# 34j/vr180-convert

Measured on AMD Instinct MI355X. Metric: Mpixels/s dual-fisheye->SBS-equirect remap; achieved HBM GB/s vs peak, higher is better.
Workload: dtype f64; 1 GPU; C2: L+R 4096x4096 fisheye -> 8192x4096 SBS equirect, PolynomialScaler([0,1,-0.1]), bilinear; arithmetic=f64 coordinates (fused chain), u8 pixels with int32 fixed-point blend, split=frames, buffer_sets=4

## Files before the change

include/vr180_remap.h:

```cpp
#ifndef VR180_REMAP_H
#define VR180_REMAP_H

#include <stdint.h>

#ifdef __cplusplus
extern "C" {
#endif

#define V1C_ABI_VERSION 1

#define V1C_OK             0
#define V1C_E_INVALID     -1
#define V1C_E_UNSUPPORTED -2
#define V1C_E_HIP         -3
#define V1C_E_NODEVICE    -4
#define V1C_E_CORRUPT     -5

#define V1C_INTER_NEAREST  0
#define V1C_INTER_LINEAR   1
#define V1C_INTER_CUBIC    2
#define V1C_INTER_AREA     3
#define V1C_INTER_LANCZOS4 4

#define V1C_BORDER_CONSTANT    0
#define V1C_BORDER_REPLICATE   1
#define V1C_BORDER_REFLECT     2
#define V1C_BORDER_WRAP        3
#define V1C_BORDER_REFLECT_101 4
#define V1C_BORDER_TRANSPARENT 5

#define V1C_MAX_OPS    16
#define V1C_MAX_PARAMS 16

enum v1c_opcode {
    V1C_OP_NORMALIZE = 1,
    V1C_OP_DENORMALIZE = 2,
    V1C_OP_DENORMALIZE_INV = 3,
    V1C_OP_ZOOM = 4,
    V1C_OP_ZOOM_INV = 5,
    V1C_OP_EQUIRECT_ENC = 6,
    V1C_OP_EQUIRECT_DEC = 7,
    V1C_OP_RADIAL = 8,
    V1C_OP_ROTATE = 9
};

enum v1c_radial {
    V1C_RAD_ENC_RECTILINEAR   = 1,
    V1C_RAD_ENC_STEREOGRAPHIC = 2,
    V1C_RAD_ENC_EQUIDISTANT   = 3,
    V1C_RAD_ENC_EQUISOLID     = 4,
    V1C_RAD_ENC_ORTHOGRAPHIC  = 5,
    V1C_RAD_DEC_RECTILINEAR   = 6,
    V1C_RAD_DEC_STEREOGRAPHIC = 7,
    V1C_RAD_DEC_EQUIDISTANT   = 8,
    V1C_RAD_DEC_EQUISOLID     = 9,
    V1C_RAD_DEC_ORTHOGRAPHIC  = 10,
    V1C_RAD_POLYNOMIAL        = 11,
    V1C_RAD_RECTDEC_FWD       = 12,
    V1C_RAD_RECTDEC_INV       = 13
};

typedef struct v1c_op {
    int32_t opcode;
    int32_t iparam;
    int32_t nparam;
    int32_t reserved;
    double  p[V1C_MAX_PARAMS];
} v1c_op;

typedef struct v1c_chain {
    int32_t n_ops;
    int32_t reserved;
    v1c_op  ops[V1C_MAX_OPS];
} v1c_chain;

typedef struct v1c_unit {
    const uint8_t* src;
    uint8_t*       dst;
    int64_t        src_pitch;
    int64_t        dst_pitch;
    double         rot[9];
    int32_t        has_rot;
    int32_t        reserved;
} v1c_unit;

typedef struct v1c_plan v1c_plan;


int v1c_abi_version(void);
int v1c_device_count(void);
const char* v1c_last_error(void);


int v1c_plan_create(v1c_plan** out, int device, const v1c_chain* chain,
                    int src_h, int src_w, int dst_h, int dst_w, int cn,
                    int interp, int border_mode, const uint8_t border_val[4]);

#define V1C_DEPTH_8U  0
#define V1C_DEPTH_16U 2
#define V1C_DEPTH_32F 5

int v1c_plan_create_ex(v1c_plan** out, int device, const v1c_chain* chain, int src_h, int src_w,
                       int dst_h, int dst_w, int cn, int depth, int interp, int border_mode,
                       const double border_val[4]);
int v1c_plan_destroy(v1c_plan* plan);

int v1c_plan_path(const v1c_plan* plan);

int v1c_plan_run(v1c_plan* plan, void* stream, const v1c_unit* units, int n_units);

int v1c_plan_run_auto(v1c_plan* plan, void* stream, const v1c_unit* units, int n_units,
                      const double* rad_dev, int n_rad);

int v1c_plan_run_auto_images(v1c_plan* plan, void* stream, const v1c_unit* units, int n_units,
                             int threshold);

int v1c_plan_release_captures(v1c_plan* plan);

enum {
    V1C_LAUNCH_GENERIC = 0,
    V1C_LAUNCH_TILE = 1,
    V1C_LAUNCH_MIRROR = 2,
    V1C_LAUNCH_CN = 3,
    V1C_LAUNCH_CN_ROT = 4,
    V1C_LAUNCH_BATCH = 5,
    V1C_LAUNCH_ROT_PAIR = 6,
    V1C_LAUNCH_WIDE = 7,
    V1C_LAUNCH_CHROMA = 8,
    V1C_LAUNCH_FIXUP = 0x100
};
int v1c_plan_last_launch(const v1c_plan* plan);

int64_t v1c_plan_tap_table_bytes(const v1c_plan* plan);

int v1c_plan_get_map(v1c_plan* plan, void* stream, float* xmap, float* ymap,
                     int64_t map_pitch, const double* rot_or_null);

int v1c_remap_fused(int device, void* stream,
                    const uint8_t* src, int src_h, int src_w, int64_t src_pitch, int cn,
                    uint8_t* dst, int dst_h, int dst_w, int64_t dst_pitch,
                    const v1c_chain* chain, int interp, int border_mode,
                    const uint8_t border_val[4]);

int v1c_fused_cache_size(void);

int v1c_remap_lut(int device, void* stream,
                  const uint8_t* src, int src_h, int src_w, int64_t src_pitch, int cn,
                  uint8_t* dst, int dst_h, int dst_w, int64_t dst_pitch,
                  const float* xmap, const float* ymap, int64_t map_pitch,
                  int interp, int border_mode, const uint8_t border_val[4]);

int v1c_remap_lut_ex(int device, void* stream, const void* src, int src_h, int src_w, int64_t src_pitch,
                     int cn, int depth, void* dst, int dst_h, int dst_w, int64_t dst_pitch,
                     const float* xmap, const float* ymap, int64_t map_pitch,
                     int interp, int border_mode, const double border_val[4]);

int v1c_get_radius(int device, void* stream, const uint8_t* img, int h, int w,
                   int64_t pitch, int cn, int threshold, double* radius);
int v1c_get_radius_async(int device, void* stream, const uint8_t* img, int h, int w,
                         int64_t pitch, int cn, int threshold, double* out_dev);

int v1c_anaglyph(int device, void* stream,
                 const uint8_t* left, int64_t left_pitch, const uint8_t* right, int64_t right_pitch,
                 int h, int w, double* out, int64_t out_pitch);

int v1c_build_itab(int interp, int16_t* out);

int v1c_build_ftab(int interp, float* out);

typedef struct v1c_feat_params {
    double  scale;
    double  radius;
    int32_t fast_threshold;
    int32_t margin;
    int32_t cell;
    int32_t per_cell;
    int32_t max_keypoints;
    int32_t max_distance;
    int32_t ratio_num;
    int32_t ratio_den;
} v1c_feat_params;

typedef struct v1c_feat_kp {
    int32_t x, y;
    int32_t score;
    int32_t bin;
    int32_t src_x2, src_y2;
} v1c_feat_kp;

int v1c_feat_detect(int device, void* stream, const uint8_t* img, int h, int w, int64_t pitch, int cn,
                    const v1c_feat_params* params, v1c_feat_kp* kp_out, uint8_t* desc_out, int32_t* count_out_dev);

int v1c_feat_match(int device, void* stream, const uint8_t* desc_a, int n_a, const uint8_t* desc_b, int n_b,
                   const v1c_feat_params* params, int32_t* pairs_out, int32_t* dist_out, int32_t* count_out_dev);

int v1c_feat_pattern(int8_t* out);

typedef struct v1c_circle_params {
    int32_t threshold;
    int32_t run;
    int32_t rounds;
    int32_t min_points;
    int32_t tol16[8];
} v1c_circle_params;

typedef struct v1c_circle_point {
    int32_t x, y;
    int32_t selected;
} v1c_circle_point;

uint64_t v1c_fit_circle_workspace(int h, int w);

int v1c_fit_circle_async(int device, void* stream, const void* img, int h, int w, int64_t pitch, int cn, int depth,
                         const v1c_circle_params* params, void* workspace, double* out_dev8);

int v1c_fit_circle(int device, void* stream, const void* img, int h, int w, int64_t pitch, int cn, int depth,
                   const v1c_circle_params* params, void* workspace, double* out_host8, v1c_circle_point* points_out,
                   int32_t capacity, int32_t* n_points_out);

#define V1C_CM_MODE_HISTOGRAM   0
#define V1C_CM_MODE_GAIN        1
#define V1C_CM_REFERENCE_LEFT   0
#define V1C_CM_REFERENCE_RIGHT  1

typedef struct v1c_color_match_params {
    int32_t mode;
    int32_t reference;
    int32_t lo, hi;
    int32_t max_shift;
    int32_t min_pixels;
} v1c_color_match_params;

uint64_t v1c_color_match_workspace(void);

int v1c_color_match_luts_async(int device, void* stream, const void* left, int64_t left_pitch, const void* right, int64_t right_pitch,
                               int h, int w, int cn, const v1c_color_match_params* params, void* workspace, uint8_t* luts_dev,
                               int32_t* report_dev);

int v1c_apply_luts_async(int device, void* stream, const void* src, int64_t src_pitch, void* dst, int64_t dst_pitch, int h, int w, int cn,
                         const uint8_t* luts_dev);

#define V1C_PNG_FILTER_UP    2
#define V1C_PNG_FILTER_PAETH 4

typedef struct v1c_png_band {
    uint32_t row0, row1;
    uint64_t offset, size;
    uint32_t adler32;
    uint32_t stored;
} v1c_png_band;

uint64_t v1c_png_bound(int h, int w, int cn, int depth, int band_rows);

int v1c_png_deflate(int device, void* stream, const void* img, int h, int w, int64_t pitch, int cn, int depth, int filter,
                    int band_rows, uint8_t* out_host, uint64_t capacity, v1c_png_band* bands_out, int32_t* n_bands_out,
                    uint64_t* size_out);

#define V1C_JPEG_444 0
#define V1C_JPEG_420 2
#define V1C_JPEG_HEADER_MAX 1024

uint64_t v1c_jpeg_bound(int h, int w, int cn, int subsampling, int restart_mcus);

int64_t v1c_jpeg_header(int h, int w, int cn, int quality, int subsampling, int restart_mcus, uint8_t* out, uint64_t capacity);

int v1c_jpeg_encode(int device, void* stream, const void* img, int h, int w, int64_t pitch, int cn, int quality, int subsampling,
                    int restart_mcus, uint8_t* out_host, uint64_t capacity, uint64_t* size_out);

typedef struct v1c_jpeg_image {
    const void* img;
    int h, w;
    int64_t pitch;
    int cn, quality, subsampling, restart_mcus;
    uint8_t* out_host;
    uint64_t capacity;
    uint64_t size;
} v1c_jpeg_image;
int v1c_jpeg_encode_batch(int device, void* stream, int n, v1c_jpeg_image* images, uint64_t workspace_budget, uint32_t* chunks_out);

#define V1C_JPEG_DHT_MAX (4 * (1 + 16 + 256))
#define V1C_JPEG_HEADER_OPT_MAX 2048

int64_t v1c_jpeg_header_opt(int h, int w, int cn, int quality, int subsampling, int restart_mcus, const uint8_t* dht, uint32_t dht_size,
                            uint8_t* out, uint64_t capacity);

int v1c_jpeg_encode_opt(int device, void* stream, const void* img, int h, int w, int64_t pitch, int cn, int quality, int subsampling,
// ... 144 lines not shown
```

vr180_convert_amd/_native.py:

```python
from __future__ import annotations

import ctypes as C
from pathlib import Path

from . import _abi

import os

LIB_PATH = Path(os.environ.get("V1C_LIB") or (Path(__file__).resolve().parent / "csrc" / "libvr180remap.so"))

SYMBOLS = [
    "v1c_abi_version", "v1c_device_count", "v1c_last_error", "v1c_plan_create", "v1c_plan_destroy",
    "v1c_plan_path", "v1c_plan_run", "v1c_plan_get_map", "v1c_remap_fused", "v1c_remap_lut",
    "v1c_get_radius", "v1c_get_radius_async", "v1c_build_itab", "v1c_anaglyph", "v1c_fused_cache_size", "v1c_plan_last_launch",
    "v1c_plan_release_captures", "v1c_plan_run_auto", "v1c_plan_run_auto_images",
    "v1c_plan_create_ex", "v1c_remap_lut_ex", "v1c_build_ftab",
    "v1c_feat_detect", "v1c_feat_match", "v1c_feat_pattern",
    "v1c_png_bound", "v1c_png_deflate",
    "v1c_jpeg_bound", "v1c_jpeg_header", "v1c_jpeg_encode", "v1c_jpeg_encode_batch",
    "v1c_jpeg_decode_info", "v1c_jpeg_decode", "v1c_jpeg_decode_batch",
    "v1c_jpeg_header_opt", "v1c_jpeg_encode_opt", "v1c_jpeg_encode_batch_opt",
    "v1c_jpeg_prog_info", "v1c_jpeg_prog_decode",
    "v1c_jpeg_transcode_bound", "v1c_jpeg_transcode_check", "v1c_jpeg_header_xc", "v1c_jpeg_transcode",
    "v1c_jpeg_compose_bound", "v1c_jpeg_compose_check", "v1c_jpeg_header_xf", "v1c_jpeg_compose",
    "v1c_fit_circle_workspace", "v1c_fit_circle_async", "v1c_fit_circle",
    "v1c_color_match_workspace", "v1c_color_match_luts_async", "v1c_apply_luts_async",
    "v1c_plan_tap_table_bytes",
    "v1c_ca_plan_create", "v1c_ca_plan_run", "v1c_ca_plan_get_map", "v1c_ca_plan_path", "v1c_ca_plan_last_launch", "v1c_ca_plan_destroy",
]


class EngineUnavailable(RuntimeError):
    """The HIP library is not built / not loadable."""


class EngineError(RuntimeError):
    """A C-ABI call returned an error code."""


_lib = None


def lib() -> C.CDLL:
    global _lib
    if _lib is not None:
        return _lib
    if not LIB_PATH.exists():
        raise EngineUnavailable(
            f"{LIB_PATH} is missing: build the HIP engine first (make -C {LIB_PATH.parent}); "
            "vr180_convert_amd has no CPU fallback"
        )
    try:
        L = C.CDLL(str(LIB_PATH))
    except OSError as e:
        raise EngineUnavailable(f"cannot load {LIB_PATH}: {e}") from e
    vp, i32, i64 = C.c_void_p, C.c_int, C.c_int64
    L.v1c_abi_version.restype = i32
    L.v1c_device_count.restype = i32
    L.v1c_last_error.restype = C.c_char_p
    L.v1c_plan_create.argtypes = [C.POINTER(vp), i32, C.POINTER(_abi.Chain), i32, i32, i32, i32, i32, i32, i32, vp]
    L.v1c_plan_destroy.argtypes = [vp]
    L.v1c_plan_path.argtypes = [vp]
    L.v1c_plan_last_launch.argtypes = [vp]
    L.v1c_plan_last_launch.restype = i32
    try:
        L.v1c_plan_release_captures.argtypes = [vp]
        L.v1c_plan_run_auto.argtypes = [vp, vp, C.POINTER(_abi.Unit), i32, vp, i32]
        L.v1c_plan_run_auto_images.argtypes = [vp, vp, C.POINTER(_abi.Unit), i32, i32]
    except AttributeError:
        pass
    try:
        L.v1c_plan_create_ex.argtypes = [C.POINTER(vp), i32, C.POINTER(_abi.Chain), i32, i32, i32, i32, i32, i32, i32, i32, vp]
        L.v1c_remap_lut_ex.argtypes = [i32, vp, vp, i32, i32, i64, i32, i32, vp, i32, i32, i64, vp, vp, i64, i32, i32, vp]
        L.v1c_build_ftab.argtypes = [i32, vp]
    except AttributeError:
        pass
    try:
        L.v1c_feat_detect.argtypes = [i32, vp, vp, i32, i32, i64, i32, vp, vp, vp, vp]
        L.v1c_feat_match.argtypes = [i32, vp, vp, i32, vp, i32, vp, vp, vp, vp]
        L.v1c_feat_pattern.argtypes = [vp]
    except AttributeError:
        pass
    try:
        L.v1c_png_bound.argtypes = [i32, i32, i32, i32, i32]
        L.v1c_png_bound.restype = C.c_uint64
        L.v1c_png_deflate.argtypes = [i32, vp, vp, i32, i32, i64, i32, i32, i32, i32, vp, C.c_uint64, vp, vp, vp]
    except AttributeError:
        pass
    try:
        L.v1c_jpeg_bound.argtypes = [i32, i32, i32, i32, i32]
        L.v1c_jpeg_bound.restype = C.c_uint64
        L.v1c_jpeg_header.argtypes = [i32, i32, i32, i32, i32, i32, vp, C.c_uint64]
        L.v1c_jpeg_header.restype = i64
        L.v1c_jpeg_encode.argtypes = [i32, vp, vp, i32, i32, i64, i32, i32, i32, i32, vp, C.c_uint64, vp]
    except AttributeError:
        pass
    try:
        L.v1c_jpeg_decode_info.argtypes = [C.c_char_p, C.c_uint64, vp]
        L.v1c_jpeg_decode.argtypes = [i32, vp, C.c_char_p, C.c_uint64, vp, i64, i32, C.c_uint32, vp]
    except AttributeError:
        pass
    try:
        L.v1c_jpeg_decode_batch.argtypes = [i32, vp, i32, vp, vp, vp, vp, vp, C.c_uint32, C.c_uint64, vp, vp, vp]
    except AttributeError:
        pass
    try:
        L.v1c_jpeg_encode_batch.argtypes = [i32, vp, i32, vp, C.c_uint64, vp]
    except AttributeError:
        pass
    try:
        L.v1c_jpeg_header_opt.argtypes = [i32, i32, i32, i32, i32, i32, vp, C.c_uint32, vp, C.c_uint64]
        L.v1c_jpeg_header_opt.restype = i64
        L.v1c_jpeg_encode_opt.argtypes = [i32, vp, vp, i32, i32, i64, i32, i32, i32, i32, vp, C.c_uint64, vp, vp, vp]
        L.v1c_jpeg_encode_batch_opt.argtypes = [i32, vp, i32, vp, C.c_uint64, vp]
    except AttributeError:
        pass
    try:
        L.v1c_jpeg_prog_info.argtypes = [C.c_char_p, C.c_uint64, vp]
        L.v1c_jpeg_prog_decode.argtypes = [i32, vp, C.c_char_p, C.c_uint64, vp, i64, i32, C.c_uint32, vp, vp, C.c_uint32]
    except AttributeError:
        pass
    try:
        L.v1c_jpeg_transcode_bound.argtypes = [C.c_char_p, C.c_uint64, i32, i32, i32]
        L.v1c_jpeg_transcode_bound.restype = C.c_uint64
        L.v1c_jpeg_transcode_check.argtypes = [C.c_char_p, C.c_uint64, i32, vp, vp]
        L.v1c_jpeg_header_xc.argtypes = [C.c_char_p, C.c_uint64, i32, i32, i32, vp, C.c_uint32, vp, C.c_uint64]
        L.v1c_jpeg_header_xc.restype = i64
        L.v1c_jpeg_transcode.argtypes = [i32, vp, C.c_char_p, C.c_uint64, i32, vp, C.c_uint32, vp]
    except AttributeError:
        pass
    try:
        L.v1c_jpeg_compose_bound.argtypes = [C.c_char_p, C.c_uint64, i32, i32, i32]
        L.v1c_jpeg_compose_bound.restype = C.c_uint64
        L.v1c_jpeg_compose_check.argtypes = [i32, vp, i32, vp, vp]
        L.v1c_jpeg_header_xf.argtypes = [C.c_char_p, C.c_uint64, i32, i32, i32, i32, vp, C.c_uint32, vp, C.c_uint64]
        L.v1c_jpeg_header_xf.restype = i64
        L.v1c_jpeg_compose.argtypes = [i32, vp, i32, vp, i32, vp, C.c_uint32, vp]
    except AttributeError:
        pass
    try:
        L.v1c_fit_circle_workspace.argtypes = [i32, i32]
        L.v1c_fit_circle_workspace.restype = C.c_uint64
        L.v1c_fit_circle_async.argtypes = [i32, vp, vp, i32, i32, i64, i32, i32, vp, vp, vp]
        L.v1c_fit_circle.argtypes = [i32, vp, vp, i32, i32, i64, i32, i32, vp, vp, vp, vp, i32, vp]
    except AttributeError:
        pass
    try:
        L.v1c_color_match_workspace.argtypes = []
        L.v1c_color_match_workspace.restype = C.c_uint64
        L.v1c_color_match_luts_async.argtypes = [i32, vp, vp, i64, vp, i64, i32, i32, i32, vp, vp, vp, vp]
        L.v1c_apply_luts_async.argtypes = [i32, vp, vp, i64, vp, i64, i32, i32, i32, vp]
    except AttributeError:
        pass
    try:
        L.v1c_ca_plan_create.argtypes = [C.POINTER(vp), i32, C.POINTER(_abi.Chain), i32, i32, i32, i32, i32, i32, vp]
        L.v1c_ca_plan_run.argtypes = [vp, vp, C.POINTER(_abi.Unit), i32]
        L.v1c_ca_plan_get_map.argtypes = [vp, vp, i32, vp, vp, i64, vp]
        L.v1c_ca_plan_path.argtypes = [vp]
        L.v1c_ca_plan_last_launch.argtypes = [vp]
        L.v1c_ca_plan_destroy.argtypes = [vp]
    except AttributeError:
        pass
    try:
        L.v1c_plan_tap_table_bytes.argtypes = [vp]
        L.v1c_plan_tap_table_bytes.restype = i64
    except AttributeError:
        pass
    L.v1c_plan_run.argtypes = [vp, vp, C.POINTER(_abi.Unit), i32]
    L.v1c_plan_get_map.argtypes = [vp, vp, vp, vp, i64, vp]
    L.v1c_remap_fused.argtypes = [i32, vp, vp, i32, i32, i64, i32, vp, i32, i32, i64, C.POINTER(_abi.Chain), i32, i32, vp]
    L.v1c_remap_lut.argtypes = [i32, vp, vp, i32, i32, i64, i32, vp, i32, i32, i64, vp, vp, i64, i32, i32, vp]
    L.v1c_get_radius.argtypes = [i32, vp, vp, i32, i32, i64, i32, i32, C.POINTER(C.c_double)]
    L.v1c_get_radius_async.argtypes = [i32, vp, vp, i32, i32, i64, i32, i32, vp]
    L.v1c_fused_cache_size.restype = i32
    L.v1c_build_itab.argtypes = [i32, vp]
    L.v1c_anaglyph.argtypes = [i32, vp, vp, i64, vp, i64, i32, i32, vp, i64]
    if L.v1c_abi_version() != _abi.ABI_VERSION:
        raise EngineUnavailable("libvr180remap.so was built for a different ABI version; rebuild it")
    _lib = L
    return L


def check(rc: int, what: str) -> None:
    if rc == _abi.OK:
        return
    msg = lib().v1c_last_error().decode("utf-8", "replace")
    if rc == _abi.E_INVALID:
        raise ValueError(f"{what}: {msg}")
    if rc == _abi.E_UNSUPPORTED:
        raise NotImplementedError(f"{what}: {msg}")
    raise EngineError(f"{what}: {msg} (code {rc})")
```

vr180_convert_amd/csrc/kernels.hpp:

```cpp
#pragma once

#include <cstdlib>
#include <vector>

#include "v1c_core.hpp"

namespace v1c {

#ifdef V1C_TUNING
inline const char* tuning_env(const char* name) { return std::getenv(name); }
#else
inline const char* tuning_env(const char*) { return nullptr; }
#endif

constexpr int kPX = 4;
constexpr int kBlockX = 64;
constexpr int kBlockY = 4;

enum { MODE_LITERAL = 0, MODE_RAY = 1, MODE_LUT = 2, MODE_FIXUP = 3 };

struct KernelCtx {
    Geom g;
    const v1c_chain* chain;
    RayParams ray;
    const short* itab;
    uint32_t* tile_flags;
    const float* xmap;
    const float* ymap;
    int64_t map_pitch;
};

constexpr int kInlineUnits = 16;
struct TileBox;
struct TileArgs {
    const KernelCtx* ctx;
    const DevUnit* units;
    const TileBox* boxes;
    const TileBox* mboxes;
    const uint32_t* rest_list;
    uint32_t* tile_flags;
    int n_units, upb;
    int half_dwords, n_rest;
    unsigned tiles_x_magic, strip_len, strip_magic, rest_rows;
    int mirror_h, kb, tiles_x, same_rot;
    const double *col_s, *col_c, *col_h, *row_s, *row_c, *row_h;
    int dst_w, dst_h, pad2[2];
    DevUnit inl[kInlineUnits];
};

struct LaunchUnits {
    const DevUnit* host;
    const DevUnit* dev;
    int n;
};

int tiles_per_unit(const Geom& g);
hipError_t launch_remap(int mode, const KernelCtx& c, const UnitArgs& ua, int n_units, hipStream_t stream);
hipError_t launch_get_map(int mode, const KernelCtx& c, const UnitArgs& u, float* xmap, float* ymap, int64_t pitch,
                          hipStream_t stream);

struct WideArgs {
    const float* ftab;
    float cval[4];
};
hipError_t launch_remap_wide(int mode, int depth, const KernelCtx& c, const UnitArgs& ua, const WideArgs& wa, int n_units, hipStream_t stream);

hipError_t launch_put_units(DevUnit* dst, const DevUnit* host, int n, hipStream_t stream);
bool tile_kernel_supports(const Geom& g);
bool cn_kernel_supports(const Geom& g);
int tile_cn_box_kb(const void* host_boxes, const Geom& g);
hipError_t launch_ray_lin_cn(const KernelCtx& c, const KernelCtx* cdev, const LaunchUnits& lu, uint32_t* flags, bool use_rot, const void* boxes,
                             int kb, hipStream_t stream);
size_t tile_box_bytes(const Geom& g);
hipError_t launch_tile_boxes(const KernelCtx& c, const KernelCtx* cdev, void* boxes, bool shared_entry, hipStream_t stream, int mirror_h = 0);
bool tile_mirror_rest(const void* host_boxes, const void* host_mboxes, const Geom& g, int half_dwords, int mirror_h,
                      std::vector<uint32_t>& rest, int raw_nwp, bool full_rows = false, int n_eyes = 2);
int tile_mirror_raw_passes(const void* host_boxes, const void* host_mboxes, const Geom& g, int permille = 980, int max_kb = 12);
hipError_t launch_ray_lin3_pair_mirror(const KernelCtx& c, const KernelCtx* cdev, const LaunchUnits& lu, uint32_t* flags, const void* boxes,
                                       const void* mboxes, int half_dwords, int mirror_h, const uint32_t* rest_list, int n_rest, int raw_nwp,
                                       hipStream_t stream, int seq_kb, const void* recs = nullptr, const void* tap_table = nullptr);
size_t tap_table_bytes(const Geom& g);
hipError_t launch_fill_tap_table(const KernelCtx& c, const KernelCtx* cdev, const void* boxes, const void* mboxes, void* table, uint32_t* overflow);
void tile_mirror_records(const void* host_boxes, const void* host_mboxes, size_t n_tiles, const Geom& g, int seq_kb, int one_kb, std::vector<char>& out);
int tile_half_dwords(const void* host_boxes, size_t n_tiles, int max_chunks, bool occupancy_classes);
hipError_t launch_ray_lin3_tile(const KernelCtx& c, const KernelCtx* cdev, const LaunchUnits& lu, uint32_t* flags, bool use_rot, const void* boxes,
                                int half_dwords, bool shared_entry, bool mpoly_all, const uint32_t* rest_list, int n_rest, int lean_half,
                                int strip_len, int lean_raw_nwp, hipStream_t stream, bool coords_bounded = false, int* kind = nullptr,
                                bool same_rot = false);
int tile_xcd_strips(const void* host_boxes, const Geom& g, int half_dwords, int lean_half);
int tile_lean_half_dwords(int half_dwords);
std::vector<uint32_t> tile_rest_list(const void* host_boxes, const Geom& g, int half_dwords, int raw_nwp);
int tile_lean_raw_passes(const void* host_boxes, const Geom& g);

hipError_t launch_anaglyph(const uint8_t* left, int64_t left_pitch, const uint8_t* right, int64_t right_pitch, int h, int w,
                           double* out, int64_t out_pitch, hipStream_t stream);

hipError_t launch_get_radius(const uint8_t* img, int h, int w, int64_t pitch, int cn, int threshold, double* out, hipStream_t stream);

hipError_t launch_patch_radius(KernelCtx* ctx_dev, const double* rad_dev, int n, double r_limit, double cx32, double cy32, hipStream_t stream);
constexpr int kAutoBlocks = 64;
constexpr int kAutoScratchInts = 2 * kInlineUnits + 1;
struct AutoLines {
    const uint8_t* line[kInlineUnits];
    int64_t step[kInlineUnits];
    int n, cn, threshold, count;
};
inline void auto_scratch_init(int* host)
{
    for (int k = 0; k < kInlineUnits; k++)
        host[k] = 0x7fffffff, host[kInlineUnits + k] = -1;
    host[2 * kInlineUnits] = 0;
}
hipError_t launch_auto_radius(KernelCtx* ctx_dev, int* scratch_dev, const AutoLines& im, double r_limit, double cx32, double cy32, hipStream_t stream);

}
```

vr180_convert_amd/csrc/kernels_mirror.hip:

```cpp
#include "tile_device.hpp"

namespace v1c {

__device__ __forceinline__ void sample_pair_cells(units_cptr U, const TileIds& t, int j, const TileBox& b, const uint32_t* boxw,
                                                  const int (&sx)[kPX], const int (&sy)[kPX])
{
    typedef uint32_t __attribute__((ext_vector_type(2))) u32x2;
    typedef const __attribute__((address_space(3))) u32x2* lds_u64_ptr;
    const uint32_t lpw8 = (uint32_t)(b.cpr * 4 + 4) * 8u;
    const uint32_t base0 = (uint32_t)(uintptr_t)(lds_u32_ptr)boxw - ((uint32_t)b.y0 * lpw8 + (uint32_t)b.x0 * 8u);
    Taps2 T0, T1;
#pragma unroll
    for (int k = 0; k < kPX; k++) {
        const uint32_t rel = __umul24((uint32_t)(sy[k] >> 5), lpw8) + (((uint32_t)sx[k] >> 2) & ~7u);
        const lds_u64_ptr ra = (lds_u64_ptr)(uintptr_t)(rel + base0), rb = (lds_u64_ptr)(uintptr_t)(rel + base0 + lpw8);
        const u32x2 a_lo = ra[0], a_hi = ra[1], b_lo = rb[0], b_hi = rb[1];
        T0.alo[k] = a_lo.x, T0.ahi[k] = a_hi.x, T0.blo[k] = b_lo.x, T0.bhi[k] = b_hi.x;
        T1.alo[k] = a_lo.y, T1.ahi[k] = a_hi.y, T1.blo[k] = b_lo.y, T1.bhi[k] = b_hi.y;
    }
    uint32_t pix[kPX];
    const uint32_t row_off = (uint32_t)t.x0 * 3u;
#pragma unroll
    for (int e = 0; e < 2; e++) {
#pragma unroll
        for (int k = 0; k < kPX; k++) {
            const BlendW w = blend_weights(sx[k], sy[k]);
            pix[k] = e == 0 ? blend3<4>(T0.alo[k], T0.ahi[k], T0.blo[k], T0.bhi[k], w) : blend3<4>(T1.alo[k], T1.ahi[k], T1.blo[k], T1.bhi[k], w);
        }
        uint8_t* drow = U[e].dst + (__umul24((uint32_t)j, (uint32_t)U[e].dst_pitch) + row_off);
        store4(drow, pix, 0xFu, dst_rows_dword_aligned(U, e));
    }
}

#ifdef V1C_TUNING
template <int VAR_W>
__global__ __launch_bounds__(256) __attribute__((amdgpu_waves_per_eu(5, 8))) void k_ray_lin3_pair_mirror(TileArgs a_)
{
    constexpr int NT = 256;
    __shared__ __attribute__((aligned(16))) double tabw[kTabSlice * kRadialCoefs];
    extern __shared__ __attribute__((aligned(16))) uint32_t dyn_box[];
    args_cref a = kernel_args();
    const int tid = threadIdx.x;
    if (blockIdx.z == 0) {
        const unsigned lin = blockIdx.y * gridDim.x + blockIdx.x;
        if (lin >= (unsigned)a.n_rest)
            return;
        const uint32_t v = ((const V1C_CONST uint32_t*)a.rest_list)[lin];
        shared_map_tile<VAR_W, 0, 2, 0, 1, NT, 0>(a, 2, 2, 0, (int)(v & 0xffffu), (int)(v >> 16), (int)gridDim.x, dyn_box, a.half_dwords,
                                                  tabw, (glb_u32_ptr) nullptr);
        return;
    }
    ctx_cref c = args_ctx(a);
    const units_cptr U = args_units(a);
    const TileBox* __restrict__ boxes = a.boxes;
    const TileBox* __restrict__ mboxes = a.mboxes;
    const int half_dwords = a.half_dwords, mirror_h = a.mirror_h;
    geom_cref g = c.g;
    ray_cref P = c.ray;
    int tx, ty;
    xcd_tile(a.tiles_x_magic, a.strip_len, a.strip_magic, tx, ty);
    ty += 1;
    const TileIds t = tile_ids(g, 0, tid, tx, ty, (int)gridDim.x, NT / kLanesX);
    const uint8_t* __restrict__ src0 = U[0].src;
    const uint8_t* __restrict__ src1 = U[1].src;
    const uint32_t pitch0 = (uint32_t)U[0].src_pitch, pitch1 = (uint32_t)U[1].src_pitch;
    const TileBox b = load_tile_box(boxes, t.box_tile), q = load_tile_box(mboxes, t.box_tile);
    if (!mirror_static_ok(b, q, half_dwords, g.src_h, g.src_w))
        return;
    ChunkMap M;
    make_chunk_map<NT>(b, tid, M);
    Staged S0, S1;
    stage_load<false, false>(M, src0, pitch0, 0u, S0);
    stage_load<false, false>(M, src1, pitch1, 0u, S1);
    typedef double __attribute__((ext_vector_type(2))) d2;
    d2 tv = {0.0, 0.0};
    const bool mpoly = (b.interior & 2) != 0;
    if (tid < b.nidx * 4)
        tv = ((const d2*)(radial_table(P, mpoly) + (size_t)b.idx0 * kRadialCoefs))[tid];
    RowCol rc;
    load_rowcol<0>(P, t.xc, t.jc, rc);
    stage_store_pair(M, S0, S1, dyn_box);
    if (tid < b.nidx * 4)
        ((d2*)tabw)[tid] = tv;
    __syncthreads();
    make_chunk_map<NT>(q, tid, M);
    stage_load<false, false>(M, src0, pitch0, 0u, S0);
    stage_load<false, false>(M, src1, pitch1, 0u, S1);
    LaneCoords L;
    if (mpoly)
        lane_coords<VAR_W, 0, 2, 0, 1, 1, 1>(c, nullptr, rc, kPX, (const double*)tabw, b.idx0, b.nidx, L);
    else
        lane_coords<VAR_W, 0, 2, 0, 1, 0, 1>(c, nullptr, rc, kPX, (const double*)tabw, b.idx0, b.nidx, L);
    sample_pair_cells(U, t, t.j, b, dyn_box, L.sx, L.sy);
    __syncthreads();
    stage_store_pair(M, S0, S1, dyn_box);
    __syncthreads();
    sample_pair_cells(U, t, mirror_h - t.j, q, dyn_box, L.sx, L.sy2);
}
#endif

template <int VAR_W, int NE, int REC>
__device__ __forceinline__ void mirror_raw_tile(V1C_MIRROR_HEAD, double* tabw, uint32_t* dyn_box)
{
    static_assert(!REC || NE == 1, "the record serves the one-eye form");
    constexpr int NT = 256;
    if (V1C_PRIO & 4)
        __builtin_amdgcn_s_setprio(3);
    args_cref a = kernel_args<kMirrorHeadBytes>();
    const int tid = threadIdx.x;
    const unsigned tiles_x = gx_rest & 0xffffu, rest_rows = gx_rest >> 16;
    if (blockIdx.y < rest_rows) {
        const unsigned lin = blockIdx.y * tiles_x + blockIdx.x;
        if (lin >= (unsigned)a.n_rest)
            return;
        const uint32_t v = ((const V1C_CONST uint32_t*)a.rest_list)[lin];
        shared_map_tile<VAR_W, 0, 2, 0, 1, NT, 0>(a, NE, 2, 0, (int)(v & 0xffffu), (int)(v >> 16), (int)tiles_x, dyn_box, a.half_dwords,
                                                  tabw, (glb_u32_ptr) nullptr);
        return;
    }
    int tx, ty;
    {
        const unsigned slen = ((rows_strip >> 16) * tiles_x) & (REC ? 0x7fffffffu : 0xffffffffu);
        xcd_tile_at(tiles_x_magic, slen, ((tiles_x_magic - 1u) >> 1) + 1u, tx, ty, rows_strip & 0xffffu, rest_rows, tiles_x, 0u);
    }
    const DstSize dsz{(int)(dst_wh & 0xffffu), (int)(dst_wh >> 16)};
    const TileIds t = tile_ids(dsz, 0, tid, tx, ty, (int)tiles_x, NT / kLanesX);
    RowCol rc;
    load_rowcol<0>(rowcol_tables_at(rowcol_tables, dsz.dst_w, dsz.dst_h), t.xc, t.jc, rc);
    TileBoxPair bq{};
    MirrorRec r{};
    if constexpr (REC)
        r = load_mirror_rec(pairs, t.box_tile);
    else
        bq = load_tile_box_pair(pairs, t.box_tile);
    const TileBox &b = bq.b, &q = bq.q;
    ctx_cref c = *(const V1C_CONST KernelCtx*)ctxp;
    const units_cptr U = (units_cptr)a.inl;
    geom_cref g = c.g;
    ray_cref P = c.ray;
    touch_plan_and_units<0, NE>(c, U, 0, NE - 1);
    const int nwp = (int)(kb_mh & 0xffffu);
    if (REC ? !(r.flags & kMirrorRecFitOne) : mirror_raw_fit(b, q, nwp, g.src_h, g.src_w) != 1)
        return;
    const bool mpoly = REC ? (r.flags & kMirrorRecMpoly) != 0 : (b.interior & 2) != 0;
    const int idx0 = REC ? r.idx0 : b.idx0, nidx = REC ? r.nidx : b.nidx;
#pragma unroll
    for (int k = 0; k < kPX; k++)
        asm volatile("" ::"v"(rc.slon[k]), "v"(rc.qlon[k]));
    asm volatile("" ::"v"(rc.sl), "v"(rc.cl), "v"(rc.hl));
    const uint32_t lds_tab = (uint32_t)(uintptr_t)(lds_u32_ptr)(const uint32_t*)tabw;
    const uint32_t box_bytes = (uint32_t)nwp * 1024u;
    const uint32_t raw_b = (uint32_t)(uintptr_t)(lds_u32_ptr)dyn_box, raw_q = raw_b + (uint32_t)NE * box_bytes;
// ... 76 lines not shown
#endif
__device__ __forceinline__ void gather_taps_raw(const uint32_t (&ta)[kPX], const BlendW (&W)[kPX], uint32_t pitch, uint32_t (&pix)[kPX])
{
#pragma unroll
    for (int k = 0; k < kPX; k++) {
        const uint32_t a = ta[k], d = a & ~3u;
        const lds_u32_ptr r0 = (lds_u32_ptr)(uintptr_t)d, r1 = (lds_u32_ptr)(uintptr_t)(d + pitch);
        const uint32_t a0 = r0[0], a1 = r0[1], a2 = r0[2], b0 = r1[0], b1 = r1[1], b2 = r1[2];
        pix[k] = blend3<3>(__builtin_amdgcn_alignbyte(a1, a0, a), __builtin_amdgcn_alignbyte(a2, a1, a), __builtin_amdgcn_alignbyte(b1, b0, a),
                           __builtin_amdgcn_alignbyte(b2, b1, a), W[k]);
    }
}

template <int VAR_W, int REST, int REC>
__device__ __forceinline__ void mirror_seq_tile(V1C_MIRROR_HEAD, double* tabw, uint32_t* dyn_box)
{
    constexpr int NT = 256;
    if (V1C_PRIO & 4)
        __builtin_amdgcn_s_setprio(3);
    args_cref a = kernel_args<kMirrorHeadBytes>();
    const int tid = threadIdx.x;
    const unsigned tiles_x = gx_rest & 0xffffu, rest_rows = REST ? gx_rest >> 16 : 0u;
    if constexpr (REST) {
        if (blockIdx.y < rest_rows) {
            const unsigned lin = blockIdx.y * tiles_x + blockIdx.x;
            if (lin >= (unsigned)a.n_rest)
                return;
            const uint32_t v = ((const V1C_CONST uint32_t*)a.rest_list)[lin];
            shared_map_tile<VAR_W, 0, 2, 0, 1, NT, 0>(a, 2, 2, 0, (int)(v & 0xffffu), (int)(v >> 16), (int)tiles_x, dyn_box,
                                                      a.half_dwords, tabw, (glb_u32_ptr) nullptr);
            return;
        }
    }
    int tx, ty;
    {
        const unsigned slen = ((rows_strip >> 16) * tiles_x) & (REC ? 0x7fffffffu : 0xffffffffu);
        xcd_tile_at(tiles_x_magic, slen, ((tiles_x_magic - 1u) >> 1) + 1u, tx, ty, rows_strip & 0xffffu, rest_rows, tiles_x, 0u);
    }
    const DstSize dsz{(int)(dst_wh & 0xffffu), (int)(dst_wh >> 16)};
    const TileIds t = tile_ids(dsz, 0, tid, tx, ty, (int)tiles_x, NT / kLanesX);
    RowCol rc;
    load_rowcol<0>(rowcol_tables_at(rowcol_tables, dsz.dst_w, dsz.dst_h), t.xc, t.jc, rc);
    TileBoxPair bq{};
    MirrorRec r{};
    if constexpr (REC)
        r = load_mirror_rec(pairs, t.box_tile);
    else
        bq = load_tile_box_pair(pairs, t.box_tile);
    const TileBox &b = bq.b, &q = bq.q;
    ctx_cref c = *(const V1C_CONST KernelCtx*)ctxp;
    const units_cptr U = (units_cptr)a.inl;
    geom_cref g = c.g;
    ray_cref P = c.ray;
    touch_plan_and_units<0, 2>(c, U, 0, 1);
    const int cap_kb = (int)(kb_mh & 0xffffu);
    if (REC ? !(r.flags & kMirrorRecFitSeq) : mirror_raw_fit(b, q, cap_kb, g.src_h, g.src_w) != 1)
        return;
    const bool mpoly = REC ? (r.flags & kMirrorRecMpoly) != 0 : (b.interior & 2) != 0;
    const int idx0 = REC ? r.idx0 : b.idx0, nidx = REC ? r.nidx : b.nidx;
#pragma unroll
    for (int k = 0; k < kPX; k++)
        asm volatile("" ::"v"(rc.slon[k]), "v"(rc.qlon[k]));
    asm volatile("" ::"v"(rc.sl), "v"(rc.cl), "v"(rc.hl));
    const uint32_t lds_tab = (uint32_t)(uintptr_t)(lds_u32_ptr)(const uint32_t*)tabw;
    const uint32_t raw_b = (uint32_t)(uintptr_t)(lds_u32_ptr)dyn_box, raw_q = raw_b + (uint32_t)cap_kb * 1024u;
    const int wave = __builtin_amdgcn_readfirstlane(tid >> 6), lane = tid & 63;
    {
        const uint32_t u = min((uint32_t)tid, (uint32_t)(nidx * 4 - 1));
        const uint8_t* gp = (const uint8_t*)(radial_table(P, mpoly) + (size_t)idx0 * kRadialCoefs) + u * 16u;
        __builtin_amdgcn_global_load_lds((glb_void_ptr)gp, (lds_void_ptr)(uintptr_t)(lds_tab + (uint32_t)__builtin_amdgcn_readfirstlane(tid & ~63) * 16u), 16, 0, 0);
    }
    const RawLanes mb = REC ? rec_lanes(r.b, lane) : raw_lanes(b.cpr, lane), mq = REC ? rec_lanes(r.q, lane) : raw_lanes(q.cpr, lane);
    auto request = [&](int e, int which) {
        const uint8_t* src = U[e].src;
        const uint32_t sp = (uint32_t)U[e].src_pitch;
        if constexpr (REC)
            return which == 0 ? rec_box_dma(r.b, mb, src, sp, lane, wave, raw_b) : rec_box_dma(r.q, mq, src, sp, lane, wave, raw_q);
        else
            return which == 0 ? raw_box_dma(b, mb, src, sp, lane, wave, raw_b) : raw_box_dma(q, mq, src, sp, lane, wave, raw_q);
    };
    const int nb = request(0, 0);
    const int nq = request(0, 1);
    if (V1C_PRIO & 4)
        __builtin_amdgcn_s_setprio(0);
    wait_vm_barrier(nb + nq);
    const uint32_t pitch_b = REC ? r.b.lpitch : (uint32_t)raw_units_per_row(b.cpr) * 16u, pitch_q = REC ? r.q.lpitch : (uint32_t)raw_units_per_row(q.cpr) * 16u;
    uint32_t ta_b[kPX], ta_q[kPX];
    BlendW W_b[kPX], W_q[kPX];
    {
        LaneCoords L;
        if (mpoly)
            lane_coords<VAR_W, 0, 2, 0, 1, 1, 1, 0, REC>(c, nullptr, rc, kPX, (const double*)tabw, idx0, nidx, L);
        else
            lane_coords<VAR_W, 0, 2, 0, 1, 0, 1, 0, REC>(c, nullptr, rc, kPX, (const double*)tabw, idx0, nidx, L);
        const uint32_t kb = r.b.tapk + raw_b, kq = r.q.tapk + raw_q;
#pragma unroll
        for (int k = 0; k < kPX; k++) {
            if constexpr (REC) {
                const uint32_t bx = ((uint32_t)L.sx[k] >> 5), x3 = bx * 2u + bx;
                ta_b[k] = mad24_vsv((uint32_t)L.sy[k] >> 5, pitch_b, x3 + kb);
                ta_q[k] = mad24_vsv((uint32_t)L.sy2[k] >> 5, pitch_q, x3 + kq);
            } else {
                const uint32_t ixb = (uint32_t)((L.sx[k] >> 5) - b.x0), ixq = (uint32_t)((L.sx[k] >> 5) - q.x0);
                ta_b[k] = __umul24((uint32_t)((L.sy[k] >> 5) - b.y0), pitch_b) + (ixb * 2u + ixb) + raw_b;
                ta_q[k] = __umul24((uint32_t)((L.sy2[k] >> 5) - q.y0), pitch_q) + (ixq * 2u + ixq) + raw_q;
            }
            W_b[k] = blend_weights(L.sx[k], L.sy[k]);
            W_q[k] = blend_weights(L.sx[k], L.sy2[k]);
        }
    }
    const uint32_t row_off = (uint32_t)t.x0 * 3u;
    const int jm = (int)(kb_mh >> 16) - t.j;
    const bool band_row = jm < dsz.dst_h;
    auto drow = [&](int e, int j) {
        return (REC ? mul24_vs((uint32_t)j, (uint32_t)U[e].dst_pitch) : __umul24((uint32_t)j, (uint32_t)U[e].dst_pitch)) + row_off;
    };
    uint32_t pix[kPX];
    wait_vm_barrier(nq);
    gather_taps_raw(ta_b, W_b, pitch_b, pix);
    asm volatile("s_waitcnt vmcnt(0) lgkmcnt(0)\n\ts_barrier" ::: "memory");
    request(1, 0);
    store4<1>(U[0].dst + drow(0, t.j), pix, 0xFu, dst_rows_dword_aligned(U, 0));
    gather_taps_raw(ta_q, W_q, pitch_q, pix);
    asm volatile("s_waitcnt lgkmcnt(0)\n\ts_barrier" ::: "memory");
    request(1, 1);
    if (band_row)
        store4<1>(U[0].dst + drow(0, jm), pix, 0xFu, dst_rows_dword_aligned(U, 0));
    wait_vm_barrier(nq + 1);
    gather_taps_raw(ta_b, W_b, pitch_b, pix);
    wait_vm_barrier_imm<0>();
    store4<1>(U[1].dst + drow(1, t.j), pix, 0xFu, dst_rows_dword_aligned(U, 1));
    gather_taps_raw(ta_q, W_q, pitch_q, pix);
    if (band_row)
        store4<1>(U[1].dst + drow(1, jm), pix, 0xFu, dst_rows_dword_aligned(U, 1));
}

template <int VAR_W, int REST = 1>
__global__ __launch_bounds__(256) __attribute__((amdgpu_waves_per_eu(REST ? V1C_SEQ_WAVES : V1C_SEQ_WAVES + 1, 8))) void k_ray_lin3_pair_mirror_seq(V1C_MIRROR_HEAD, TileArgs a_)
{
    __shared__ __attribute__((aligned(16))) double tabw[kTabSlice * kRadialCoefs];
    extern __shared__ __attribute__((aligned(16))) uint32_t dyn_box[];
    mirror_seq_tile<VAR_W, REST, 1>(pairs, tiles_x_magic, gx_rest, rows_strip, dst_wh, rowcol_tables, ctxp, kb_mh, tabw, dyn_box);
}
#ifdef V1C_TUNING
template <int VAR_W, int REST = 1>
__global__ __launch_bounds__(256) __attribute__((amdgpu_waves_per_eu(REST ? V1C_SEQ_WAVES : V1C_SEQ_WAVES + 1, 8))) void k_ray_lin3_pair_mirror_seq_box(V1C_MIRROR_HEAD, TileArgs a_)
{
    __shared__ __attribute__((aligned(16))) double tabw[kTabSlice * kRadialCoefs];
    extern __shared__ __attribute__((aligned(16))) uint32_t dyn_box[];
    mirror_seq_tile<VAR_W, REST, 0>(pairs, tiles_x_magic, gx_rest, rows_strip, dst_wh, rowcol_tables, ctxp, kb_mh, tabw, dyn_box);
}
#endif

constexpr int kTapSliceBytes = 256 * kTapEntryBytes;
__global__ __launch_bounds__(256) __attribute__((amdgpu_waves_per_eu(V1C_SEQ_WAVES + 1, 8))) void k_ray_lin3_pair_mirror_seq_tab(V1C_MIRROR_HEAD, TileArgs a_)
{
    constexpr int NT = 256;
    __shared__ __attribute__((aligned(16))) uint32_t tapw[kTapSliceBytes / 4];
    extern __shared__ __attribute__((aligned(16))) uint32_t dyn_box[];
    if (V1C_PRIO & 4)
        __builtin_amdgcn_s_setprio(3);
    args_cref a = kernel_args<kMirrorHeadBytes>();
    const int tid = threadIdx.x;
    const unsigned tiles_x = gx_rest & 0xffffu;
    int tx, ty;
    {
        const unsigned slen = ((rows_strip >> 16) * tiles_x) & 0x7fffffffu;
        xcd_tile_at(tiles_x_magic, slen, ((tiles_x_magic - 1u) >> 1) + 1u, tx, ty, rows_strip & 0xffffu, 0u, tiles_x, 0u);
    }
    const DstSize dsz{(int)(dst_wh & 0xffffu), (int)(dst_wh >> 16)};
    const TileIds t = tile_ids(dsz, 0, tid, tx, ty, (int)tiles_x, NT / kLanesX);
    const MirrorRec r = load_mirror_rec(pairs, t.box_tile);
    const units_cptr U = (units_cptr)a.inl;
    const uint8_t* usrc[2] = {U[0].src, U[1].src};
    uint8_t* udst[2] = {U[0].dst, U[1].dst};
    uint32_t uspitch[2] = {(uint32_t)U[0].src_pitch, (uint32_t)U[1].src_pitch}, udpitch[2] = {(uint32_t)U[0].dst_pitch, (uint32_t)U[1].dst_pitch};
    asm volatile("" : "+s"(usrc[0]), "+s"(usrc[1]), "+s"(udst[0]), "+s"(udst[1]), "+s"(uspitch[0]), "+s"(uspitch[1]), "+s"(udpitch[0]), "+s"(udpitch[1]));
    const bool ualigned[2] = {((((uintptr_t)udst[0]) | (uintptr_t)udpitch[0]) & 3u) == 0, ((((uintptr_t)udst[1]) | (uintptr_t)udpitch[1]) & 3u) == 0};
    const int cap_kb = (int)(kb_mh & 0xffffu);
    if (!(r.flags & kMirrorRecFitSeq))
        return;
    const uint32_t lds_tap = (uint32_t)(uintptr_t)(lds_u32_ptr)(const uint32_t*)tapw;
    const uint32_t raw_b = (uint32_t)(uintptr_t)(lds_u32_ptr)dyn_box, raw_q = raw_b + (uint32_t)cap_kb * 1024u;
    const int wave = __builtin_amdgcn_readfirstlane(tid >> 6), lane = tid & 63;
    {
        const uint32_t wave_off = (uint32_t)__builtin_amdgcn_readfirstlane(tid & ~63) * (uint32_t)kTapEntryBytes;
        const uint8_t* gp = (const uint8_t*)rowcol_tables + ((size_t)(uint32_t)__builtin_amdgcn_readfirstlane(t.box_tile) * (size_t)kTapSliceBytes + wave_off) +
                            (uint32_t)lane * 16u;
        if (lane < 64 * kTapEntryBytes / 16)
            __builtin_amdgcn_global_load_lds((glb_void_ptr)gp, (lds_void_ptr)(uintptr_t)(lds_tap + wave_off), 16, 0, 0);
    }
    const RawLanes mb = rec_lanes(r.b, lane), mq = rec_lanes(r.q, lane);
    auto request = [&](int e, int which) {
        const uint8_t* src = usrc[e];
        const uint32_t sp = uspitch[e];
        return which == 0 ? rec_box_dma(r.b, mb, src, sp, lane, wave, raw_b) : rec_box_dma(r.q, mq, src, sp, lane, wave, raw_q);
    };
    const int nb = request(0, 0);
    const int nq = request(0, 1);
    if (V1C_PRIO & 4)
        __builtin_amdgcn_s_setprio(0);
    wait_vm_barrier(nb + nq);
    const uint32_t pitch_b = r.b.lpitch, pitch_q = r.q.lpitch;
    uint32_t ta_b[kPX], ta_q[kPX];
    BlendW W_b[kPX], W_q[kPX];
    {
        const lds_u32_ptr ep = (lds_u32_ptr)(uintptr_t)(lds_tap + (uint32_t)tid * (uint32_t)kTapEntryBytes);
        const TapCoords tc = tap_entry_decode(TapEntry{{ep[0], ep[1], ep[2]}});
        const uint32_t kb = raw_b, kq = raw_q + (uint32_t)(r.b.x3 - r.q.x3);
#pragma unroll
        for (int k = 0; k < kPX; k++) {
            const uint32_t ix = (uint32_t)tc.x[k] >> 5, x3 = ix * 2u + ix;
            ta_b[k] = mad24_vsv((uint32_t)tc.y[k] >> 5, pitch_b, x3 + kb);
            ta_q[k] = mad24_vsv((uint32_t)tc.y2[k] >> 5, pitch_q, x3 + kq);
            W_b[k] = blend_weights(tc.x[k], tc.y[k]);
            W_q[k] = blend_weights(tc.x[k], tc.y2[k]);
        }
    }
    const uint32_t row_off = (uint32_t)t.x0 * 3u;
    const int jm = (int)(kb_mh >> 16) - t.j;
    const bool band_row = jm < dsz.dst_h;
    auto drow = [&](int e, int j) { return mul24_vs((uint32_t)j, udpitch[e]) + row_off; };
    uint32_t pix[kPX];
    wait_vm_barrier(nq);
    gather_taps_raw(ta_b, W_b, pitch_b, pix);
    asm volatile("s_waitcnt vmcnt(0) lgkmcnt(0)\n\ts_barrier" ::: "memory");
    request(1, 0);
    store4<1>(udst[0] + drow(0, t.j), pix, 0xFu, ualigned[0]);
    gather_taps_raw(ta_q, W_q, pitch_q, pix);
    asm volatile("s_waitcnt lgkmcnt(0)\n\ts_barrier" ::: "memory");
    request(1, 1);
    if (band_row)
        store4<1>(udst[0] + drow(0, jm), pix, 0xFu, ualigned[0]);
    wait_vm_barrier(nq + 1);
    gather_taps_raw(ta_b, W_b, pitch_b, pix);
    wait_vm_barrier_imm<0>();
    store4<1>(udst[1] + drow(1, t.j), pix, 0xFu, ualigned[1]);
    gather_taps_raw(ta_q, W_q, pitch_q, pix);
    if (band_row)
        store4<1>(udst[1] + drow(1, jm), pix, 0xFu, ualigned[1]);
}

template <int VAR_W>
__global__ __launch_bounds__(256) void k_fill_tap_table(const KernelCtx* ctxp, const TileBox* __restrict__ boxes, const TileBox* __restrict__ mboxes,
                                                        int tiles_x, uint32_t* __restrict__ table, uint32_t* overflow)
{
    ctx_cref c = *(const V1C_CONST KernelCtx*)ctxp;
    ray_cref P = c.ray;
    const int tid = threadIdx.x;
    const TileIds t = tile_ids(c.g, 0, tid, (int)blockIdx.x, (int)blockIdx.y, tiles_x, 256 / kLanesX);
    const TileBox b = boxes[t.box_tile], q = mboxes[t.box_tile];
    RowCol rc;
    load_rowcol<0>(P, t.xc, t.jc, rc);
    const bool mpoly = (b.interior & 2) != 0;
    const int nidx = max(b.nidx, 1), idx0 = max(b.idx0, 0);
    const double* tab = (mpoly ? P.radial_m : P.radial) + (size_t)idx0 * kRadialCoefs;
    LaneCoords L;
    if (mpoly)
        lane_coords<VAR_W, 0, 2, 0, 1, 1, 1, 0, 1>(c, nullptr, rc, kPX, tab, idx0, nidx, L);
    else
        lane_coords<VAR_W, 0, 2, 0, 1, 0, 1, 0, 1>(c, nullptr, rc, kPX, tab, idx0, nidx, L);
    TapCoords tc;
#pragma unroll
    for (int k = 0; k < kPX; k++) {
        tc.x[k] = (int)((uint32_t)L.sx[k] - kRoundBias) - 32 * b.x0;
        tc.y[k] = (int)((uint32_t)L.sy[k] - kRoundBias) - 32 * b.y0;
        tc.y2[k] = (int)((uint32_t)L.sy2[k] - kRoundBias) - 32 * q.y0;
    }
    if (!tap_entry_fits(tc))
        atomicOr(overflow, 1u);
    const TapEntry e = tap_entry_encode(tc);
    uint32_t* out = table + ((size_t)t.box_tile * 256u + (size_t)tid) * 3u;
    out[0] = e.w[0], out[1] = e.w[1], out[2] = e.w[2];
}

size_t tap_table_bytes(const Geom& g)
{
    const dim3 full = tile_grid(g, 256, 1);
    return (size_t)full.x * (size_t)(full.y / 2 + 1) * (size_t)kTapSliceBytes;
}

hipError_t launch_fill_tap_table(const KernelCtx& c, const KernelCtx* cdev, const void* boxes, const void* mboxes, void* table, uint32_t* overflow)
{
    const dim3 full = tile_grid(c.g, 256, 1);
    const dim3 grid(full.x, full.y / 2 + 1, 1), block(256, 1, 1);
    if (c.ray.var_is_w)
        hipLaunchKernelGGL((k_fill_tap_table<1>), grid, block, 0, 0, cdev, (const TileBox*)boxes, (const TileBox*)mboxes, (int)full.x, (uint32_t*)table, overflow);
    else
        hipLaunchKernelGGL((k_fill_tap_table<0>), grid, block, 0, 0, cdev, (const TileBox*)boxes, (const TileBox*)mboxes, (int)full.x, (uint32_t*)table, overflow);
    return hipGetLastError();
}

int tile_mirror_raw_passes(const void* host_boxes, const void* host_mboxes, const Geom& g, int permille, int max_kb)
{
    const TileBox* b = (const TileBox*)host_boxes;
    const TileBox* q = (const TileBox*)host_mboxes;
    const dim3 d = tile_grid(g, tile_threads(g), 1);
    std::vector<int> hist(kRawMaxWavePasses + 2, 0);
    size_t n = 0;
    for (unsigned ty = 0; ty <= d.y / 2; ty++)
        for (unsigned tx = 0; tx < d.x; tx++) {
            const size_t i = (size_t)ty * d.x + tx;
            if (b[i].cpr <= 0 || q[i].cpr <= 0 || b[i].cpr > kMaxCpr || q[i].cpr > kMaxCpr)
                continue;
            const int u = std::max(b[i].nrows * raw_units_per_row(b[i].cpr), q[i].nrows * raw_units_per_row(q[i].cpr));
            hist[std::min((u + 63) / 64, kRawMaxWavePasses + 1)]++, n++;
        }
    size_t acc = 0;
    for (int k = 0; k <= kRawMaxWavePasses; k++) {
        acc += hist[k];
        if (acc * 1000 >= n * (size_t)permille)
            return std::min(std::max(k, 4), max_kb);
    }
    return max_kb;
}

bool tile_mirror_rest(const void* host_boxes, const void* host_mboxes, const Geom& g, int half_dwords, int mirror_h,
                      std::vector<uint32_t>& rest, int raw_nwp, bool full_rows, int n_eyes)
{
    const TileBox* b = (const TileBox*)host_boxes;
    const TileBox* q = (const TileBox*)host_mboxes;
    const dim3 d = tile_grid(g, tile_threads(g), 1);
    rest.clear();
    const int th = tile_threads(g) / kLanesX;
    if (mirror_h != g.dst_h || g.dst_h % (2 * th) != 0 || g.dst_w % 4 != 0 || d.x > 0xffffu || d.y > 0xffffu)
        return false;
    const unsigned TY = d.y, TYh = TY / 2;
    if (TYh < 3)
        return false;
    std::vector<uint8_t> in_rest((size_t)d.x * d.y, 0);
    auto add = [&](unsigned tx, unsigned ty) { in_rest[(size_t)ty * d.x + tx] = 1; };
    if (full_rows && raw_nwp > 0) {
        for (unsigned ty = 0; ty <= TYh; ty++)
            for (unsigned tx = 0; tx < d.x; tx++) {
                const size_t i = (size_t)ty * d.x + tx;
                const int fit = mirror_raw_fit(b[i], q[i], raw_nwp, g.src_h, g.src_w);
                if (fit != 1) {
                    add(tx, ty);
                    if (ty < TYh) {
                        add(tx, TY - 1 - ty);
                        if (ty > 0)
                            add(tx, TY - ty);
                    }
                }
            }
    } else {
        for (unsigned tx = 0; tx < d.x; tx++)
            add(tx, 0), add(tx, TYh), add(tx, TY - 1);
        for (unsigned ty = 1; ty < TYh; ty++)
            for (unsigned tx = 0; tx < d.x; tx++) {
                const size_t i = (size_t)ty * d.x + tx;
                if (raw_nwp > 0 ? !mirror_raw_static_ok(b[i], q[i], raw_nwp, g.src_h, g.src_w) : !mirror_static_ok(b[i], q[i], half_dwords, g.src_h, g.src_w))
                    add(tx, ty), add(tx, TY - 1 - ty), add(tx, TY - ty);
            }
    }
    for (unsigned ty = 0; ty < d.y; ty++)
        for (unsigned tx = 0; tx < d.x; tx++)
            if (in_rest[(size_t)ty * d.x + tx])
                rest.push_back(ty << 16 | tx);
    return rest.size() <= (size_t)d.x * (TYh - 1) && rest.size() * 4 <= (size_t)d.x * d.y;
}

void tile_mirror_records(const void* host_boxes, const void* host_mboxes, size_t n_tiles, const Geom& g, int seq_kb, int one_kb, std::vector<char>& out)
{
    const TileBox* b = (const TileBox*)host_boxes;
    const TileBox* q = (const TileBox*)host_mboxes;
    out.resize(n_tiles * sizeof(MirrorRecWords));
    for (size_t i = 0; i < n_tiles; i++) {
        const MirrorRecWords w = mirror_rec_encode(b[i], q[i], seq_kb, one_kb, g.src_h, g.src_w);
        std::memcpy(&out[i * sizeof(MirrorRecWords)], &w, sizeof(w));
    }
}

hipError_t launch_ray_lin3_pair_mirror(const KernelCtx& c, const KernelCtx* cdev, const LaunchUnits& lu, uint32_t* flags, const void* boxes,
                                       const void* mboxes, int half_dwords, int mirror_h, const uint32_t* rest_list, int n_rest, int raw_nwp,
                                       hipStream_t stream, int seq_kb, const void* recs, const void* tap_table)
{
    const int n_eyes = lu.n;
    const dim3 full = tile_grid(c.g, 256, 1);
    const dim3 block(256, 1, 1);
    TileArgs a = tile_args(c, cdev, lu, flags);
    a.boxes = (const TileBox*)boxes, a.mboxes = (const TileBox*)mboxes;
    a.rest_list = rest_list, a.n_rest = n_rest;
    a.half_dwords = half_dwords, a.mirror_h = mirror_h;
    a.tiles_x_magic = (unsigned)(0x100000000ull / full.x) + 1u;
    static const unsigned strip_rows = [] {
        const char* e = tuning_env("V1C_MIRROR_STRIP_ROWS");
        return e ? (unsigned)std::atoi(e) : 2u;
    }();
    static const unsigned block_rows = [] {
        const char* e = tuning_env("V1C_MIRROR_BLOCK_ROWS");
        return e ? (unsigned)std::atoi(e) : 0u;
    }();
    [[maybe_unused]] auto strips = [&](unsigned rows) {
        const unsigned per = (full.x * rows) >> 3;
        unsigned slen = strip_rows && strip_rows * full.x < per ? strip_rows * full.x : 0u;
        if (block_rows && full.x % 8 == 0 && raw_nwp > 0)
            slen = 0x80000000u | std::min(block_rows, 0xffffu);
        a.strip_len = slen;
        a.strip_magic = (slen && !(slen & 0x80000000u)) ? (unsigned)(0x100000000ull / slen) + 1u : 0u;
    };
    const unsigned raw_rows = full.y / 2 + 1;
    const unsigned rest_rows = ((((unsigned)n_rest + full.x - 1) / full.x) + 7u) & ~7u;
    const unsigned srows = strip_rows == 2u && 2u * full.x < ((full.x * raw_rows) >> 3) ? 2u : 0u;
    const unsigned rows_strip = raw_rows | srows << 16, dst_wh = (unsigned)c.g.dst_w | (unsigned)c.g.dst_h << 16;
    const TileBox* head_pairs = (const TileBox*)recs;
#define V1C_MIRROR_LAUNCH(KERNEL, GRID, LDS, RESTROWS)                                                                                    \
    hipLaunchKernelGGL(KERNEL, GRID, block, LDS, stream, head_pairs, a.tiles_x_magic, full.x | (unsigned)(RESTROWS) << 16, rows_strip, dst_wh, \
                       a.col_s, a.ctx, (unsigned)a.kb | (unsigned)a.mirror_h << 16, a)
    [[maybe_unused]] bool rec_off = false;
#ifdef V1C_TUNING
    static const bool rec_off_env = [] {
        const char* e = tuning_env("V1C_MIRROR_REC");
        return e && e[0] == '0';
    }();
    rec_off = rec_off_env;
#endif
    if (seq_kb > 0 && n_eyes == 2) {
        static const bool norest_off = [] {
            const char* e = tuning_env("V1C_SEQ_NOREST");
            return e && e[0] == '0';
        }();
        a.kb = seq_kb;
        if (!rec_off && recs == nullptr)
            return hipErrorInvalidValue;
        if (n_rest == 0 && !norest_off) {
            const dim3 rgrid(full.x, raw_rows, 1);
            const size_t slds = (size_t)2 * 1024 * (size_t)seq_kb + 16;
            a.rest_rows = 0;
#ifdef V1C_TUNING
            if (rec_off) {
                head_pairs = a.mboxes;
                if (c.ray.var_is_w)
                    V1C_MIRROR_LAUNCH((k_ray_lin3_pair_mirror_seq_box<1, 0>), rgrid, slds, 0u);
                else
                    V1C_MIRROR_LAUNCH((k_ray_lin3_pair_mirror_seq_box<0, 0>), rgrid, slds, 0u);
                return hipGetLastError();
            }
            static const bool tab_off = [] {
                const char* e = tuning_env("V1C_MIRROR_TAB");
                return e && e[0] == '0';
            }();
            if (tab_off)
                tap_table = nullptr;
#endif
            if (tap_table) {
                hipLaunchKernelGGL(k_ray_lin3_pair_mirror_seq_tab, rgrid, block, slds, stream, head_pairs, a.tiles_x_magic, full.x, rows_strip, dst_wh,
                                   (const double*)tap_table, a.ctx, (unsigned)a.kb | (unsigned)a.mirror_h << 16, a);
                return hipGetLastError();
            }
            if (c.ray.var_is_w)
                V1C_MIRROR_LAUNCH((k_ray_lin3_pair_mirror_seq<1, 0>), rgrid, slds, 0u);
            else
                V1C_MIRROR_LAUNCH((k_ray_lin3_pair_mirror_seq<0, 0>), rgrid, slds, 0u);
            return hipGetLastError();
        }
        const dim3 rgrid(full.x, raw_rows + rest_rows, 1);
        const size_t slds = std::max((size_t)half_dwords * 8 + 16, (size_t)2 * 1024 * (size_t)seq_kb);
        a.rest_rows = rest_rows;
#ifdef V1C_TUNING
        if (rec_off) {
            head_pairs = a.mboxes;
            if (c.ray.var_is_w)
                V1C_MIRROR_LAUNCH((k_ray_lin3_pair_mirror_seq_box<1>), rgrid, slds, rest_rows);
            else
                V1C_MIRROR_LAUNCH((k_ray_lin3_pair_mirror_seq_box<0>), rgrid, slds, rest_rows);
            return hipGetLastError();
        }
#endif
        if (c.ray.var_is_w)
            V1C_MIRROR_LAUNCH((k_ray_lin3_pair_mirror_seq<1>), rgrid, slds, rest_rows);
        else
            V1C_MIRROR_LAUNCH((k_ray_lin3_pair_mirror_seq<0>), rgrid, slds, rest_rows);
        return hipGetLastError();
    }
    if (raw_nwp > 0 && n_eyes == 1) {
        const dim3 rgrid(full.x, raw_rows + rest_rows, 1);
        const size_t lds = std::max((size_t)half_dwords * 4 + 16, (size_t)2 * 1024 * (size_t)raw_nwp);
        a.kb = raw_nwp, a.rest_rows = rest_rows;
        if (!rec_off && recs == nullptr)
            return hipErrorInvalidValue;
#ifdef V1C_TUNING
        if (rec_off) {
            head_pairs = a.mboxes;
            if (c.ray.var_is_w)
                V1C_MIRROR_LAUNCH((k_ray_lin3_pair_mirror_box_raw<1>), rgrid, lds, rest_rows);
            else
                V1C_MIRROR_LAUNCH((k_ray_lin3_pair_mirror_box_raw<0>), rgrid, lds, rest_rows);
            return hipGetLastError();
        }
#endif
        if (c.ray.var_is_w)
            V1C_MIRROR_LAUNCH((k_ray_lin3_pair_mirror_raw<1, 1>), rgrid, lds, rest_rows);
        else
            V1C_MIRROR_LAUNCH((k_ray_lin3_pair_mirror_raw<0, 1>), rgrid, lds, rest_rows);
        return hipGetLastError();
    }
#ifdef V1C_TUNING
    if (n_eyes != 2)
        return hipErrorInvalidValue;
    const size_t lds = std::max((size_t)half_dwords * 8 + 16, (size_t)4 * 1024 * (size_t)std::max(raw_nwp, 0));
    if (raw_nwp > 0) {
        dim3 rgrid(full.x, raw_rows + rest_rows, 1);
        strips(raw_rows);
        a.kb = raw_nwp, a.rest_rows = rest_rows;
        static const int skip = [] {
            const char* e = tuning_env("V1C_MIRROR_SKIP");
            return e ? std::atoi(e) : 0;
        }();
        if (skip == 1)
            a.n_rest = 0, a.rest_rows = 0, rgrid.y = raw_rows;
        if (skip == 2)
            rgrid.y = rest_rows;
        const unsigned rr = skip == 1 ? 0u : rest_rows;
        head_pairs = a.mboxes;
        if (c.ray.var_is_w)
            V1C_MIRROR_LAUNCH((k_ray_lin3_pair_mirror_raw<1, 2>), rgrid, lds, rr);
        else
            V1C_MIRROR_LAUNCH((k_ray_lin3_pair_mirror_raw<0, 2>), rgrid, lds, rr);
        return hipGetLastError();
    }
    const dim3 grid(full.x, full.y / 2 - 1, 2);
    strips(grid.y);
    if (c.ray.var_is_w)
        hipLaunchKernelGGL((k_ray_lin3_pair_mirror<1>), grid, block, lds, stream, a);
    else
        hipLaunchKernelGGL((k_ray_lin3_pair_mirror<0>), grid, block, lds, stream, a);
    return hipGetLastError();
#else
    return hipErrorInvalidValue;
#endif
}

}
```

vr180_convert_amd/csrc/plan.hip:

```cpp
#include <hip/hip_runtime.h>

#include <algorithm>
#include <atomic>
#include <chrono>
#include <cmath>
#include <cstdio>
#include <cstdlib>
#include <cstring>
#include <list>
#include <map>
#include <memory>
#include <mutex>
#include <string>
#include <vector>

#include "../../include/vr180_remap.h"
#include "host_util.hpp"
#include "kernels.hpp"
#include "radial_fit.hpp"

using namespace v1c;

static thread_local std::string g_err;

static int fail(int code, const std::string& msg)
{
    g_err = msg;
    return code;
}

namespace v1c {
int set_error(int code, const std::string& msg)
{
    return fail(code, msg);
}
}

#define HIP_TRY(expr)                                                                                   \
    do {                                                                                                \
        hipError_t _e = (expr);                                                                         \
        if (_e != hipSuccess)                                                                           \
            return fail(V1C_E_HIP, std::string(#expr) + ": " + hipGetErrorString(_e));                  \
    } while (0)

static int cv_round_host(float v)
{
    return (std::fabs(v) < 2147483648.0f) ? (int)std::nearbyintf(v) : INT_MIN;
}

static short sat_short_host(int v)
{
    return (short)std::min(32767, std::max(-32768, v));
}

static void coeffs_1d(int interp, float x, float* c)
{
    if (interp == V1C_INTER_CUBIC) {
        const float A = -0.75f;
        c[0] = ((A * (x + 1) - 5 * A) * (x + 1) + 8 * A) * (x + 1) - 4 * A;
        c[1] = ((A + 2) * x - (A + 3)) * x * x + 1;
        c[2] = ((A + 2) * (1 - x) - (A + 3)) * (1 - x) * (1 - x) + 1;
        c[3] = 1.f - c[0] - c[1] - c[2];
        return;
    }
    static const double s45 = 0.70710678118654752440084436210485;
    static const double cs[][2] = {{1, 0},  {-s45, -s45}, {0, 1},  {s45, -s45},
                                   {-1, 0}, {s45, s45},   {0, -1}, {-s45, s45}};
    if (x < 1.1920928955078125e-07f) {
        for (int i = 0; i < 8; i++)
            c[i] = 0;
        c[3] = 1;
        return;
    }
    float sum = 0;
    const double y0 = -(x + 3) * 3.1415926535897932384626433832795 * 0.25, s0 = std::sin(y0), c0 = std::cos(y0);
    for (int i = 0; i < 8; i++) {
        const double y = -(x + 3 - i) * 3.1415926535897932384626433832795 * 0.25;
        c[i] = (float)((cs[i][0] * s0 + cs[i][1] * c0) / (y * y));
        sum += c[i];
    }
    sum = 1.f / sum;
    for (int i = 0; i < 8; i++)
        c[i] *= sum;
}

#pragma clang fp contract(off)
static std::vector<short> build_itab(int interp)
{
    const int K = interp == V1C_INTER_CUBIC ? 4 : 8;
    std::vector<float> t1(32 * K);
    for (int i = 0; i < 32; i++)
        coeffs_1d(interp, i * (1.f / 32), &t1[i * K]);
    std::vector<short> tab((size_t)1024 * K * K);
    for (int fy = 0; fy < 32; fy++)
        for (int fx = 0; fx < 32; fx++) {
            short* e = &tab[(size_t)(fy * 32 + fx) * K * K];
            int isum = 0;
            for (int k1 = 0; k1 < K; k1++)
                for (int k2 = 0; k2 < K; k2++) {
                    const float v = t1[fy * K + k1] * t1[fx * K + k2];
                    e[k1 * K + k2] = sat_short_host(cv_round_host(v * 32768));
                    isum += e[k1 * K + k2];
                }
            if (isum != 32768) {
                const int diff = isum - 32768, h = K / 2;
                int Mk = h * K + h, mk = h * K + h;
                for (int k1 = h; k1 < h + 2; k1++)
                    for (int k2 = h; k2 < h + 2; k2++) {
                        const int q = k1 * K + k2;
                        if (e[q] < e[mk])
                            mk = q;
                        else if (e[q] > e[Mk])
                            Mk = q;
                    }
                if (diff < 0)
                    e[Mk] = (short)(e[Mk] - diff);
                else
                    e[mk] = (short)(e[mk] - diff);
            }
        }
    return tab;
}
#pragma clang fp contract(fast)

extern "C" int v1c_build_itab(int interp, int16_t* out)
{
    if (!out || (interp != V1C_INTER_CUBIC && interp != V1C_INTER_LANCZOS4))
        return fail(V1C_E_INVALID, "v1c_build_itab: interp must be CUBIC or LANCZOS4, out non-NULL");
    const std::vector<short> tab = build_itab(interp);
    std::memcpy(out, tab.data(), tab.size() * sizeof(short));
    return V1C_OK;
}

#pragma clang fp contract(off)
static std::vector<float> build_ftab(int interp)
{
    const int K = interp == V1C_INTER_LINEAR ? 2 : (interp == V1C_INTER_CUBIC ? 4 : 8);
    std::vector<float> t1(32 * K);
    for (int i = 0; i < 32; i++) {
        if (K == 2) {
            t1[i * 2 + 1] = i * (1.f / 32);
            t1[i * 2] = 1.f - t1[i * 2 + 1];
        } else {
            coeffs_1d(interp, i * (1.f / 32), &t1[i * K]);
        }
    }
    std::vector<float> tab((size_t)1024 * K * K);
    for (int fy = 0; fy < 32; fy++)
        for (int fx = 0; fx < 32; fx++)
            for (int k1 = 0; k1 < K; k1++)
                for (int k2 = 0; k2 < K; k2++)
                    tab[((size_t)(fy * 32 + fx) * K + k1) * K + k2] = t1[fy * K + k1] * t1[fx * K + k2];
    return tab;
}
#pragma clang fp contract(fast)

extern "C" int v1c_build_ftab(int interp, float* out)
{
    if (!out || (interp != V1C_INTER_LINEAR && interp != V1C_INTER_CUBIC && interp != V1C_INTER_LANCZOS4))
        return fail(V1C_E_INVALID, "v1c_build_ftab: interp must be LINEAR, CUBIC or LANCZOS4, out non-NULL");
    const std::vector<float> tab = build_ftab(interp);
    std::memcpy(out, tab.data(), tab.size() * sizeof(float));
    return V1C_OK;
}

static int depth_bytes(int depth)
{
    return depth == V1C_DEPTH_8U ? 1 : depth == V1C_DEPTH_16U ? 2 : depth == V1C_DEPTH_32F ? 4 : 0;
}

static void border_for_depth(int depth, const double* bv, uint8_t cval8[4], float cvalf[4])
{
    for (int k = 0; k < 4; k++) {
        const double v = bv ? bv[k] : 0.0;
        cval8[k] = (uint8_t)border_component(V1C_DEPTH_8U, v);
        cvalf[k] = border_component(depth, v);
    }
}

static constexpr size_t kTapTableMaxBytes = (size_t)64 << 20;

struct v1c_plan {
    int device = 0;
    int mode = MODE_LITERAL;
    v1c_chain chain{};
    RayAnalysis ana;
    RadialTable table;
    bool chain_has_rot = false;
    int n_rot_stages = 0;
    bool ray_no_rot_safe = false;
    bool ray_plan_rot_safe = false;
    bool front_hemisphere = false;
    KernelCtx ctx{};
    KernelCtx* ctx_dev = nullptr;
    static constexpr int kRingSlots = 4, kCaptureSlots = 4, kRingUnits = 256;
    DevUnit* ring = nullptr;
    hipEvent_t ring_ev[kRingSlots] = {nullptr, nullptr, nullptr, nullptr};
    hipStream_t ring_last[kRingSlots] = {nullptr, nullptr, nullptr, nullptr};
    bool ring_used[kRingSlots] = {false, false, false, false};
    int ring_next = 0, capture_next = 0;
    std::mutex ring_mu;
    int tiles = 0;
    void* tile_boxes = nullptr;
    int half_dwords = 256;
    const uint32_t* rest_list = nullptr;
    int n_rest = 0;
    int lean_half = 256;
    int lean_raw_nwp = 0;
    int strip_len = 0;
    void* mirror_boxes = nullptr;
    const void* mirror_recs = nullptr;
    const void* tap_table = nullptr;
    size_t tap_table_bytes = 0;
    const void* mirror_pairs = nullptr;
    const uint32_t* mirror_rest = nullptr;
    int n_mirror_rest = 0;
    int cn_kb = 0;
    int mirror_seq_kb = 0;
    const uint32_t* mirror_rest1 = nullptr;
    int n_mirror_rest1 = -1;
    int mirror_raw_nwp = 0;
    int mirror_h = 0;
    bool disable_fast = false;
    bool disable_coords_bounded = false;
    bool disable_shared_entry = false;
    bool disable_mpoly = false;
    bool plan_shared_entry = false;
    double ray_step = 0;
    int mp_valid_upto = -1;
    int gen_mode = 0;
    TableStep step;
    double m_reach_norot = 0;
    std::vector<double> g_bounds;
    std::mutex flags_mu;
    hipEvent_t flags_ev = nullptr;
    hipStream_t flags_stream = nullptr;
    bool flags_pending = false;
    int depth = V1C_DEPTH_8U;
    WideArgs wide{};
    std::atomic<int> last_launch{-1};
    KernelCtx* ctx_dyn = nullptr;
    int* auto_scratch = nullptr;
    std::mutex dyn_mu;
    hipEvent_t dyn_ev = nullptr;
    hipStream_t dyn_stream = nullptr;
    bool dyn_pending = false;
    std::vector<void*> allocs;
};

template <typename T>
static int upload(v1c_plan* p, const std::vector<T>& h, const T** out)
{
    void* d = nullptr;
    HIP_TRY(hipMalloc(&d, std::max<size_t>(h.size() * sizeof(T), 16)));
    p->allocs.push_back(d);
    if (!h.empty())
        HIP_TRY(hipMemcpy(d, h.data(), h.size() * sizeof(T), hipMemcpyHostToDevice));
    *out = (const T*)d;
    return V1C_OK;
}

static int validate_chain(const v1c_chain* ch)
{
    if (!ch)
        return fail(V1C_E_INVALID, "chain is NULL");
    if (ch->n_ops < 1 || ch->n_ops > V1C_MAX_OPS)
        return fail(V1C_E_INVALID, "chain.n_ops out of range");
    for (int i = 0; i < ch->n_ops; i++) {
        const v1c_op& op = ch->ops[i];
        if (op.opcode < V1C_OP_NORMALIZE || op.opcode > V1C_OP_ROTATE)
            return fail(V1C_E_INVALID, "unknown opcode in chain");
        if (op.nparam < 0 || op.nparam > V1C_MAX_PARAMS)
            return fail(V1C_E_INVALID, "op.nparam out of range");
        if (op.opcode == V1C_OP_RADIAL && (op.iparam < V1C_RAD_ENC_RECTILINEAR || op.iparam > V1C_RAD_RECTDEC_INV))
            return fail(V1C_E_INVALID, "unknown radial kind in chain");
    }
    return V1C_OK;
}

static int validate_geom(int src_h, int src_w, int dst_h, int dst_w, int cn, int interp, int border)
{
    if (src_h <= 0 || src_w <= 0 || dst_h <= 0 || dst_w <= 0)
        return fail(V1C_E_INVALID, "image sizes must be positive");
    if (src_h >= 32768 || src_w >= 32768 || dst_h >= 32768 || dst_w >= 32768)
        return fail(V1C_E_INVALID, "image sizes must be < 32768 (cv2.remap limit)");
    if (cn != 1 && cn != 3 && cn != 4)
        return fail(V1C_E_INVALID, "cn must be 1, 3 or 4");
    if (interp < V1C_INTER_NEAREST || interp > V1C_INTER_LANCZOS4)
        return fail(V1C_E_INVALID, "unknown interpolation");
    if (border < V1C_BORDER_CONSTANT || border > V1C_BORDER_TRANSPARENT)
        return fail(V1C_E_INVALID, "unknown border mode");
    return V1C_OK;
}

extern "C" int v1c_abi_version(void)
{
    return V1C_ABI_VERSION;
}

extern "C" int v1c_device_count(void)
{
    int n = 0;
    if (hipGetDeviceCount(&n) != hipSuccess)
        return fail(V1C_E_NODEVICE, "hipGetDeviceCount failed");
    return n;
}

extern "C" const char* v1c_last_error(void)
{
    return g_err.c_str();
}

extern "C" int v1c_plan_destroy(v1c_plan* p)
{
    if (!p)
        return V1C_OK;
    DeviceGuard dg(p->device);
    for (void* d : p->allocs)
        (void)hipFree(d);
    if (p->flags_ev)
        (void)hipEventDestroy(p->flags_ev);
    if (p->dyn_ev)
        (void)hipEventDestroy(p->dyn_ev);
    for (hipEvent_t e : p->ring_ev)
        if (e)
            (void)hipEventDestroy(e);
    delete p;
    return V1C_OK;
}

static int plan_common(v1c_plan* p, int device, int src_h, int src_w, int dst_h, int dst_w, int cn, int interp,
                       int border_mode, const uint8_t border_val[4])
{
    p->device = device;
    Geom& g = p->ctx.g;
    g.src_h = src_h, g.src_w = src_w, g.dst_h = dst_h, g.dst_w = dst_w;
    g.cn = cn;
    g.interp = interp == V1C_INTER_AREA ? V1C_INTER_LINEAR : interp;
    g.border = border_mode;
    for (int k = 0; k < 4; k++)
        g.cval[k] = border_val ? border_val[k] : 0;
    p->tiles = tiles_per_unit(g);
    if (g.interp == V1C_INTER_CUBIC || g.interp == V1C_INTER_LANCZOS4) {
        const std::vector<short> tab = build_itab(g.interp);
        int rc = upload(p, tab, &p->ctx.itab);
        if (rc)
            return rc;
    }
    return V1C_OK;
}

namespace {
struct FitKey {
    std::string ops;
    int n_int, fn, force_var;
    double m_max, m_front;
    bool operator==(const FitKey& o) const
    {
        return n_int == o.n_int && fn == o.fn && force_var == o.force_var && m_max == o.m_max && m_front == o.m_front && ops == o.ops;
    }
};
struct FitEntry {
    FitKey key;
    std::shared_ptr<const RadialTable> table;
    std::shared_ptr<const MPolyTable> mpoly;
};
// ... 243 lines not shown
                }
                void* ring = nullptr;
                if (e == hipSuccess)
                    e = hipMalloc(&ring, sizeof(DevUnit) * (size_t)(v1c_plan::kRingSlots + v1c_plan::kCaptureSlots) * v1c_plan::kRingUnits);
                if (e == hipSuccess)
                    p->allocs.push_back(ring);
                for (int k = 0; k < v1c_plan::kRingSlots && e == hipSuccess; k++)
                    e = hipEventCreateWithFlags(&p->ring_ev[k], hipEventDisableTiming);
                if (e != hipSuccess) {
                    v1c_plan_destroy(p);
                    return fail(V1C_E_HIP, std::string("plan context upload: ") + hipGetErrorString(e));
                }
                p->ctx_dev = (KernelCtx*)dctx;
                p->ring = (DevUnit*)ring;
                void* ddyn = nullptr;
                const size_t ctx_bytes = (sizeof(KernelCtx) + 15) & ~(size_t)15;
                e = hipMalloc(&ddyn, ctx_bytes + kAutoScratchInts * sizeof(int));
                if (e == hipSuccess) {
                    p->allocs.push_back(ddyn);
                    e = hipMemcpy(ddyn, &p->ctx, sizeof(KernelCtx), hipMemcpyHostToDevice);
                }
                if (e == hipSuccess) {
                    int init[kAutoScratchInts];
                    auto_scratch_init(init);
                    e = hipMemcpy((char*)ddyn + ctx_bytes, init, sizeof(init), hipMemcpyHostToDevice);
                }
                if (e == hipSuccess)
                    e = hipEventCreateWithFlags(&p->dyn_ev, hipEventDisableTiming);
                if (e != hipSuccess) {
                    v1c_plan_destroy(p);
                    return fail(V1C_E_HIP, std::string("plan context (dynamic radius): ") + hipGetErrorString(e));
                }
                p->ctx_dyn = (KernelCtx*)ddyn;
                p->auto_scratch = (int*)((char*)ddyn + ctx_bytes);
            }
            t_up = now_ms();
            const Geom& g = p->ctx.g;
            if (p->depth == V1C_DEPTH_8U && cn_kernel_supports(g) && p->plan_shared_entry && !p->disable_shared_entry && p->gen_mode == 0) {
                void* bx = nullptr;
                e = hipMalloc(&bx, tile_box_bytes(g));
                if (e == hipSuccess) {
                    p->allocs.push_back(bx);
                    e = launch_tile_boxes(p->ctx, p->ctx_dev, bx, true, nullptr);
                }
                std::vector<char> hb(tile_box_bytes(g));
                if (e == hipSuccess)
                    e = hipMemcpy(hb.data(), bx, hb.size(), hipMemcpyDeviceToHost);
                if (e != hipSuccess) {
                    v1c_plan_destroy(p);
                    return fail(V1C_E_HIP, std::string("tile boxes (cn): ") + hipGetErrorString(e));
                }
                p->tile_boxes = bx;
                p->cn_kb = tile_cn_box_kb(hb.data(), g);
                if (const char* kbsw = tuning_env("V1C_CN_KB"))
                    p->cn_kb = std::min(std::max(std::atoi(kbsw), 0), 16);
                if (const char* dbg = tuning_env("V1C_DEBUG"); dbg && dbg[0] == '1')
                    std::fprintf(stderr, "[v1c] cn = %d tile kernel: box buffers of %d KB\n", g.cn, p->cn_kb);
            }
            if (p->depth == V1C_DEPTH_8U && tile_kernel_supports(g)) {
                void* bx = nullptr;
                e = hipMalloc(&bx, tile_box_bytes(g));
                if (e == hipSuccess) {
                    p->allocs.push_back(bx);
                    e = launch_tile_boxes(p->ctx, p->ctx_dev, bx, p->plan_shared_entry && !p->disable_shared_entry, nullptr);
                }
                if (e != hipSuccess) {
                    v1c_plan_destroy(p);
                    return fail(V1C_E_HIP, std::string("tile boxes: ") + hipGetErrorString(e));
                }
                p->tile_boxes = bx;
                std::vector<char> hb(tile_box_bytes(g));
                e = hipMemcpy(hb.data(), bx, hb.size(), hipMemcpyDeviceToHost);
                if (e != hipSuccess) {
                    v1c_plan_destroy(p);
                    return fail(V1C_E_HIP, std::string("tile boxes readback: ") + hipGetErrorString(e));
                }
                p->half_dwords = tile_half_dwords(hb.data(), hb.size() / 32, (p->gen_mode != 0 && (g.interp == V1C_INTER_LANCZOS4 || g.interp == V1C_INTER_CUBIC)) ? 2048 : 1024,
                                                  g.interp == V1C_INTER_LINEAR || g.interp == V1C_INTER_NEAREST);
                if (const char* e = tuning_env("V1C_HALF_CAP"); e && std::atoi(e) >= 256)
                    p->half_dwords = std::min(p->half_dwords, std::atoi(e));
                {
                    p->lean_half = tile_lean_half_dwords(p->half_dwords);
                    p->strip_len = tile_xcd_strips(hb.data(), g, p->half_dwords, p->lean_half);
                    if (const char* dbg = tuning_env("V1C_DEBUG"); dbg && dbg[0] == '1')
                        std::fprintf(stderr, "[v1c] XCD interleave: strips of %d tiles\n", p->strip_len);
                    {
                        const char* sw = tuning_env("V1C_LEAN_RAW");
                        const int v = sw ? std::atoi(sw) : 1;
                        p->lean_raw_nwp = v == 1 ? tile_lean_raw_passes(hb.data(), g) : v > 1 ? std::min(v, 16) : 0;
                    }
                    const std::vector<uint32_t> rest = tile_rest_list(hb.data(), g, p->lean_half, p->lean_raw_nwp);
                    const dim3 full((unsigned)((g.dst_w + 63) / 64), (unsigned)((g.dst_h + 15) / 16));
                    if (full.x <= 0xffffu && full.y <= 0xffffu) {
                        if ((rc = upload(p, rest, &p->rest_list))) {
                            v1c_plan_destroy(p);
                            return rc;
                        }
                        p->n_rest = (int)rest.size();
                    }
                    if (const char* dbg = tuning_env("V1C_DEBUG"); dbg && dbg[0] == '1')
                        std::fprintf(stderr, "[v1c] lean batch kernel: %d of %zu tiles left to the general kernel (raw box KB %d)\n", p->n_rest, hb.size() / 32, p->lean_raw_nwp);
                }
                t_boxes = now_ms();
                {
                    const char* off = tuning_env("V1C_DISABLE_MIRROR");
                    const double two_cy = 2.0 * p->ana.norm_cy;
                    if (!(off && off[0] == '1') && g.interp == V1C_INTER_LINEAR && !p->ana.has_rot && p->plan_shared_entry &&
                        !p->disable_shared_entry && two_cy == (double)g.dst_h) {
                        void* mbx = nullptr;
                        e = hipMalloc(&mbx, tile_box_bytes(g));
                        if (e == hipSuccess) {
                            p->allocs.push_back(mbx);
                            e = launch_tile_boxes(p->ctx, p->ctx_dev, mbx, true, nullptr, g.dst_h);
                        }
                        std::vector<char> hm(tile_box_bytes(g));
                        if (e == hipSuccess)
                            e = hipMemcpy(hm.data(), mbx, hm.size(), hipMemcpyDeviceToHost);
                        if (e != hipSuccess) {
                            v1c_plan_destroy(p);
                            return fail(V1C_E_HIP, std::string("mirror boxes: ") + hipGetErrorString(e));
                        }
                        std::vector<uint32_t> mrest;
                        const char* rawsw = tuning_env("V1C_MIRROR_RAW");
                        const int rawv = rawsw ? std::atoi(rawsw) : 1;
                        p->mirror_raw_nwp = rawv == 1 ? tile_mirror_raw_passes(hb.data(), hm.data(), g) : rawv > 1 ? std::min(rawv, 16) : 0;
                        const char* seqsw = tuning_env("V1C_MIRROR_SEQ");
                        const char* seqkb = tuning_env("V1C_MIRROR_SEQ_KB");
                        if (p->mirror_raw_nwp > 0 && !(seqsw && seqsw[0] == '0'))
                            p->mirror_seq_kb = seqkb ? std::min(std::max(std::atoi(seqkb), 2), 16) : tile_mirror_raw_passes(hb.data(), hm.data(), g, 998, 11);
                        if (tile_mirror_rest(hb.data(), hm.data(), g, p->half_dwords, g.dst_h, mrest,
                                             p->mirror_seq_kb > 0 ? p->mirror_seq_kb : p->mirror_raw_nwp, true, 2)) {
                            if ((rc = upload(p, mrest, &p->mirror_rest))) {
                                v1c_plan_destroy(p);
                                return rc;
                            }
                            p->mirror_boxes = mbx, p->n_mirror_rest = (int)mrest.size(), p->mirror_h = g.dst_h;
#ifdef V1C_TUNING
                            {
                                std::vector<char> pairs(2 * hb.size());
                                for (size_t i = 0; i < hb.size() / 32; i++) {
                                    std::memcpy(&pairs[64 * i], &hb[32 * i], 32);
                                    std::memcpy(&pairs[64 * i + 32], &hm[32 * i], 32);
                                }
                                const char* dp = nullptr;
                                if ((rc = upload(p, pairs, &dp))) {
                                    v1c_plan_destroy(p);
                                    return rc;
                                }
                                p->mirror_pairs = dp;
                            }
#endif
                            if (p->mirror_raw_nwp > 0) {
                                std::vector<char> recs;
                                tile_mirror_records(hb.data(), hm.data(), hb.size() / 32, g, p->mirror_seq_kb, p->mirror_raw_nwp, recs);
                                const char* dr = nullptr;
                                if ((rc = upload(p, recs, &dr))) {
                                    v1c_plan_destroy(p);
                                    return rc;
                                }
                                p->mirror_recs = dr;
                            }
                            if (p->mirror_recs && p->mirror_seq_kb > 0 && mrest.empty() && tap_table_bytes(g) <= kTapTableMaxBytes) {
                                const size_t tb = tap_table_bytes(g);
                                void* tt = nullptr;
                                uint32_t over = 1;
                                if (hipMalloc(&tt, tb + 16) == hipSuccess) {
                                    uint32_t* flag = (uint32_t*)((char*)tt + tb);
                                    hipError_t te = hipMemset(flag, 0, 16);
                                    if (te == hipSuccess)
                                        te = launch_fill_tap_table(p->ctx, p->ctx_dev, p->tile_boxes, mbx, tt, flag);
                                    if (te == hipSuccess)
                                        te = hipMemcpy(&over, flag, sizeof(over), hipMemcpyDeviceToHost);
                                    if (te != hipSuccess) {
                                        (void)hipFree(tt);
                                        v1c_plan_destroy(p);
                                        return fail(V1C_E_HIP, std::string("tap table: ") + hipGetErrorString(te));
                                    }
                                    if (over == 0)
                                        p->allocs.push_back(tt), p->tap_table = tt, p->tap_table_bytes = tb;
                                    else
                                        (void)hipFree(tt);
                                } else {
                                    (void)hipGetLastError();
                                }
                                if (const char* dbg = tuning_env("V1C_DEBUG"); dbg && dbg[0] == '1')
                                    std::fprintf(stderr, "[v1c] tap table: %zu bytes, %s\n", tb, p->tap_table ? "in use" : "not kept");
                            }
                            std::vector<uint32_t> mrest1;
                            if (p->mirror_raw_nwp > 0 && tile_mirror_rest(hb.data(), hm.data(), g, p->half_dwords, g.dst_h, mrest1, p->mirror_raw_nwp, true, 1)) {
                                if ((rc = upload(p, mrest1, &p->mirror_rest1))) {
                                    v1c_plan_destroy(p);
                                    return rc;
                                }
                                p->n_mirror_rest1 = (int)mrest1.size();
                            }
                            if (const char* dbg = tuning_env("V1C_DEBUG"); dbg && dbg[0] == '1')
                                std::fprintf(stderr, "[v1c] mirror launch: seq buffers %d KB\n", p->mirror_seq_kb);
                        }
                        if (const char* dbg = tuning_env("V1C_DEBUG"); dbg && dbg[0] == '1')
                            std::fprintf(stderr, "[v1c] mirror pair launch: %s, %zu of %zu tiles left to the pair kernel (raw wave-passes %d)\n",
                                         p->mirror_boxes ? "yes" : "no", mrest.size(), hb.size() / 32, p->mirror_raw_nwp);
                    }
                }
                if (const char* dbg = tuning_env("V1C_DEBUG"); dbg && dbg[0] == '1') {
                    const int* bi = (const int*)hb.data();
                    const size_t nt = hb.size() / 32;
                    int hist[12] = {0};
                    for (size_t i = 0; i < nt; i++) {
                        const int cpr = bi[i * 8 + 2], nrows = bi[i * 8 + 3];
                        const int need = cpr > 0 ? nrows * (cpr * 4 + 4) : 0;
                        int k = 0;
                        while (k < 11 && need > (512 << k) / 2)
                            k++;
                        hist[k]++;
                    }
                    std::fprintf(stderr, "[v1c] tile boxes: %zu tiles, half_dwords=%d; need<=256:%d <=512:%d <=1k:%d <=2k:%d <=4k:%d <=8k:%d <=16k:%d more:%d\n",
                                 nt, p->half_dwords, hist[0], hist[1], hist[2], hist[3], hist[4], hist[5], hist[6], hist[7] + hist[8] + hist[9] + hist[10] + hist[11]);
                }
            }
        }
    }
    hipError_t e = hipDeviceSynchronize();
    if (e != hipSuccess) {
        v1c_plan_destroy(p);
        return fail(V1C_E_HIP, std::string("plan upload: ") + hipGetErrorString(e));
    }
    if (dbg_t)
        std::fprintf(stderr, "[v1c] plan_create: analysis + fits %.3f ms, tables / context / ring %.3f, tile boxes + sizing + rest list %.3f, mirror boxes + lists + sync %.3f\n",
                     t_fit - t_start, t_up - t_fit, t_boxes - t_up, now_ms() - t_boxes);
    *out = p;
    return V1C_OK;
}

#ifdef V1C_STAMPS
extern "C" int v1c_debug_read_stamps(v1c_plan* p, unsigned long long* out8)
{
    if (!p || !p->ctx.xmap)
        return V1C_E_INVALID;
    DeviceGuard dg(p->device);
    HIP_TRY(hipDeviceSynchronize());
    HIP_TRY(hipMemcpy(out8, p->ctx.xmap, 64, hipMemcpyDeviceToHost));
    HIP_TRY(hipMemset((void*)p->ctx.xmap, 0, 64));
    return V1C_OK;
}
#endif

extern "C" int64_t v1c_plan_tap_table_bytes(const v1c_plan* p)
{
    return p ? (int64_t)p->tap_table_bytes : 0;
}

extern "C" int v1c_plan_path(const v1c_plan* p)
{
    if (!p)
        return fail(V1C_E_INVALID, "plan is NULL");
    return p->mode == MODE_RAY ? (p->ana.base == 1 ? 2 : 1) : 0;
}

static int fill_unit(const v1c_plan* p, const v1c_unit& in, DevUnit& out)
{
    if (!in.src || !in.dst)
        return fail(V1C_E_INVALID, "unit src/dst is NULL");
    const Geom& g = p->ctx.g;
    const int eb = depth_bytes(p->depth);
    if (in.src_pitch < (int64_t)g.src_w * g.cn * eb || in.dst_pitch < (int64_t)g.dst_w * g.cn * eb)
        return fail(V1C_E_INVALID, "unit pitch smaller than a row");
    if (((uintptr_t)in.src | (uintptr_t)in.dst | (uint64_t)in.src_pitch | (uint64_t)in.dst_pitch) & (uint64_t)(eb - 1))
        return fail(V1C_E_INVALID, "unit pointers and pitches must be multiples of the pixel size");
    if (in.has_rot && !p->chain_has_rot)
        return fail(V1C_E_INVALID, "unit carries a rotation but the plan's chain has no rotate stage");
    out.src = in.src, out.dst = in.dst;
    out.src_pitch = in.src_pitch, out.dst_pitch = in.dst_pitch;
    out.has_rot = in.has_rot ? 1 : 0;
    out.pad = 0;
    const bool plan_rot = p->mode == MODE_RAY && p->ana.has_rot;
    for (int q = 0; q < 9; q++)
        out.rot[q] = in.has_rot ? in.rot[q] : (plan_rot ? p->ana.rot[q] : 0.0);
    return V1C_OK;
}

static UnitArgs unit_args(const DevUnit* du, int n)
{
    UnitArgs ua;
    std::memset(&ua, 0, sizeof(ua));
    std::memcpy(ua.u, du, sizeof(DevUnit) * (size_t)n);
    return ua;
}

struct LaunchPlan {
    bool any_rot = false;
    bool fast = false;
    bool need_fixup = false;
    bool shared_entry = false;
    bool mpoly_all = false;
    bool coords_bounded = false;
};

static LaunchPlan decide_launch(const v1c_plan* p, const DevUnit* du, int n, double r32_limit = 0)
{
    LaunchPlan d;
    for (int k = 0; k < n; k++)
        d.any_rot |= du[k].has_rot != 0;
    const Geom& g = p->ctx.g;
    d.fast = p->tile_boxes != nullptr && !p->disable_fast;
    for (int k = 0; k < n && d.fast; k++)
        d.fast = (uint64_t)g.src_h * (uint64_t)du[k].src_pitch < 0xFFFFFF00ull && du[k].src_pitch < (1 << 24) &&
                 (uint64_t)g.dst_h * (uint64_t)du[k].dst_pitch < 0xFFFFFF00ull && du[k].dst_pitch < (1 << 24);
    d.need_fixup = !(p->ray_no_rot_safe || p->ray_plan_rot_safe);
    d.shared_entry = p->plan_shared_entry;
    d.mpoly_all = d.any_rot && p->ctx.ray.radial_m != nullptr;
    d.coords_bounded = d.any_rot && p->front_hemisphere;
    if (d.any_rot) {
        d.need_fixup = !p->front_hemisphere;
        d.shared_entry = p->front_hemisphere;
        for (int k = 0; k < n && !d.need_fixup; k++) {
            const double* r = du[k].has_rot ? du[k].rot : p->ana.rot;
            const bool rotated = du[k].has_rot || p->ana.has_rot;
            const bool covered = rotated ? ray_reach_is_safe(p->table, rotated_reach(r)) : p->ray_no_rot_safe;
            d.need_fixup = !covered;
            if (d.coords_bounded) {
                const RayParams& rp = p->ctx.ray;
                const double gb = covered ? radial_table_g_bound(p->table, p->g_bounds, rotated ? rotated_reach(r) : p->m_reach_norot) : INFINITY;
                const double ax = r32_limit > 0 ? r32_limit : std::fabs(rp.rx32), ay = r32_limit > 0 ? r32_limit : std::fabs(rp.ry32);
                d.coords_bounded = gb * ax + std::fabs(rp.cx32) < 2097152.0 && gb * ay + std::fabs(rp.cy32) < 2097152.0;
            }
            d.shared_entry = d.shared_entry && covered &&
                             (rotated ? ray_entry_is_shared(p->table, rotated_reach(r), p->step) : p->plan_shared_entry);
            if (d.mpoly_all) {
                const double mr = rotated ? rotated_reach(r) : p->m_reach_norot;
                const double u_reach = (p->table.var_is_w ? std::sqrt(mr / 2) : mr) * (1 + 1e-9);
                d.mpoly_all = covered && std::min(p->table.n_int - 1, (int)(u_reach * p->table.inv_step) + 2) <= p->mp_valid_upto;
            }
        }
        d.shared_entry = d.shared_entry && !d.need_fixup;
        d.mpoly_all = d.mpoly_all && d.shared_entry;
        d.coords_bounded = d.coords_bounded && d.shared_entry;
    }
    return d;
}

static int ring_put(v1c_plan* p, hipStream_t st, const DevUnit* du, int n, const DevUnit** out, int* slot_out)
{
    hipStreamCaptureStatus cap = hipStreamCaptureStatusNone;
    if (hipStreamIsCapturing(st, &cap) != hipSuccess)
        cap = hipStreamCaptureStatusNone;
    int slot;
    if (cap != hipStreamCaptureStatusNone) {
        if (p->capture_next >= v1c_plan::kCaptureSlots)
            return fail(V1C_E_UNSUPPORTED, "too many graph-captured launches of more than 16 units for one plan (v1c_plan_release_captures "
                                           "hands the slots out again once their graphs are destroyed)");
        slot = v1c_plan::kRingSlots + p->capture_next++;
        *slot_out = -1;
    } else {
        slot = p->ring_next;
        p->ring_next = (p->ring_next + 1) % v1c_plan::kRingSlots;
        if (p->ring_used[slot] && p->ring_last[slot] != st)
            HIP_TRY(hipStreamWaitEvent(st, p->ring_ev[slot], 0));
        *slot_out = slot;
    }
    DevUnit* dst = p->ring + (size_t)slot * v1c_plan::kRingUnits;
    HIP_TRY(launch_put_units(dst, du, n, st));
    *out = dst;
    return V1C_OK;
}

static int ring_done(v1c_plan* p, hipStream_t st, int slot)
{
    if (slot < 0)
        return V1C_OK;
    HIP_TRY(hipEventRecord(p->ring_ev[slot], st));
    p->ring_last[slot] = st, p->ring_used[slot] = true;
    return V1C_OK;
}

extern "C" int v1c_plan_release_captures(v1c_plan* p)
{
    if (!p)
        return fail(V1C_E_INVALID, "plan is NULL");
    std::lock_guard<std::mutex> lk(p->ring_mu);
    p->capture_next = 0;
    return V1C_OK;
}

static int run_wide(v1c_plan* p, hipStream_t st, const DevUnit* du, int n_units)
{
    for (int base = 0; base < n_units;) {
        const int n = std::min(kMaxUnitsPerLaunch, n_units - base);
        const DevUnit* u = du + base;
        base += n;
        const UnitArgs ua = unit_args(u, n);
        int mode = MODE_LITERAL;
        bool need_fixup = false;
        if (p->mode == MODE_RAY) {
            const LaunchPlan d = decide_launch(p, u, n);
            if (!(d.any_rot && (p->n_rot_stages > 1 || p->gen_mode != 0)))
                mode = MODE_RAY, need_fixup = d.need_fixup;
        }
        if (!need_fixup) {
            HIP_TRY(launch_remap_wide(mode, p->depth, p->ctx, ua, p->wide, n, st));
            p->last_launch.store(V1C_LAUNCH_WIDE, std::memory_order_relaxed);
            continue;
        }
        std::lock_guard<std::mutex> flags_lk(p->flags_mu);
        hipStreamCaptureStatus cap = hipStreamCaptureStatusNone;
        if (hipStreamIsCapturing(st, &cap) != hipSuccess)
            cap = hipStreamCaptureStatusNone;
        const bool capturing = cap != hipStreamCaptureStatusNone;
        if (!capturing && p->flags_pending && p->flags_stream != st)
            HIP_TRY(hipStreamWaitEvent(st, p->flags_ev, 0));
        HIP_TRY(launch_remap_wide(MODE_RAY, p->depth, p->ctx, ua, p->wide, n, st));
        HIP_TRY(launch_remap_wide(MODE_FIXUP, p->depth, p->ctx, ua, p->wide, n, st));
        if (!capturing) {
            HIP_TRY(hipEventRecord(p->flags_ev, st));
            p->flags_stream = st, p->flags_pending = true;
        }
        p->last_launch.store(V1C_LAUNCH_WIDE | V1C_LAUNCH_FIXUP, std::memory_order_relaxed);
    }
    return V1C_OK;
}

extern "C" int v1c_plan_run(v1c_plan* p, void* stream, const v1c_unit* units, int n_units)
{
    if (!p || !units || n_units <= 0)
        return fail(V1C_E_INVALID, "v1c_plan_run: bad arguments");
    DeviceGuard dg(p->device);
    if (!dg.ok)
        return fail(V1C_E_NODEVICE, "hipSetDevice failed");
    hipStream_t st = (hipStream_t)stream;
    DevUnit du_small[kMaxUnitsPerLaunch];
    std::vector<DevUnit> du_big;
    DevUnit* du = du_small;
    if (n_units > kMaxUnitsPerLaunch) {
        du_big.resize((size_t)n_units);
        du = du_big.data();
    }
    for (int k = 0; k < n_units; k++) {
        int rc = fill_unit(p, units[k], du[k]);
        if (rc)
            return rc;
    }
    if (p->depth != V1C_DEPTH_8U)
        return run_wide(p, st, du, n_units);
    for (int base = 0; base < n_units;) {
        if (p->mode != MODE_RAY) {
            const int n = std::min(kMaxUnitsPerLaunch, n_units - base);
            HIP_TRY(launch_remap(MODE_LITERAL, p->ctx, unit_args(du + base, n), n, st));
            p->last_launch.store(V1C_LAUNCH_GENERIC, std::memory_order_relaxed);
            base += n;
            continue;
        }
        int n = std::min(v1c_plan::kRingUnits, n_units - base);
        LaunchPlan d = decide_launch(p, du + base, n);
        const bool literal = d.any_rot && (p->n_rot_stages > 1 || p->gen_mode != 0);
        if (n > kMaxUnitsPerLaunch && (literal || !d.fast || d.need_fixup || p->ctx.g.cn != 3)) {
            n = kMaxUnitsPerLaunch;
            d = decide_launch(p, du + base, n);
        }
        const DevUnit* u = du + base;
        base += n;
        if (literal) {
            HIP_TRY(launch_remap(MODE_LITERAL, p->ctx, unit_args(u, n), n, st));
            p->last_launch.store(V1C_LAUNCH_GENERIC, std::memory_order_relaxed);
            continue;
        }
        std::unique_lock<std::mutex> flags_lk(p->flags_mu, std::defer_lock);
        bool capturing = false;
        if (d.need_fixup) {
            flags_lk.lock();
            hipStreamCaptureStatus cap = hipStreamCaptureStatusNone;
            if (hipStreamIsCapturing(st, &cap) != hipSuccess)
                cap = hipStreamCaptureStatusNone;
            capturing = cap != hipStreamCaptureStatusNone;
            if (!capturing && p->flags_pending && p->flags_stream != st)
                HIP_TRY(hipStreamWaitEvent(st, p->flags_ev, 0));
        }
        uint32_t* flags = d.need_fixup ? p->ctx.tile_flags : nullptr;
        LaunchUnits lu{u, nullptr, n};
        int slot = -1;
        std::unique_lock<std::mutex> ring_lk(p->ring_mu, std::defer_lock);
        if (d.fast && n > kInlineUnits) {
            ring_lk.lock();
            int rc = ring_put(p, st, u, n, &lu.dev, &slot);
            if (rc)
                return rc;
        }
        const bool shared = d.shared_entry && !p->disable_shared_entry;
        bool aligned = true;
        for (int k = 0; k < n && aligned; k++)
            aligned = ((((uintptr_t)u[k].src) | (uintptr_t)u[k].src_pitch) & 3u) == 0;
        const bool mirror = d.fast && (n == 2 || (n == 1 && p->mirror_raw_nwp > 0 && p->n_mirror_rest1 >= 0)) && !d.any_rot &&
                            p->mirror_boxes != nullptr && shared && aligned;
        int kind = V1C_LAUNCH_GENERIC;
        if (mirror) {
            kind = V1C_LAUNCH_MIRROR;
            HIP_TRY(launch_ray_lin3_pair_mirror(p->ctx, p->ctx_dev, lu, flags, p->tile_boxes, p->mirror_raw_nwp > 0 ? p->mirror_pairs : p->mirror_boxes,
                                                p->half_dwords, p->mirror_h,
                                                n == 1 ? p->mirror_rest1 : p->mirror_rest, n == 1 ? p->n_mirror_rest1 : p->n_mirror_rest,
                                                p->mirror_raw_nwp, st, p->mirror_seq_kb, p->mirror_recs, n == 2 ? p->tap_table : nullptr));
        } else if (d.fast && p->ctx.g.cn != 3) {
            if (p->cn_kb > 0 && !d.any_rot && shared && aligned) {
                kind = V1C_LAUNCH_CN;
                HIP_TRY(launch_ray_lin_cn(p->ctx, p->ctx_dev, lu, flags, p->ana.has_rot, p->tile_boxes, p->cn_kb, st));
            } else if (d.any_rot && shared && aligned && cn_kernel_supports(p->ctx.g)) {
                kind = V1C_LAUNCH_CN_ROT;
                HIP_TRY(launch_ray_lin_cn(p->ctx, p->ctx_dev, lu, flags, true, nullptr, 12, st));
            } else {
                HIP_TRY(launch_remap(MODE_RAY, p->ctx, unit_args(u, n), n, st));
            }
        } else if (d.fast) {
            kind = V1C_LAUNCH_TILE;
            HIP_TRY(launch_ray_lin3_tile(p->ctx, p->ctx_dev, lu, flags, d.any_rot || p->ana.has_rot, d.any_rot ? nullptr : p->tile_boxes,
                                         p->half_dwords, shared, d.mpoly_all && !p->disable_mpoly, d.any_rot ? nullptr : p->rest_list, p->n_rest,
                                         p->lean_half, p->strip_len, p->lean_raw_nwp, st, d.coords_bounded && !p->disable_coords_bounded, &kind));
        } else {
            HIP_TRY(launch_remap(MODE_RAY, p->ctx, unit_args(u, n), n, st));
        }
        if (slot >= 0) {
            int rc = ring_done(p, st, slot);
            if (rc)
                return rc;
        }
        if (ring_lk.owns_lock())
            ring_lk.unlock();
        p->last_launch.store(kind | (d.need_fixup ? V1C_LAUNCH_FIXUP : 0), std::memory_order_relaxed);
        if (d.need_fixup) {
            HIP_TRY(launch_remap(MODE_FIXUP, p->ctx, unit_args(u, n), n, st));
            if (!capturing) {
                HIP_TRY(hipEventRecord(p->flags_ev, st));
                p->flags_stream = st, p->flags_pending = true;
            }
        }
    }
    return V1C_OK;
}

static int run_auto(v1c_plan* p, void* stream, const v1c_unit* units, int n_units, const double* rad_dev, int n_rad, int threshold)
{
    if (!p || !units || n_units <= 0 || (rad_dev && n_rad <= 0))
        return fail(V1C_E_INVALID, "v1c_plan_run_auto: bad arguments");
    if (n_units > kInlineUnits)
        return fail(V1C_E_UNSUPPORTED, "v1c_plan_run_auto: at most 16 units per call");
    if (p->depth != V1C_DEPTH_8U)
        return fail(V1C_E_UNSUPPORTED, "v1c_plan_run_auto: 8-bit images only (16-bit / float32: take the radius to the host)");
    if (p->mode != MODE_RAY || p->gen_mode != 0 || p->ana.base != 0 || p->n_rot_stages > 1 || p->disable_fast)
        return fail(V1C_E_UNSUPPORTED, "v1c_plan_run_auto: chains of the form EquirectangularEncoder() * [one rotation] * radial stages only");
    if (p->ctx.ray.rx != p->ctx.ray.ry)
        return fail(V1C_E_UNSUPPORTED, "v1c_plan_run_auto: the plan's Denormalize scale must be isotropic (rx == ry)");
    DeviceGuard dg(p->device);
    if (!dg.ok)
        return fail(V1C_E_NODEVICE, "hipSetDevice failed");
    hipStream_t st = (hipStream_t)stream;
    const Geom& g = p->ctx.g;
    DevUnit du[kInlineUnits];
    bool aligned = true;
    for (int k = 0; k < n_units; k++) {
        int rc = fill_unit(p, units[k], du[k]);
        if (rc)
            return rc;
        if (!du[k].has_rot && !p->ana.has_rot)
            for (int q = 0; q < 9; q++)
                du[k].rot[q] = (q % 4 == 0) ? 1.0 : 0.0;
        du[k].has_rot = 1;
        aligned = aligned && ((((uintptr_t)du[k].src) | (uintptr_t)du[k].src_pitch) & 3u) == 0;
    }
    bool same_rot = true;
    for (int k = 1; k < n_units && same_rot; k++)
        same_rot = std::memcmp(du[k].rot, du[0].rot, sizeof(du[0].rot)) == 0;
    const double r_limit = 4.0 * (double)std::max(g.src_h, g.src_w);
    const LaunchPlan d = decide_launch(p, du, n_units, 32.0 * r_limit);
    if (!d.fast || d.need_fixup)
        return fail(V1C_E_UNSUPPORTED, "v1c_plan_run_auto: this chain needs a fix-up pass (or 64-bit offsets): use the radius on the host");
    const bool shared = d.shared_entry && !p->disable_shared_entry;
    if (g.cn != 3 && !(shared && aligned && cn_kernel_supports(g)))
        return fail(V1C_E_UNSUPPORTED, "v1c_plan_run_auto: grayscale / BGRA need dword-aligned sources and one table entry per lane");
    std::lock_guard<std::mutex> lk(p->dyn_mu);
    if (!p->ctx_dyn)
        return fail(V1C_E_UNSUPPORTED, "v1c_plan_run_auto: the plan has no tile kernels");
    hipStreamCaptureStatus cap = hipStreamCaptureStatusNone;
    if (hipStreamIsCapturing(st, &cap) != hipSuccess)
        cap = hipStreamCaptureStatusNone;
    const bool capturing = cap != hipStreamCaptureStatusNone;
    if (!capturing && p->dyn_pending && p->dyn_stream != st)
        HIP_TRY(hipStreamWaitEvent(st, p->dyn_ev, 0));
    if (rad_dev) {
        HIP_TRY(launch_patch_radius(p->ctx_dyn, rad_dev, n_rad, r_limit, p->ctx.ray.cx32, p->ctx.ray.cy32, st));
    } else {
        AutoLines im;
        std::memset(&im, 0, sizeof(im));
        const bool use_row = g.src_w > g.src_h;
        for (int k = 0; k < n_units; k++)
            im.line[k] = use_row ? du[k].src + (int64_t)(g.src_h / 2) * du[k].src_pitch : du[k].src + (int64_t)(g.src_w / 2) * g.cn;
        im.n = use_row ? g.src_w : g.src_h, im.cn = g.cn, im.threshold = threshold, im.count = n_units;
        for (int k = 0; k < n_units; k++)
            im.step[k] = use_row ? (int64_t)g.cn : du[k].src_pitch;
        HIP_TRY(launch_auto_radius(p->ctx_dyn, p->auto_scratch, im, r_limit, p->ctx.ray.cx32, p->ctx.ray.cy32, st));
    }
    LaunchUnits lu{du, nullptr, n_units};
    int kind = V1C_LAUNCH_GENERIC;
    if (g.cn != 3) {
        kind = V1C_LAUNCH_CN_ROT;
        HIP_TRY(launch_ray_lin_cn(p->ctx, p->ctx_dyn, lu, nullptr, true, nullptr, 12, st));
    } else {
        kind = V1C_LAUNCH_TILE;
        HIP_TRY(launch_ray_lin3_tile(p->ctx, p->ctx_dyn, lu, nullptr, true, nullptr, p->half_dwords, shared, d.mpoly_all && !p->disable_mpoly, nullptr, 0,
                                     p->lean_half, p->strip_len, p->lean_raw_nwp, st, d.coords_bounded && !p->disable_coords_bounded, &kind, same_rot));
    }
    if (!capturing) {
        HIP_TRY(hipEventRecord(p->dyn_ev, st));
        p->dyn_stream = st, p->dyn_pending = true;
    }
    p->last_launch.store(kind, std::memory_order_relaxed);
    return V1C_OK;
}

extern "C" int v1c_plan_run_auto(v1c_plan* p, void* stream, const v1c_unit* units, int n_units, const double* rad_dev, int n_rad)
{
    if (!rad_dev)
        return fail(V1C_E_INVALID, "v1c_plan_run_auto: bad arguments");
    return run_auto(p, stream, units, n_units, rad_dev, n_rad, 0);
}

extern "C" int v1c_plan_run_auto_images(v1c_plan* p, void* stream, const v1c_unit* units, int n_units, int threshold)
{
    return run_auto(p, stream, units, n_units, nullptr, 0, threshold);
}

extern "C" int v1c_plan_get_map(v1c_plan* p, void* stream, float* xmap, float* ymap, int64_t map_pitch,
                                const double* rot_or_null)
{
    if (!p || !xmap || !ymap)
        return fail(V1C_E_INVALID, "v1c_plan_get_map: bad arguments");
    if (map_pitch < (int64_t)p->ctx.g.dst_w * 4 || (map_pitch & 3))
        return fail(V1C_E_INVALID, "map_pitch too small or not a multiple of 4");
    if (rot_or_null && !p->chain_has_rot)
        return fail(V1C_E_INVALID, "rotation given but the plan's chain has no rotate stage");
    DeviceGuard dg(p->device);
    if (!dg.ok)
        return fail(V1C_E_NODEVICE, "hipSetDevice failed");
    UnitArgs ua;
    std::memset(&ua, 0, sizeof(ua));
    int mode = p->mode;
    if (rot_or_null) {
        ua.u[0].has_rot = 1;
        for (int q = 0; q < 9; q++)
            ua.u[0].rot[q] = rot_or_null[q];
        if (p->n_rot_stages > 1 || p->gen_mode != 0)
            mode = MODE_LITERAL;
    }
    HIP_TRY(launch_get_map(mode, p->ctx, ua, xmap, ymap, map_pitch, (hipStream_t)stream));
    return V1C_OK;
}
// ... 232 lines not shown
```

vr180_convert_amd/csrc/tap_table.hpp:

```cpp
#pragma once
#include <cstdint>

#if !defined(__HIPCC__) && !defined(__host__)
#define __host__
#define __device__
#define V1C_TAP_TABLE_OWN_QUALIFIERS
#endif

namespace v1c {

constexpr int kTapPX = 4;
constexpr int kTapEntryBytes = 12;
constexpr int kTapBaseMax = 4095;
constexpr int kTapDxMax = 127;
constexpr int kTapDyMin = -32, kTapDyMax = 31;

struct TapEntry {
    uint32_t w[3];
};
static_assert(sizeof(TapEntry) == kTapEntryBytes, "three dwords per lane");

struct TapCoords {
    int x[kTapPX], y[kTapPX], y2[kTapPX];
};

__host__ __device__ inline bool tap_entry_fits(const TapCoords& c)
{
    bool ok = c.x[0] >= 0 && c.x[0] <= kTapBaseMax && c.y[0] >= 0 && c.y[0] <= kTapBaseMax && c.y2[0] >= 0 && c.y2[0] <= kTapBaseMax;
    for (int k = 1; k < kTapPX; k++) {
        const int dx = c.x[k] - c.x[k - 1], dy = c.y[k] - c.y[k - 1], dy2 = c.y2[k] - c.y2[k - 1];
        ok = ok && dx >= 0 && dx <= kTapDxMax && dy >= kTapDyMin && dy <= kTapDyMax && dy2 >= kTapDyMin && dy2 <= kTapDyMax;
    }
    return ok;
}

__host__ __device__ inline TapEntry tap_entry_encode(const TapCoords& c)
{
    const uint32_t dx1 = (uint32_t)(c.x[1] - c.x[0]) & 127u, dx2 = (uint32_t)(c.x[2] - c.x[1]) & 127u, dx3 = (uint32_t)(c.x[3] - c.x[2]) & 127u;
    TapEntry e;
    e.w[0] = ((uint32_t)c.x[0] & 4095u) | dx1 << 12 | dx2 << 19 | (dx3 & 63u) << 26;
    e.w[1] = ((uint32_t)c.y[0] & 4095u) | ((uint32_t)(c.y[1] - c.y[0]) & 63u) << 12 | ((uint32_t)(c.y[2] - c.y[1]) & 63u) << 18 |
             ((uint32_t)(c.y[3] - c.y[2]) & 63u) << 24 | (dx3 >> 6) << 30;
    e.w[2] = ((uint32_t)c.y2[0] & 4095u) | ((uint32_t)(c.y2[1] - c.y2[0]) & 63u) << 12 | ((uint32_t)(c.y2[2] - c.y2[1]) & 63u) << 18 |
             ((uint32_t)(c.y2[3] - c.y2[2]) & 63u) << 24;
    return e;
}

__host__ __device__ inline int tap_sext6(uint32_t w, int pos)
{
    return (int)(w << (26 - pos)) >> 26;
}

__host__ __device__ inline TapCoords tap_entry_decode(const TapEntry& e)
{
    TapCoords c;
    c.x[0] = (int)(e.w[0] & 4095u);
    c.x[1] = c.x[0] + (int)((e.w[0] >> 12) & 127u);
    c.x[2] = c.x[1] + (int)((e.w[0] >> 19) & 127u);
    c.x[3] = c.x[2] + (int)((e.w[0] >> 26) | ((e.w[1] >> 30) & 1u) << 6);
    c.y[0] = (int)(e.w[1] & 4095u), c.y2[0] = (int)(e.w[2] & 4095u);
    for (int k = 1; k < kTapPX; k++) {
        c.y[k] = c.y[k - 1] + tap_sext6(e.w[1], 6 + 6 * k);
        c.y2[k] = c.y2[k - 1] + tap_sext6(e.w[2], 6 + 6 * k);
    }
    return c;
}

}

#ifdef V1C_TAP_TABLE_OWN_QUALIFIERS
#undef __host__
#undef __device__
#undef V1C_TAP_TABLE_OWN_QUALIFIERS
#endif
```

vr180_convert_amd/csrc/tile_device.hpp:

```cpp
#pragma once

#include <algorithm>
#include <cstddef>
#include <cstdlib>
#include <cstring>

#include "kernels.hpp"
#include "tap_table.hpp"

#ifndef V1C_PRIO
#define V1C_PRIO 15
#endif

namespace v1c {


#ifndef V1C_TILE_W
#define V1C_TILE_W 64
#endif
#define V1C_CONST __attribute__((address_space(4)))
typedef const V1C_CONST KernelCtx& ctx_cref;
typedef const V1C_CONST Geom& geom_cref;
typedef const V1C_CONST RayParams& ray_cref;
typedef const V1C_CONST DevUnit* units_cptr;
// ... 1431 lines not shown
__device__ __forceinline__ void rot_shared_pair_tile(args_cref a, int zA, int zB, int btx, int bty, int* red, uint32_t* boxw, WPtr wtab)
{
    constexpr int NT = 256;
    ctx_cref c = args_ctx(a);
    const units_cptr U = args_units(a);
    geom_cref g = c.g;
    ray_cref P = c.ray;
    const int tid = threadIdx.x;
    const TileIds t = tile_ids(g, zA, tid, btx, bty, gridDim.x, NT / kLanesX);
    RowCol rc;
    load_rowcol<1>(P, t.xc, t.jc, rc);
    const int ext = kxk_ext(g);
    LaneCoords L;
    lane_coords<VAR_W, 1, K, OWN, 0, 0, 0, NN>(c, U[zA].rot, rc, t.npx, P.radial, 0, P.n_int, L, ext);
    const TileBox b = reduce_box<K, NT / 64>(L, red, tid);
    const uint8_t* __restrict__ srcA = U[zA].src;
    const uint8_t* __restrict__ srcB = U[zB].src;
    const uint32_t pitchA = (uint32_t)U[zA].src_pitch, pitchB = (uint32_t)U[zB].src_pitch;
    const bool fits = box_fits(b, srcA, pitchA, 4 * NT, kBoxBytes / 4) & box_fits(b, srcB, pitchB, 4 * NT, kBoxBytes / 4);
    if (!fits) {
        uint32_t px[kPX] = {0, 0, 0, 0};
        patch_and_store<K, NN>(c, U, zA, t, L, px, 0u, srcA);
        patch_and_store<K, NN>(c, U, zB, t, L, px, 0u, srcB);
        return;
    }
    ChunkMap M;
    make_chunk_map<NT>(b, tid, M);
    Staged SA, SB;
    if (ext && box_leaves_source(b, g)) {
        stage_load_ext<true>(M, srcA, pitchA, g, SA);
        stage_load_ext<true>(M, srcB, pitchB, g, SB);
    } else {
        stage_load<true, true>(M, srcA, pitchA, (uint32_t)(g.src_h - 1) * pitchA + (uint32_t)g.src_w * 3u, SA);
        stage_load<true, true>(M, srcB, pitchB, (uint32_t)(g.src_h - 1) * pitchB + (uint32_t)g.src_w * 3u, SB);
    }
    stage_store_pair(M, SA, SB, boxw);
    __syncthreads();
    if (L.ok != (1u << t.npx) - 1)
        if (uint32_t* flags = a.tile_flags) {
            flags[t.flag_tile] = 1;
            flags[t.flag_tile + (zB - zA) * t.flag_stride] = 1;
        }
    uint32_t pa[kPX], pb[kPX];
    kxk_pair_gather<K>(tid, L, b, boxw, boxw + 2 * (kBoxBytes / 4) + 4, wtab, pa, pb);
    patch_and_store<K, NN>(c, U, zA, t, L, pa, L.inside, srcA);
    patch_and_store<K, NN>(c, U, zB, t, L, pb, L.inside, srcB);
}

__host__ __device__ inline bool mirror_box_ok(int x0, int y0, int cpr, int nrows, int half_dwords, int src_h, int src_w)
{
    return cpr > 0 && cpr <= kMaxCpr && nrows * cpr <= 1024 && nrows * (cpr * 4 + 4) <= half_dwords &&
           !((y0 + nrows >= src_h) && (x0 + 4 * cpr > src_w));
}

__host__ __device__ inline bool mirror_static_ok(const TileBox& b, const TileBox& q, int half_dwords, int src_h, int src_w)
{
    return b.interior != 0 && q.interior == b.interior && b.nidx > 0 && b.nidx <= kTabSlice && q.idx0 == b.idx0 && q.nidx == b.nidx &&
           mirror_box_ok(b.x0, b.y0, b.cpr, b.nrows, half_dwords, src_h, src_w) &&
           mirror_box_ok(q.x0, q.y0, q.cpr, q.nrows, half_dwords, src_h, src_w);
}

constexpr int kRawMaxWavePasses = 16;
__host__ __device__ inline int raw_units_per_row(int cpr)
{
    return (3 * cpr + 3) >> 2;
}
__host__ __device__ inline bool raw_box_ok(int x0, int y0, int cpr, int nrows, int nwp, int src_h, int src_w)
{
    const int upr = raw_units_per_row(cpr);
    return cpr > 0 && cpr <= kMaxCpr && nrows * upr <= nwp * 64 && !((y0 + nrows >= src_h) && (x0 * 3 + upr * 16 > src_w * 3));
}
__host__ __device__ inline int mirror_raw_fit(const TileBox& b, const TileBox& q, int nwp, int src_h, int src_w)
{
    if (!(b.interior != 0 && q.interior == b.interior && b.nidx > 0 && b.nidx <= kTabSlice && q.nidx > 0 && q.idx0 >= b.idx0 &&
          q.idx0 + q.nidx <= b.idx0 + b.nidx))
        return 0;
    if (raw_box_ok(b.x0, b.y0, b.cpr, b.nrows, nwp, src_h, src_w) && raw_box_ok(q.x0, q.y0, q.cpr, q.nrows, nwp, src_h, src_w))
        return 1;
    if (raw_box_ok(b.x0, b.y0, b.cpr, b.nrows, 2 * nwp, src_h, src_w) && raw_box_ok(q.x0, q.y0, q.cpr, q.nrows, 2 * nwp, src_h, src_w))
        return 2;
    return 0;
}
__host__ __device__ inline bool mirror_raw_static_ok(const TileBox& b, const TileBox& q, int nwp, int src_h, int src_w)
{
    return b.interior != 0 && q.interior == b.interior && b.nidx > 0 && b.nidx <= kTabSlice && q.idx0 == b.idx0 && q.nidx == b.nidx &&
           raw_box_ok(b.x0, b.y0, b.cpr, b.nrows, nwp, src_h, src_w) && raw_box_ok(q.x0, q.y0, q.cpr, q.nrows, nwp, src_h, src_w);
}

typedef __attribute__((address_space(3))) void* lds_void_ptr;
typedef const __attribute__((address_space(1))) void* glb_void_ptr;

struct RawLanes {
    uint32_t row_l, col16;
    int R, upr;
};

__device__ __forceinline__ RawLanes raw_lanes_upr(int upr, int lane)
{
    RawLanes m;
    m.upr = upr;
    const float rupr = __builtin_amdgcn_rcpf((float)m.upr);
    m.R = __builtin_amdgcn_readfirstlane((int)(64.5f * rupr));
    m.row_l = (uint32_t)(((float)lane + 0.5f) * rupr);
    m.col16 = ((uint32_t)lane - __umul24(m.row_l, (uint32_t)m.upr)) * 16u;
    return m;
}

__device__ __forceinline__ RawLanes raw_lanes(int cpr, int lane)
{
    return raw_lanes_upr(raw_units_per_row(cpr), lane);
}

template <int BPP = 3>
__device__ __forceinline__ int raw_box_dma(const TileBox& b, const RawLanes& m, const uint8_t* __restrict__ src, uint32_t spitch, int lane,
                                            int wave, uint32_t lds_box)
{
    const uint32_t sp = (uint32_t)__builtin_amdgcn_readfirstlane((int)spitch);
    uint32_t voff;
    asm("v_mul_u32_u24 %0, %1, %2" : "=v"(voff) : "v"(m.row_l), "s"(sp));
    voff += m.col16;
    const int rows = min(m.R, b.nrows);
    const int last0 = b.nrows - rows;
    const bool active = lane < rows * m.upr;
    const uint64_t org = (uint64_t)(uintptr_t)src + (uint64_t)((uint32_t)b.y0 * sp + (uint32_t)b.x0 * (uint32_t)BPP);
    const uint32_t lpitch = (uint32_t)m.upr * 16u;
    int n = 0;
    for (int r0 = wave * m.R; r0 < b.nrows; r0 += 4 * m.R) {
        const int rs = min(r0, last0);
        const uint64_t base = org + (uint64_t)((uint32_t)rs * sp);
        const uint32_t m0v = lds_box + (uint32_t)rs * lpitch;
        uint32_t m0_saved;
        if (active)
            asm volatile("s_mov_b32 %0, m0\n\ts_mov_b32 m0, %3\n\ts_nop 2\n\tglobal_load_lds_dwordx4 %1, %2\n\ts_mov_b32 m0, %0"
                         : "=&s"(m0_saved)
                         : "v"(voff), "s"(base), "s"(m0v)
                         : "memory");
        n++;
    }
    return n;
}

constexpr uint32_t kRoundBias = 0x4B400000u;
constexpr uint32_t kMirrorRecMpoly = 1u, kMirrorRecFitSeq = 2u, kMirrorRecFitOne = 4u;
struct MirrorRecBox {
    int y0, x3;
    int nrows, last0;
    int upr, R, nact;
    uint32_t magic, lpitch, tapk;
};
struct MirrorRec {
    MirrorRecBox b, q;
    int idx0, nidx;
    uint32_t flags;
};
struct MirrorRecWords {
    uint32_t w[16];
};
static_assert(sizeof(MirrorRecWords) == 2 * sizeof(TileBox), "one record per (tile box, band box) slot");

__host__ __device__ inline uint32_t mul24_lo(uint32_t a, uint32_t b)
{
    return (uint32_t)((uint64_t)(a & 0xFFFFFFu) * (uint64_t)(b & 0xFFFFFFu));
}
__host__ __device__ inline uint32_t mirror_rec_lane_row(uint32_t lane, uint32_t magic)
{
    return mul24_lo(lane, magic) >> 16;
}
__host__ __device__ inline uint32_t mirror_rec_tap(uint32_t bx, uint32_t by, uint32_t lpitch, uint32_t tapk)
{
    return mul24_lo(by >> 5, lpitch) + (bx >> 5) * 3u + tapk;
}
__host__ __device__ inline bool mirror_rec_box(const TileBox& t, MirrorRecBox& r, uint32_t (&w)[5])
{
    const bool ok = t.cpr > 0 && t.cpr <= kMaxCpr && t.nrows >= 0 && t.nrows < 2048 && t.x0 >= 0 && t.y0 >= 0 && t.x0 < 32768 && t.y0 < 32768;
    r = MirrorRecBox{0, 0, 0, 0, 1, 1, 0, 65536u, 16u, 0u};
    if (ok) {
        r.upr = raw_units_per_row(t.cpr);
        r.R = 64 / r.upr;
        r.y0 = t.y0, r.x3 = 3 * t.x0, r.nrows = t.nrows;
        const int rows = r.R < t.nrows ? r.R : t.nrows;
        r.last0 = t.nrows - rows, r.nact = rows * r.upr;
        r.magic = (65536u + (uint32_t)r.upr - 1u) / (uint32_t)r.upr;
        r.lpitch = (uint32_t)r.upr * 16u;
        r.tapk = 0u - (((uint32_t)t.y0 + (0xFFFFFFu & (kRoundBias >> 5))) * r.lpitch + 3u * ((uint32_t)t.x0 + (kRoundBias >> 5)));
    }
    w[0] = (uint32_t)r.y0 | (uint32_t)r.nrows << 16;
    w[1] = (uint32_t)r.x3 | (uint32_t)r.last0 << 20;
    w[2] = (uint32_t)r.upr | (uint32_t)r.R << 8 | (uint32_t)r.nact << 16;
    w[3] = r.magic;
    w[4] = r.tapk;
    return ok;
}
__host__ __device__ inline MirrorRecBox mirror_rec_unbox(uint32_t w0, uint32_t w1, uint32_t w2, uint32_t w3, uint32_t w4)
{
    MirrorRecBox r;
    r.y0 = (int)(w0 & 0xffffu), r.nrows = (int)(w0 >> 16);
    r.x3 = (int)(w1 & 0xfffffu), r.last0 = (int)(w1 >> 20);
    r.upr = (int)(w2 & 0xffu), r.R = (int)((w2 >> 8) & 0xffu), r.nact = (int)(w2 >> 16);
    r.magic = w3, r.lpitch = (w2 & 0xffu) * 16u, r.tapk = w4;
    return r;
}
__host__ __device__ inline MirrorRecWords mirror_rec_encode(const TileBox& b, const TileBox& q, int seq_kb, int one_kb, int src_h, int src_w)
{
    MirrorRecWords o;
    MirrorRecBox rb, rq;
    uint32_t wb[5], wq[5];
    const bool okb = mirror_rec_box(b, rb, wb), okq = mirror_rec_box(q, rq, wq);
    for (int k = 0; k < 5; k++)
        o.w[k] = wb[k], o.w[5 + k] = wq[k];
    const bool ok = okb && okq && b.idx0 >= 0;
    const bool fit_seq = ok && seq_kb > 0 && mirror_raw_fit(b, q, seq_kb, src_h, src_w) == 1;
    const bool fit_one = ok && one_kb > 0 && mirror_raw_fit(b, q, one_kb, src_h, src_w) == 1;
    const bool fit = fit_seq || fit_one;
    o.w[10] = fit ? (uint32_t)b.idx0 : 0u;
    o.w[11] = (fit ? (uint32_t)b.nidx : 1u) |
              (((b.interior & 2) ? kMirrorRecMpoly : 0u) | (fit_seq ? kMirrorRecFitSeq : 0u) | (fit_one ? kMirrorRecFitOne : 0u)) << 16;
    o.w[12] = o.w[13] = o.w[14] = o.w[15] = 0u;
    return o;
}
__host__ __device__ inline MirrorRec mirror_rec_decode(const MirrorRecWords& v)
{
    MirrorRec r;
    r.b = mirror_rec_unbox(v.w[0], v.w[1], v.w[2], v.w[3], v.w[4]);
    r.q = mirror_rec_unbox(v.w[5], v.w[6], v.w[7], v.w[8], v.w[9]);
    r.idx0 = (int)v.w[10], r.nidx = (int)(v.w[11] & 0xffffu), r.flags = v.w[11] >> 16;
    return r;
}
__device__ __forceinline__ MirrorRec load_mirror_rec(const TileBox* pairs, int tile)
{
    typedef uint32_t __attribute__((ext_vector_type(16))) u32x16;
    const u32x16 v = *(const V1C_CONST u32x16*)(pairs + 2 * __builtin_amdgcn_readfirstlane(tile));
    MirrorRecWords o;
#pragma unroll
    for (int k = 0; k < 16; k++)
        o.w[k] = v[k];
    return mirror_rec_decode(o);
}

__device__ __forceinline__ uint32_t mul24_vs(uint32_t v, uint32_t s)
{
    uint32_t r;
    asm("v_mul_u32_u24 %0, %1, %2" : "=v"(r) : "v"(v), "s"(s));
    return r;
}
__device__ __forceinline__ uint32_t mad24_vsv(uint32_t v, uint32_t s, uint32_t add)
{
    uint32_t r;
    asm("v_mad_u32_u24 %0, %1, %2, %3" : "=v"(r) : "v"(v), "s"(s), "v"(add));
    return r;
}

__device__ __forceinline__ RawLanes rec_lanes(const MirrorRecBox& r, int lane)
{
    RawLanes m;
    m.upr = r.upr, m.R = r.R;
    m.row_l = mul24_vs((uint32_t)lane, r.magic) >> 16;
    m.col16 = ((uint32_t)lane - mul24_vs(m.row_l, (uint32_t)r.upr)) * 16u;
    return m;
}
__device__ __forceinline__ int rec_box_dma(const MirrorRecBox& r, const RawLanes& m, const uint8_t* __restrict__ src, uint32_t spitch, int lane,
                                            int wave, uint32_t lds_box)
{
    const uint32_t sp = (uint32_t)__builtin_amdgcn_readfirstlane((int)spitch);
    const uint32_t voff = mul24_vs(m.row_l, sp) + m.col16;
    const bool active = lane < r.nact;
    const uint64_t org = (uint64_t)(uintptr_t)src + (uint64_t)((uint32_t)r.y0 * sp + (uint32_t)r.x3);
    int n = 0;
    for (int r0 = wave * r.R; r0 < r.nrows; r0 += 4 * r.R) {
        const int rs = min(r0, r.last0);
        const uint64_t base = org + (uint64_t)((uint32_t)rs * sp);
        const uint32_t m0v = lds_box + (uint32_t)rs * r.lpitch;
        uint32_t m0_saved;
        if (active)
            asm volatile("s_mov_b32 %0, m0\n\ts_mov_b32 m0, %3\n\ts_nop 2\n\tglobal_load_lds_dwordx4 %1, %2\n\ts_mov_b32 m0, %0"
                         : "=&s"(m0_saved)
                         : "v"(voff), "s"(base), "s"(m0v)
                         : "memory");
        n++;
    }
    return n;
}

#define V1C_WAIT_BLOCK(i, extra) "s_waitcnt vmcnt(" #i ")" extra "\n\ts_barrier\n\ts_branch 1f\n\ts_nop 0\n\t"
#define V1C_WAIT_TABLE(extra)                                                                                                      \
    V1C_WAIT_BLOCK(0, extra) V1C_WAIT_BLOCK(1, extra) V1C_WAIT_BLOCK(2, extra) V1C_WAIT_BLOCK(3, extra) V1C_WAIT_BLOCK(4, extra)    \
    V1C_WAIT_BLOCK(5, extra) V1C_WAIT_BLOCK(6, extra) V1C_WAIT_BLOCK(7, extra) V1C_WAIT_BLOCK(8, extra) V1C_WAIT_BLOCK(9, extra)    \
    V1C_WAIT_BLOCK(10, extra) V1C_WAIT_BLOCK(11, extra) V1C_WAIT_BLOCK(12, extra) V1C_WAIT_BLOCK(13, extra)                         \
    V1C_WAIT_BLOCK(14, extra) V1C_WAIT_BLOCK(15, extra) V1C_WAIT_BLOCK(16, extra) V1C_WAIT_BLOCK(17, extra)                         \
    V1C_WAIT_BLOCK(18, extra) V1C_WAIT_BLOCK(19, extra) V1C_WAIT_BLOCK(20, extra)
#define V1C_WAIT_JUMP(extra)                                                                                                       \
    uint32_t off_;                                                                                                                 \
    asm volatile("s_getpc_b64 vcc\n\t"                                               \
                 "s_lshl_b32 %0, %1, 4\n\t"                                                         \
                 "s_add_u32 %0, %0, 20\n\t"                                       \
                 "s_add_u32 vcc_lo, vcc_lo, %0\n\t"                                                                              \
                 "s_addc_u32 vcc_hi, vcc_hi, 0\n\t"                                                                              \
                 "s_setpc_b64 vcc\n\t" V1C_WAIT_TABLE(extra) "1:"                                                                \
                 : "=&s"(off_)                                                                                                     \
                 : "s"(__builtin_amdgcn_readfirstlane((int)min((uint32_t)max(n, 0), 20u)))                                                                            \
                 : "vcc", "scc", "memory")

__device__ __forceinline__ void wait_vm_barrier(int n)
{
    V1C_WAIT_JUMP("");
}

template <int N>
__device__ __forceinline__ void wait_vm_barrier_imm()
{
    static_assert(N >= 0 && N <= 2, "add the case");
    if (N == 0)
        asm volatile("s_waitcnt vmcnt(0)\n\ts_barrier" ::: "memory");
    else if (N == 1)
        asm volatile("s_waitcnt vmcnt(1)\n\ts_barrier" ::: "memory");
    else
        asm volatile("s_waitcnt vmcnt(2)\n\ts_barrier" ::: "memory");
}

__device__ __forceinline__ void gather_pair_raw(const TileBox& b, uint32_t raw, uint32_t eye_off, const int (&sx)[kPX], const int (&sy)[kPX],
                                                uint32_t (&pix0)[kPX], uint32_t (&pix1)[kPX])
{
    const uint32_t pitch = (uint32_t)raw_units_per_row(b.cpr) * 16u;
    const uint32_t base0 = raw - ((uint32_t)b.y0 * pitch + (uint32_t)b.x0 * 3u);
#pragma unroll
    for (int k = 0; k < kPX; k++) {
        const uint32_t ix = (uint32_t)sx[k] >> 5;
        const uint32_t a = __umul24((uint32_t)(sy[k] >> 5), pitch) + (ix * 2u + ix) + base0;
        const uint32_t d = a & ~3u;
        const lds_u32_ptr r0 = (lds_u32_ptr)(uintptr_t)d, r1 = (lds_u32_ptr)(uintptr_t)(d + pitch);
        const lds_u32_ptr s0 = (lds_u32_ptr)(uintptr_t)(d + eye_off), s1 = (lds_u32_ptr)(uintptr_t)(d + pitch + eye_off);
        const uint32_t a0 = r0[0], a1 = r0[1], a2 = r0[2], b0 = r1[0], b1 = r1[1], b2 = r1[2];
        const uint32_t c0 = s0[0], c1 = s0[1], c2 = s0[2], e0 = s1[0], e1 = s1[1], e2 = s1[2];
        const BlendW w = blend_weights(sx[k], sy[k]);
        pix0[k] = blend3<3>(__builtin_amdgcn_alignbyte(a1, a0, a), __builtin_amdgcn_alignbyte(a2, a1, a), __builtin_amdgcn_alignbyte(b1, b0, a),
                            __builtin_amdgcn_alignbyte(b2, b1, a), w);
        pix1[k] = blend3<3>(__builtin_amdgcn_alignbyte(c1, c0, a), __builtin_amdgcn_alignbyte(c2, c1, a), __builtin_amdgcn_alignbyte(e1, e0, a),
                            __builtin_amdgcn_alignbyte(e2, e1, a), w);
    }
}

__device__ __forceinline__ void store_pair_row(units_cptr U, const TileIds& t, int j, const uint32_t (&pix0)[kPX], const uint32_t (&pix1)[kPX])
{
    const uint32_t row_off = (uint32_t)t.x0 * 3u;
    store4<1>(U[0].dst + (__umul24((uint32_t)j, (uint32_t)U[0].dst_pitch) + row_off), pix0, 0xFu, dst_rows_dword_aligned(U, 0));
    store4<1>(U[1].dst + (__umul24((uint32_t)j, (uint32_t)U[1].dst_pitch) + row_off), pix1, 0xFu, dst_rows_dword_aligned(U, 1));
}

__device__ __forceinline__ void gather_one_raw(const TileBox& b, uint32_t raw, const int (&sx)[kPX], const int (&sy)[kPX], uint32_t (&pix)[kPX])
{
    const uint32_t pitch = (uint32_t)raw_units_per_row(b.cpr) * 16u;
    const uint32_t base0 = raw - ((uint32_t)b.y0 * pitch + (uint32_t)b.x0 * 3u);
#pragma unroll
    for (int k = 0; k < kPX; k++) {
        const uint32_t ix = (uint32_t)sx[k] >> 5;
        const uint32_t a = __umul24((uint32_t)(sy[k] >> 5), pitch) + (ix * 2u + ix) + base0;
        const uint32_t d = a & ~3u;
        const lds_u32_ptr r0 = (lds_u32_ptr)(uintptr_t)d, r1 = (lds_u32_ptr)(uintptr_t)(d + pitch);
        const uint32_t a0 = r0[0], a1 = r0[1], a2 = r0[2], b0 = r1[0], b1 = r1[1], b2 = r1[2];
        pix[k] = blend3<3>(__builtin_amdgcn_alignbyte(a1, a0, a), __builtin_amdgcn_alignbyte(a2, a1, a), __builtin_amdgcn_alignbyte(b1, b0, a),
                           __builtin_amdgcn_alignbyte(b2, b1, a), blend_weights(sx[k], sy[k]));
    }
}

__device__ __forceinline__ void gather_one_rec(const MirrorRecBox& r, uint32_t raw, const int (&bx)[kPX], const int (&by)[kPX], uint32_t (&pix)[kPX])
{
    const uint32_t kb = r.tapk + raw;
#pragma unroll
    for (int k = 0; k < kPX; k++) {
        const uint32_t ix = (uint32_t)bx[k] >> 5;
        const uint32_t a = mad24_vsv((uint32_t)by[k] >> 5, r.lpitch, ix * 2u + ix + kb);
        const uint32_t d = a & ~3u;
        const lds_u32_ptr r0 = (lds_u32_ptr)(uintptr_t)d, r1 = (lds_u32_ptr)(uintptr_t)(d + r.lpitch);
        const uint32_t a0 = r0[0], a1 = r0[1], a2 = r0[2], b0 = r1[0], b1 = r1[1], b2 = r1[2];
        pix[k] = blend3<3>(__builtin_amdgcn_alignbyte(a1, a0, a), __builtin_amdgcn_alignbyte(a2, a1, a), __builtin_amdgcn_alignbyte(b1, b0, a),
                           __builtin_amdgcn_alignbyte(b2, b1, a), blend_weights(bx[k], by[k]));
    }
}

// ... 42 lines not shown
```

vr180_convert_amd/remapper.py:

```python
from __future__ import annotations

import ctypes as C
import threading
import time
from collections import OrderedDict
import logging
from logging import getLogger
from pathlib import Path
from typing import Any, Literal, Sequence

import numpy as np
import torch
from numpy.typing import NDArray

from . import _abi, _hostpipe, _io, _native
from .chain import NotLowerable, TransformerBase, denormalize_center, get_radius, lower_for_get_map
from .chain import DenormalizeTransformer, NormalizeTransformer

LOG = getLogger(__name__)

INTER_LANCZOS4 = _abi.INTER_LANCZOS4
BORDER_CONSTANT = _abi.BORDER_CONSTANT


def _device(device: Any = None) -> torch.device:
    if not torch.cuda.is_available():
        raise _native.EngineUnavailable(
            "no HIP device visible: vr180_convert_amd runs the remap on an MI355X and has no CPU fallback"
        )
    if device is None:
        return torch.device("cuda", torch.cuda.current_device())
    d = torch.device(device)
    if d.type != "cuda":
        raise ValueError("device must be a cuda (HIP) device")
    return torch.device("cuda", d.index if d.index is not None else torch.cuda.current_device())


try:
    _raw_stream = torch._C._cuda_getCurrentRawStream
except AttributeError:
    _raw_stream = None


def _stream_ptr(dev: torch.device) -> int:
    if _raw_stream is not None and dev.index is not None:
        return int(_raw_stream(dev.index))
    return int(torch.cuda.current_stream(dev).cuda_stream)


def border_scalar(value: Any) -> np.ndarray:
    vals = [value] if np.isscalar(value) else list(value)
    out = np.zeros(4, np.uint8)
    for i, v in enumerate(vals[:4]):
        out[i] = int(min(255, max(0, np.rint(float(v)))))
    return out


def border_scalar_f64(value: Any) -> np.ndarray:
    vals = [value] if np.isscalar(value) else list(value)
    out = np.zeros(4, np.float64)
    for i, v in enumerate(vals[:4]):
        out[i] = float(v)
    return out


DEPTHS = {torch.uint8: _abi.DEPTH_8U, torch.uint16: _abi.DEPTH_16U, torch.float32: _abi.DEPTH_32F}
NP_DTYPES = (np.uint8, np.uint16, np.float32)


def _border_key(value: Any, dtype: torch.dtype) -> bytes:
    return border_scalar(value).tobytes() if dtype == torch.uint8 else border_scalar_f64(value).tobytes()


def _check_image_tensor(t: torch.Tensor, what: str) -> None:
    if t.dtype not in DEPTHS or t.dim() != 3:
        raise TypeError(f"{what} must be a uint8, uint16 or float32 (H, W, C) tensor")
    cn = t.shape[2]
    if (cn > 1 and t.stride(2) != 1) or (t.shape[1] > 1 and t.stride(1) != cn) or (
        t.shape[0] > 1 and t.stride(0) < t.shape[1] * cn
    ):
        raise ValueError(f"{what}: pixels must be contiguous within a row (column-sliced views are fine)")


def marshal_units(srcs: Sequence[torch.Tensor], dsts: Sequence[torch.Tensor], rots: Sequence[Any] | None, *,
                  src_hw: tuple[int, int], dst_wh: tuple[int, int], cn: int, device: torch.device | None,
                  dtype: torch.dtype | None = None):
    n = len(srcs)
    units = (_abi.Unit * n)()
    for k, (s, d) in enumerate(zip(srcs, dsts)):
        _check_image_tensor(s, "src")
        _check_image_tensor(d, "dst")
        if s.dtype != d.dtype or (dtype is not None and s.dtype != dtype):
            raise TypeError(f"unit {k}: src {s.dtype} / dst {d.dtype}: source and destination must both have the plan's pixel type"
                            + ("" if dtype is None else f" ({dtype})"))
        if tuple(s.shape) != (*src_hw, cn) or tuple(d.shape) != (dst_wh[1], dst_wh[0], cn):
            raise ValueError(f"unit {k}: tensor shapes {tuple(s.shape)} -> {tuple(d.shape)} do not match the plan")
        if device is not None and (s.device != device or d.device != device):
            raise ValueError(f"unit {k}: tensors must live on {device}")
        units[k].src, units[k].dst = s.data_ptr(), d.data_ptr()
        units[k].src_pitch, units[k].dst_pitch = s.stride(0) * s.element_size(), d.stride(0) * d.element_size()
        if rots is not None and rots[k] is not None:
            m = np.asarray(rots[k], dtype=np.float64).reshape(9)
            units[k].has_rot = 1
            for q in range(9):
                units[k].rot[q] = m[q]
    return units


class Plan:

    def __init__(self, chain: _abi.Chain, *, src_hw, dst_wh, cn, interpolation, border_mode, border_value, device,
                 dtype: torch.dtype = torch.uint8):
        self.device = _device(device)
        self.src_hw, self.dst_wh, self.cn = tuple(src_hw), tuple(dst_wh), int(cn)
        if dtype not in DEPTHS:
            raise TypeError(f"pixel type {dtype}: uint8, uint16 or float32 only (cv2.remap's CV_8U / CV_16U / CV_32F)")
        self.dtype = dtype
        self._h = C.c_void_p()
        self._memo: "OrderedDict[tuple, Any]" = OrderedDict()
        t0 = time.perf_counter()
        if dtype == torch.uint8:
            bv = border_scalar(border_value)
            rc = _native.lib().v1c_plan_create(
                C.byref(self._h), self.device.index, C.byref(chain), src_hw[0], src_hw[1], dst_wh[1], dst_wh[0],
                cn, int(interpolation), int(border_mode), bv.ctypes.data,
            )
            _native.check(rc, "v1c_plan_create")
        else:
            bv = border_scalar_f64(border_value)
            rc = _native.lib().v1c_plan_create_ex(
                C.byref(self._h), self.device.index, C.byref(chain), src_hw[0], src_hw[1], dst_wh[1], dst_wh[0],
                cn, DEPTHS[dtype], int(interpolation), int(border_mode), bv.ctypes.data,
            )
            _native.check(rc, "v1c_plan_create_ex")
        self.create_ms = (time.perf_counter() - t0) * 1e3

    @property
    def path(self) -> str:
        return {1: "ray", 2: "planar"}.get(_native.lib().v1c_plan_path(self._h), "literal")

    def last_launch(self) -> str:
        k = _native.lib().v1c_plan_last_launch(self._h)
        if k < 0:
            return ""
        return _abi.LAUNCH_NAMES.get(k & 0xFF, "?") + ("+fixup" if k & _abi.LAUNCH_FIXUP else "")

    def tap_table_bytes(self) -> int:
        f = getattr(_native.lib(), "v1c_plan_tap_table_bytes", None)
        return int(f(self._h)) if f is not None else 0

    def run(self, srcs: Sequence[torch.Tensor], dsts: Sequence[torch.Tensor], rots: Sequence[Any] | None = None) -> None:
        n = len(srcs)
        if n == 0 or len(dsts) != n or (rots is not None and len(rots) != n):
            raise ValueError("srcs / dsts / rots lengths differ or are empty")
        sig = None
        if rots is None:
            try:
                sig = tuple((s.data_ptr(), s.stride(), s.shape, s.dtype, d.data_ptr(), d.stride(), d.shape, d.dtype) for s, d in zip(srcs, dsts))
            except AttributeError:
                sig = None
            units = self._memo.get(sig) if sig is not None else None
            if units is not None:
                rc = _native.lib().v1c_plan_run(self._h, _stream_ptr(self.device), units, n)
                _native.check(rc, "v1c_plan_run")
                return
        units = marshal_units(srcs, dsts, rots, src_hw=self.src_hw, dst_wh=self.dst_wh, cn=self.cn, device=self.device, dtype=self.dtype)
        rc = _native.lib().v1c_plan_run(self._h, _stream_ptr(self.device), units, n)
        _native.check(rc, "v1c_plan_run")
        if sig is not None:
            self._memo[sig] = units
            while len(self._memo) > 64:
                try:
                    self._memo.popitem(last=False)
                except KeyError:
                    break

    def run_auto(self, srcs: Sequence[torch.Tensor], dsts: Sequence[torch.Tensor], rad: torch.Tensor | None = None,
                 rots: Sequence[Any] | None = None, threshold: int = 10) -> None:
        units = marshal_units(srcs, dsts, rots, src_hw=self.src_hw, dst_wh=self.dst_wh, cn=self.cn, device=self.device, dtype=self.dtype)
        if rad is None:
            rc = _native.lib().v1c_plan_run_auto_images(self._h, _stream_ptr(self.device), units, len(srcs), int(threshold))
            _native.check(rc, "v1c_plan_run_auto_images")
            return
        if rad.dtype != torch.float64 or rad.dim() != 2 or rad.shape[1] != 2 or not rad.is_contiguous() or rad.device != self.device:
            raise ValueError("rad must be a contiguous float64 (n, 2) tensor on the plan's device")
        rc = _native.lib().v1c_plan_run_auto(self._h, _stream_ptr(self.device), units, len(srcs), rad.data_ptr(), int(rad.shape[0]))
        _native.check(rc, "v1c_plan_run_auto")

    def run_units(self, units: Any, n: int) -> None:
        rc = _native.lib().v1c_plan_run(self._h, _stream_ptr(self.device), units, int(n))
        _native.check(rc, "v1c_plan_run")

    def release_captures(self) -> None:
        _native.check(_native.lib().v1c_plan_release_captures(self._h), "v1c_plan_release_captures")

    def get_map(self, rot: Any = None) -> tuple[torch.Tensor, torch.Tensor]:
        w, h = self.dst_wh
        xm = torch.empty((h, w), dtype=torch.float32, device=self.device)
        ym = torch.empty((h, w), dtype=torch.float32, device=self.device)
        r = None if rot is None else np.ascontiguousarray(np.asarray(rot, np.float64).reshape(9))
        rc = _native.lib().v1c_plan_get_map(
            self._h, _stream_ptr(self.device), xm.data_ptr(), ym.data_ptr(), xm.stride(0) * 4,
            None if r is None else r.ctypes.data,
        )
        _native.check(rc, "v1c_plan_get_map")
        return xm, ym

    def __del__(self):
        try:
            if self._h:
                _native.lib().v1c_plan_destroy(self._h)
                self._h = C.c_void_p()
        except Exception:
            pass


_PLANS: "OrderedDict[tuple, Plan]" = OrderedDict()
_PLAN_CACHE_SIZE = 32
_PLANS_LOCK = threading.Lock()


_AUTO_LAST: dict = {}
_TLS = threading.local()


class _LutLaunch:

    @staticmethod
    def last_launch() -> str:
        return "lut"


def last_launch_kinds() -> list[str]:
    return [p.last_launch() for p in getattr(_TLS, "plans", [])]


def last_tap_table_bytes() -> list[int]:
    return [p.tap_table_bytes() if isinstance(p, Plan) else 0 for p in getattr(_TLS, "plans", [])]


def last_auto_radius_form() -> str:
    return getattr(_TLS, "auto_form", "")


def clear_caches() -> None:
    with _PLANS_LOCK:
        _PLANS.clear()
        _LOWERED.clear()
        _LAST_SHARED[0] = None
        _AUTO_LAST.clear()
    import sys

    ca = sys.modules.get(__package__ + ".chromatic")
    if ca is not None:
        ca.clear_caches()


def _plan_for(chain: _abi.Chain, *, src_hw, dst_wh, cn, interpolation, border_mode, border_value, device,
              dtype: torch.dtype = torch.uint8) -> Plan:
    dev = _device(device)
    key = (chain.key(), tuple(src_hw), tuple(dst_wh), cn, int(interpolation), int(border_mode),
           _border_key(border_value, dtype), dev.index, dtype)
    with _PLANS_LOCK:
        plan = _PLANS.get(key)
        if plan is not None:
            _PLANS.move_to_end(key)
            return plan
    plan = Plan(chain, src_hw=src_hw, dst_wh=dst_wh, cn=cn, interpolation=interpolation,
                border_mode=border_mode, border_value=border_value, device=dev, dtype=dtype)
    with _PLANS_LOCK:
        plan = _PLANS.setdefault(key, plan)
        _PLANS.move_to_end(key)
        while len(_PLANS) > _PLAN_CACHE_SIZE:
            _PLANS.popitem(last=False)
    return plan


def _split_single_rotation(chain: _abi.Chain) -> tuple[_abi.Chain, np.ndarray | None]:
    idx = [i for i in range(chain.n_ops) if chain.ops[i].opcode == _abi.OP_ROTATE]
    if len(idx) != 1:
        return chain, None
    i = idx[0]
    rot = np.array(chain.ops[i].p[:9], dtype=np.float64)
    blank = _abi.Chain.from_buffer_copy(bytes(chain))
    for q in range(9):
        blank.ops[i].p[q] = 1.0 if q in (0, 4, 8) else 0.0
    return blank, rot


def _host_map(transformer: TransformerBase, *, radius, size_input, size_output, center=None):
    xmap, ymap = np.meshgrid(np.arange(size_output[0]), np.arange(size_output[1]))
    full = (
        NormalizeTransformer()
        * transformer
        * DenormalizeTransformer(scale=(radius, radius), center=denormalize_center(size_input, center))
    )
    xmap, ymap = full.transform(xmap, ymap)
    return xmap.astype(np.float32), ymap.astype(np.float32)


_LOWERED: "OrderedDict[tuple, _abi.Chain]" = OrderedDict()
_LAST_SHARED: list = [None]


class _NoKey(Exception):
    """The transformer holds state the memo key cannot capture exactly: lower it on every call."""


_FIELD_NAMES: dict = {}


def _param_key(obj: Any):
    t = type(obj)
    if t is float:
        return ("f", obj.hex())
    if t is int:
        return ("i", obj)
    if obj is None or t is bool or t is str or t is bytes:
        return obj
    names = _FIELD_NAMES.get(t, 0)
    if names == 0:
        import dataclasses

        if dataclasses.is_dataclass(t):
            names = tuple(f.name for f in dataclasses.fields(t)) if t.__module__ == TransformerBase.__module__ else None
        else:
            names = False
        _FIELD_NAMES[t] = names
    if names is None:
        raise _NoKey
    if names is not False:
        return (t.__name__, tuple([_param_key(getattr(obj, n)) for n in names]))
    if isinstance(obj, (bool, str, bytes)):
        return obj
    if isinstance(obj, (int, np.integer)):
        return ("i", int(obj))
    if isinstance(obj, (float, np.floating)):
        return ("f", float(obj).hex())
    if isinstance(obj, np.ndarray):
        if obj.dtype == object:
            raise _NoKey
        a = np.ascontiguousarray(obj)
        return ("nd", a.dtype.str, a.shape, a.tobytes())
    if isinstance(obj, (list, tuple)):
        return (t.__name__, tuple([_param_key(v) for v in obj]))
    if all(hasattr(obj, c) for c in "wxyz"):
        return ("q", tuple(float(getattr(obj, c)).hex() for c in "wxyz"))
    raise _NoKey


def _transformer_key(t: Any):
    try:
        return _param_key(t)
    except (_NoKey, TypeError, ValueError):
        return None


def _lower_cached(t: TransformerBase, *, radius, size_input, size_output, center=None) -> _abi.Chain:
    k = _transformer_key(t)
    if k is None:
        return lower_for_get_map(t, radius=radius, size_input=size_input, size_output=size_output, center=center)
    key = (k, float(radius).hex(), tuple(size_input), tuple(size_output))
    if center is not None:
        key += (("center", float(center[0]).hex(), float(center[1]).hex()),)
    with _PLANS_LOCK:
        ch = _LOWERED.get(key)
    if ch is None:
        ch = lower_for_get_map(t, radius=radius, size_input=size_input, size_output=size_output, center=center)
        with _PLANS_LOCK:
            _LOWERED[key] = ch
            while len(_LOWERED) > 64:
                _LOWERED.popitem(last=False)
    return ch


def remap_tensors(
    transformer: TransformerBase | Sequence[TransformerBase],
    srcs: Sequence[torch.Tensor],
    dsts: Sequence[torch.Tensor],
    *,
    radius: float,
    interpolation: int = INTER_LANCZOS4,
    boarder_mode: int = BORDER_CONSTANT,
    boarder_value: Any = 0,
    size_input: tuple[int, int] | None = None,
    rotations: Sequence[Any] | None = None,
    center: Any = None,
    chromatic: Any = None,
) -> list[str]:
    n = len(srcs)
    if n == 0:
# ... 736 lines not shown
```

Before: 761,500 Mpixels/s.

## Add compact 8-byte tap table entries with delta encoding for mirror seq kernel

Adds a compact 8-byte-per-lane tap table format that stores each source coordinate as a base, a first delta and second-order deltas, and reconstructs the mirrored y2 coordinates from a per-tile constant K kept in the mirror record. Large tables (over 8 MiB at 12 bytes per entry) default to the compact form, and a templated kernel variant decodes it from LDS. The aim is to cut the HBM traffic and LDS footprint of the precomputed tap table in exchange for extra decode ALU work. If any entry does not fit the narrow fields, the table is discarded and the slower path is used.

New measurement: 774,000 Mpixels/s (median of 6 runs). About the same (+1.6%).

```diff
diff --git a/include/vr180_remap.h b/include/vr180_remap.h
--- a/include/vr180_remap.h
+++ b/include/vr180_remap.h
@@ -132,6 +132,7 @@
 int v1c_plan_last_launch(const v1c_plan* plan);
 
 int64_t v1c_plan_tap_table_bytes(const v1c_plan* plan);
+int v1c_plan_tap_entry_bytes(const v1c_plan* plan);
 
 int v1c_plan_get_map(v1c_plan* plan, void* stream, float* xmap, float* ymap,
                      int64_t map_pitch, const double* rot_or_null);
diff --git a/vr180_convert_amd/_native.py b/vr180_convert_amd/_native.py
--- a/vr180_convert_amd/_native.py
+++ b/vr180_convert_amd/_native.py
@@ -25,7 +25,7 @@
     "v1c_jpeg_compose_bound", "v1c_jpeg_compose_check", "v1c_jpeg_header_xf", "v1c_jpeg_compose",
     "v1c_fit_circle_workspace", "v1c_fit_circle_async", "v1c_fit_circle",
     "v1c_color_match_workspace", "v1c_color_match_luts_async", "v1c_apply_luts_async",
-    "v1c_plan_tap_table_bytes",
+    "v1c_plan_tap_table_bytes", "v1c_plan_tap_entry_bytes",
     "v1c_ca_plan_create", "v1c_ca_plan_run", "v1c_ca_plan_get_map", "v1c_ca_plan_path", "v1c_ca_plan_last_launch", "v1c_ca_plan_destroy",
 ]
 
@@ -166,6 +166,11 @@
         L.v1c_plan_tap_table_bytes.restype = i64
     except AttributeError:
         pass
+    try:
+        L.v1c_plan_tap_entry_bytes.argtypes = [vp]
+        L.v1c_plan_tap_entry_bytes.restype = i32
+    except AttributeError:
+        pass
     L.v1c_plan_run.argtypes = [vp, vp, C.POINTER(_abi.Unit), i32]
     L.v1c_plan_get_map.argtypes = [vp, vp, vp, vp, i64, vp]
     L.v1c_remap_fused.argtypes = [i32, vp, vp, i32, i32, i64, i32, vp, i32, i32, i64, C.POINTER(_abi.Chain), i32, i32, vp]
diff --git a/vr180_convert_amd/csrc/kernels.hpp b/vr180_convert_amd/csrc/kernels.hpp
--- a/vr180_convert_amd/csrc/kernels.hpp
+++ b/vr180_convert_amd/csrc/kernels.hpp
@@ -78,10 +78,14 @@
 int tile_mirror_raw_passes(const void* host_boxes, const void* host_mboxes, const Geom& g, int permille = 980, int max_kb = 12);
 hipError_t launch_ray_lin3_pair_mirror(const KernelCtx& c, const KernelCtx* cdev, const LaunchUnits& lu, uint32_t* flags, const void* boxes,
                                        const void* mboxes, int half_dwords, int mirror_h, const uint32_t* rest_list, int n_rest, int raw_nwp,
-                                       hipStream_t stream, int seq_kb, const void* recs = nullptr, const void* tap_table = nullptr);
-size_t tap_table_bytes(const Geom& g);
-hipError_t launch_fill_tap_table(const KernelCtx& c, const KernelCtx* cdev, const void* boxes, const void* mboxes, void* table, uint32_t* overflow);
-void tile_mirror_records(const void* host_boxes, const void* host_mboxes, size_t n_tiles, const Geom& g, int seq_kb, int one_kb, std::vector<char>& out);
+                                       hipStream_t stream, int seq_kb, const void* recs = nullptr, const void* tap_table = nullptr,
+                                       int tap_entry_bytes = 12);
+size_t tap_table_bytes(const Geom& g, int entry_bytes = 12);
+int tap_table_s(const KernelCtx& c);
+hipError_t launch_fill_tap_table(const KernelCtx& c, const KernelCtx* cdev, const void* boxes, const void* mboxes, void* table, uint32_t* overflow,
+                                 int entry_bytes = 12);
+void tile_mirror_records(const void* host_boxes, const void* host_mboxes, size_t n_tiles, const Geom& g, int seq_kb, int one_kb, std::vector<char>& out,
+                         int tap_s = 0);
 int tile_half_dwords(const void* host_boxes, size_t n_tiles, int max_chunks, bool occupancy_classes);
 hipError_t launch_ray_lin3_tile(const KernelCtx& c, const KernelCtx* cdev, const LaunchUnits& lu, uint32_t* flags, bool use_rot, const void* boxes,
                                 int half_dwords, bool shared_entry, bool mpoly_all, const uint32_t* rest_list, int n_rest, int lean_half,
diff --git a/vr180_convert_amd/csrc/kernels_mirror.hip b/vr180_convert_amd/csrc/kernels_mirror.hip
--- a/vr180_convert_amd/csrc/kernels_mirror.hip
+++ b/vr180_convert_amd/csrc/kernels_mirror.hip
@@ -1,3 +1,5 @@
+#include <cmath>
+
 #include "tile_device.hpp"
 
 namespace v1c {
@@ -380,12 +382,12 @@
 }
 #endif
 
-constexpr int kTapSliceBytes = 256 * kTapEntryBytes;
-__global__ __launch_bounds__(256) __attribute__((amdgpu_waves_per_eu(V1C_SEQ_WAVES + 1, 8))) void k_ray_lin3_pair_mirror_seq_tab(V1C_MIRROR_HEAD, TileArgs a_)
-{
+constexpr int kTapSliceBytes = 256 * kTapEntryBytes, kTap8SliceBytes = 256 * kTap8EntryBytes;
+template <int EB>
+__device__ __forceinline__ void mirror_seq_tab_tile(V1C_MIRROR_HEAD, uint32_t* tapw, uint32_t* dyn_box)
+{
+    static_assert(EB == kTapEntryBytes || EB == kTap8EntryBytes, "the 12-byte entry or the compact one");
     constexpr int NT = 256;
-    __shared__ __attribute__((aligned(16))) uint32_t tapw[kTapSliceBytes / 4];
-    extern __shared__ __attribute__((aligned(16))) uint32_t dyn_box[];
     if (V1C_PRIO & 4)
         __builtin_amdgcn_s_setprio(3);
     args_cref a = kernel_args<kMirrorHeadBytes>();
@@ -412,10 +414,10 @@
     const uint32_t raw_b = (uint32_t)(uintptr_t)(lds_u32_ptr)dyn_box, raw_q = raw_b + (uint32_t)cap_kb * 1024u;
     const int wave = __builtin_amdgcn_readfirstlane(tid >> 6), lane = tid & 63;
     {
-        const uint32_t wave_off = (uint32_t)__builtin_amdgcn_readfirstlane(tid & ~63) * (uint32_t)kTapEntryBytes;
-        const uint8_t* gp = (const uint8_t*)rowcol_tables + ((size_t)(uint32_t)__builtin_amdgcn_readfirstlane(t.box_tile) * (size_t)kTapSliceBytes + wave_off) +
+        const uint32_t wave_off = (uint32_t)__builtin_amdgcn_readfirstlane(tid & ~63) * (uint32_t)EB;
+        const uint8_t* gp = (const uint8_t*)rowcol_tables + ((size_t)(uint32_t)__builtin_amdgcn_readfirstlane(t.box_tile) * (size_t)(256 * EB) + wave_off) +
                             (uint32_t)lane * 16u;
-        if (lane < 64 * kTapEntryBytes / 16)
+        if (lane < 64 * EB / 16)
             __builtin_amdgcn_global_load_lds((glb_void_ptr)gp, (lds_void_ptr)(uintptr_t)(lds_tap + wave_off), 16, 0, 0);
     }
     const RawLanes mb = rec_lanes(r.b, lane), mq = rec_lanes(r.q, lane);
@@ -433,8 +435,16 @@
     uint32_t ta_b[kPX], ta_q[kPX];
     BlendW W_b[kPX], W_q[kPX];
     {
-        const lds_u32_ptr ep = (lds_u32_ptr)(uintptr_t)(lds_tap + (uint32_t)tid * (uint32_t)kTapEntryBytes);
-        const TapCoords tc = tap_entry_decode(TapEntry{{ep[0], ep[1], ep[2]}});
+        TapCoords tc;
+        if constexpr (EB == kTap8EntryBytes) {
+            typedef uint32_t __attribute__((ext_vector_type(2))) u32x2;
+            typedef const __attribute__((address_space(3))) u32x2* lds_u64_ptr;
+            const u32x2 ev = *(lds_u64_ptr)(uintptr_t)(lds_tap + (uint32_t)tid * (uint32_t)EB);
+            tc = tap8_decode(TapEntry8{{ev.x, ev.y}}, r.tap_k);
+        } else {
+            const lds_u32_ptr ep = (lds_u32_ptr)(uintptr_t)(lds_tap + (uint32_t)tid * (uint32_t)EB);
+            tc = tap_entry_decode(TapEntry{{ep[0], ep[1], ep[2]}});
+        }
         const uint32_t kb = raw_b, kq = raw_q + (uint32_t)(r.b.x3 - r.q.x3);
 #pragma unroll
         for (int k = 0; k < kPX; k++) {
@@ -469,9 +479,22 @@
         store4<1>(udst[1] + drow(1, jm), pix, 0xFu, ualigned[1]);
 }
 
+__global__ __launch_bounds__(256) __attribute__((amdgpu_waves_per_eu(V1C_SEQ_WAVES + 1, 8))) void k_ray_lin3_pair_mirror_seq_tab(V1C_MIRROR_HEAD, TileArgs a_)
+{
+    __shared__ __attribute__((aligned(16))) uint32_t tapw[kTapSliceBytes / 4];
+    extern __shared__ __attribute__((aligned(16))) uint32_t dyn_box[];
+    mirror_seq_tab_tile<kTapEntryBytes>(pairs, tiles_x_magic, gx_rest, rows_strip, dst_wh, rowcol_tables, ctxp, kb_mh, tapw, dyn_box);
+}
+__global__ __launch_bounds__(256) __attribute__((amdgpu_waves_per_eu(V1C_SEQ_WAVES + 1, 8))) void k_ray_lin3_pair_mirror_seq_tab8(V1C_MIRROR_HEAD, TileArgs a_)
+{
+    __shared__ __attribute__((aligned(16))) uint32_t tapw[kTap8SliceBytes / 4];
+    extern __shared__ __attribute__((aligned(16))) uint32_t dyn_box[];
+    mirror_seq_tab_tile<kTap8EntryBytes>(pairs, tiles_x_magic, gx_rest, rows_strip, dst_wh, rowcol_tables, ctxp, kb_mh, tapw, dyn_box);
+}
+
 template <int VAR_W>
 __global__ __launch_bounds__(256) void k_fill_tap_table(const KernelCtx* ctxp, const TileBox* __restrict__ boxes, const TileBox* __restrict__ mboxes,
-                                                        int tiles_x, uint32_t* __restrict__ table, uint32_t* overflow)
+                                                        int tiles_x, uint32_t* __restrict__ table, uint32_t* overflow, int entry_bytes, int tap_s)
 {
     ctx_cref c = *(const V1C_CONST KernelCtx*)ctxp;
     ray_cref P = c.ray;
@@ -495,27 +518,49 @@
         tc.y[k] = (int)((uint32_t)L.sy[k] - kRoundBias) - 32 * b.y0;
         tc.y2[k] = (int)((uint32_t)L.sy2[k] - kRoundBias) - 32 * q.y0;
     }
+    const size_t at = (size_t)t.box_tile * 256u + (size_t)tid;
+    if (entry_bytes == kTap8EntryBytes) {
+        const int K = tap_s - 32 * (b.y0 + q.y0);
+        if (!tap8_fits(tc, K))
+            atomicOr(overflow, 1u);
+        const TapEntry8 e = tap8_encode(tc, K);
+        uint32_t* out = table + at * 2u;
+        out[0] = e.w[0], out[1] = e.w[1];
+        return;
+    }
     if (!tap_entry_fits(tc))
         atomicOr(overflow, 1u);
     const TapEntry e = tap_entry_encode(tc);
-    uint32_t* out = table + ((size_t)t.box_tile * 256u + (size_t)tid) * 3u;
+    uint32_t* out = table + at * 3u;
     out[0] = e.w[0], out[1] = e.w[1], out[2] = e.w[2];
 }
 
-size_t tap_table_bytes(const Geom& g)
+size_t tap_table_bytes(const Geom& g, int entry_bytes)
 {
     const dim3 full = tile_grid(g, 256, 1);
-    return (size_t)full.x * (size_t)(full.y / 2 + 1) * (size_t)kTapSliceBytes;
-}
-
-hipError_t launch_fill_tap_table(const KernelCtx& c, const KernelCtx* cdev, const void* boxes, const void* mboxes, void* table, uint32_t* overflow)
-{
+    return (size_t)full.x * (size_t)(full.y / 2 + 1) * 256u * (size_t)entry_bytes;
+}
+
+int tap_table_s(const KernelCtx& c)
+{
+    const double s = 2.0 * c.ray.cy32;
+    return std::fabs(s) < 1.0e9 ? (int)std::llrint(s) : 0;
+}
+
+hipError_t launch_fill_tap_table(const KernelCtx& c, const KernelCtx* cdev, const void* boxes, const void* mboxes, void* table, uint32_t* overflow,
+                                 int entry_bytes)
+{
+    if (entry_bytes != kTapEntryBytes && entry_bytes != kTap8EntryBytes)
+        return hipErrorInvalidValue;
     const dim3 full = tile_grid(c.g, 256, 1);
     const dim3 grid(full.x, full.y / 2 + 1, 1), block(256, 1, 1);
+    const int tap_s = tap_table_s(c);
     if (c.ray.var_is_w)
-        hipLaunchKernelGGL((k_fill_tap_table<1>), grid, block, 0, 0, cdev, (const TileBox*)boxes, (const TileBox*)mboxes, (int)full.x, (uint32_t*)table, overflow);
+        hipLaunchKernelGGL((k_fill_tap_table<1>), grid, block, 0, 0, cdev, (const TileBox*)boxes, (const TileBox*)mboxes, (int)full.x, (uint32_t*)table, overflow,
+                           entry_bytes, tap_s);
     else
-        hipLaunchKernelGGL((k_fill_tap_table<0>), grid, block, 0, 0, cdev, (const TileBox*)boxes, (const TileBox*)mboxes, (int)full.x, (uint32_t*)table, overflow);
+        hipLaunchKernelGGL((k_fill_tap_table<0>), grid, block, 0, 0, cdev, (const TileBox*)boxes, (const TileBox*)mboxes, (int)full.x, (uint32_t*)table, overflow,
+                           entry_bytes, tap_s);
     return hipGetLastError();
 }
 
@@ -589,20 +634,21 @@
     return rest.size() <= (size_t)d.x * (TYh - 1) && rest.size() * 4 <= (size_t)d.x * d.y;
 }
 
-void tile_mirror_records(const void* host_boxes, const void* host_mboxes, size_t n_tiles, const Geom& g, int seq_kb, int one_kb, std::vector<char>& out)
+void tile_mirror_records(const void* host_boxes, const void* host_mboxes, size_t n_tiles, const Geom& g, int seq_kb, int one_kb, std::vector<char>& out,
+                         int tap_s)
 {
     const TileBox* b = (const TileBox*)host_boxes;
     const TileBox* q = (const TileBox*)host_mboxes;
     out.resize(n_tiles * sizeof(MirrorRecWords));
     for (size_t i = 0; i < n_tiles; i++) {
-        const MirrorRecWords w = mirror_rec_encode(b[i], q[i], seq_kb, one_kb, g.src_h, g.src_w);
+        const MirrorRecWords w = mirror_rec_encode(b[i], q[i], seq_kb, one_kb, g.src_h, g.src_w, tap_s);
         std::memcpy(&out[i * sizeof(MirrorRecWords)], &w, sizeof(w));
     }
 }
 
 hipError_t launch_ray_lin3_pair_mirror(const KernelCtx& c, const KernelCtx* cdev, const LaunchUnits& lu, uint32_t* flags, const void* boxes,
                                        const void* mboxes, int half_dwords, int mirror_h, const uint32_t* rest_list, int n_rest, int raw_nwp,
-                                       hipStream_t stream, int seq_kb, const void* recs, const void* tap_table)
+                                       hipStream_t stream, int seq_kb, const void* recs, const void* tap_table, int tap_entry_bytes)
 {
     const int n_eyes = lu.n;
     const dim3 full = tile_grid(c.g, 256, 1);
@@ -673,8 +719,12 @@
                 tap_table = nullptr;
 #endif
             if (tap_table) {
-                hipLaunchKernelGGL(k_ray_lin3_pair_mirror_seq_tab, rgrid, block, slds, stream, head_pairs, a.tiles_x_magic, full.x, rows_strip, dst_wh,
-                                   (const double*)tap_table, a.ctx, (unsigned)a.kb | (unsigned)a.mirror_h << 16, a);
+                if (tap_entry_bytes == kTap8EntryBytes)
+                    hipLaunchKernelGGL(k_ray_lin3_pair_mirror_seq_tab8, rgrid, block, slds, stream, head_pairs, a.tiles_x_magic, full.x, rows_strip, dst_wh,
+                                       (const double*)tap_table, a.ctx, (unsigned)a.kb | (unsigned)a.mirror_h << 16, a);
+                else
+                    hipLaunchKernelGGL(k_ray_lin3_pair_mirror_seq_tab, rgrid, block, slds, stream, head_pairs, a.tiles_x_magic, full.x, rows_strip, dst_wh,
+                                       (const double*)tap_table, a.ctx, (unsigned)a.kb | (unsigned)a.mirror_h << 16, a);
                 return hipGetLastError();
             }
             if (c.ray.var_is_w)
diff --git a/vr180_convert_amd/csrc/plan.hip b/vr180_convert_amd/csrc/plan.hip
--- a/vr180_convert_amd/csrc/plan.hip
+++ b/vr180_convert_amd/csrc/plan.hip
@@ -18,6 +18,7 @@
 #include "host_util.hpp"
 #include "kernels.hpp"
 #include "radial_fit.hpp"
+#include "tap_table.hpp"
 
 using namespace v1c;
 
@@ -179,6 +180,7 @@
 }
 
 static constexpr size_t kTapTableMaxBytes = (size_t)64 << 20;
+static constexpr size_t kTapCompactMinBytes = (size_t)8 << 20;
 
 struct v1c_plan {
     int device = 0;
@@ -212,6 +214,7 @@
     const void* mirror_recs = nullptr;
     const void* tap_table = nullptr;
     size_t tap_table_bytes = 0;
+    int tap_entry_bytes = 0;
     const void* mirror_pairs = nullptr;
     const uint32_t* mirror_rest = nullptr;
     int n_mirror_rest = 0;
@@ -761,7 +764,7 @@
 #endif
                             if (p->mirror_raw_nwp > 0) {
                                 std::vector<char> recs;
-                                tile_mirror_records(hb.data(), hm.data(), hb.size() / 32, g, p->mirror_seq_kb, p->mirror_raw_nwp, recs);
+                                tile_mirror_records(hb.data(), hm.data(), hb.size() / 32, g, p->mirror_seq_kb, p->mirror_raw_nwp, recs, tap_table_s(p->ctx));
                                 const char* dr = nullptr;
                                 if ((rc = upload(p, recs, &dr))) {
                                     v1c_plan_destroy(p);
@@ -769,15 +772,18 @@
                                 }
                                 p->mirror_recs = dr;
                             }
-                            if (p->mirror_recs && p->mirror_seq_kb > 0 && mrest.empty() && tap_table_bytes(g) <= kTapTableMaxBytes) {
-                                const size_t tb = tap_table_bytes(g);
+                            int tap_form = tap_table_bytes(g, kTapEntryBytes) > kTapCompactMinBytes ? kTap8EntryBytes : kTapEntryBytes;
+                            if (const char* f = tuning_env("V1C_TAP_FORM"); f && (std::atoi(f) == kTapEntryBytes || std::atoi(f) == kTap8EntryBytes))
+                                tap_form = std::atoi(f);
+                            if (p->mirror_recs && p->mirror_seq_kb > 0 && mrest.empty() && tap_table_bytes(g, tap_form) <= kTapTableMaxBytes) {
+                                const size_t tb = tap_table_bytes(g, tap_form);
                                 void* tt = nullptr;
                                 uint32_t over = 1;
                                 if (hipMalloc(&tt, tb + 16) == hipSuccess) {
                                     uint32_t* flag = (uint32_t*)((char*)tt + tb);
                                     hipError_t te = hipMemset(flag, 0, 16);
                                     if (te == hipSuccess)
-                                        te = launch_fill_tap_table(p->ctx, p->ctx_dev, p->tile_boxes, mbx, tt, flag);
+                                        te = launch_fill_tap_table(p->ctx, p->ctx_dev, p->tile_boxes, mbx, tt, flag, tap_form);
                                     if (te == hipSuccess)
                                         te = hipMemcpy(&over, flag, sizeof(over), hipMemcpyDeviceToHost);
                                     if (te != hipSuccess) {
@@ -786,14 +792,14 @@
                                         return fail(V1C_E_HIP, std::string("tap table: ") + hipGetErrorString(te));
                                     }
                                     if (over == 0)
-                                        p->allocs.push_back(tt), p->tap_table = tt, p->tap_table_bytes = tb;
+                                        p->allocs.push_back(tt), p->tap_table = tt, p->tap_table_bytes = tb, p->tap_entry_bytes = tap_form;
                                     else
                                         (void)hipFree(tt);
                                 } else {
                                     (void)hipGetLastError();
                                 }
                                 if (const char* dbg = tuning_env("V1C_DEBUG"); dbg && dbg[0] == '1')
-                                    std::fprintf(stderr, "[v1c] tap table: %zu bytes, %s\n", tb, p->tap_table ? "in use" : "not kept");
+                                    std::fprintf(stderr, "[v1c] tap table: %zu bytes, %d per lane, %s\n", tb, tap_form, p->tap_table ? "in use" : "not kept");
                             }
                             std::vector<uint32_t> mrest1;
                             if (p->mirror_raw_nwp > 0 && tile_mirror_rest(hb.data(), hm.data(), g, p->half_dwords, g.dst_h, mrest1, p->mirror_raw_nwp, true, 1)) {
@@ -857,6 +863,11 @@
 extern "C" int64_t v1c_plan_tap_table_bytes(const v1c_plan* p)
 {
     return p ? (int64_t)p->tap_table_bytes : 0;
+}
+
+extern "C" int v1c_plan_tap_entry_bytes(const v1c_plan* p)
+{
+    return p ? p->tap_entry_bytes : 0;
 }
 
 extern "C" int v1c_plan_path(const v1c_plan* p)
@@ -1105,7 +1116,7 @@
             HIP_TRY(launch_ray_lin3_pair_mirror(p->ctx, p->ctx_dev, lu, flags, p->tile_boxes, p->mirror_raw_nwp > 0 ? p->mirror_pairs : p->mirror_boxes,
                                                 p->half_dwords, p->mirror_h,
                                                 n == 1 ? p->mirror_rest1 : p->mirror_rest, n == 1 ? p->n_mirror_rest1 : p->n_mirror_rest,
-                                                p->mirror_raw_nwp, st, p->mirror_seq_kb, p->mirror_recs, n == 2 ? p->tap_table : nullptr));
+                                                p->mirror_raw_nwp, st, p->mirror_seq_kb, p->mirror_recs, n == 2 ? p->tap_table : nullptr, p->tap_entry_bytes));
         } else if (d.fast && p->ctx.g.cn != 3) {
             if (p->cn_kb > 0 && !d.any_rot && shared && aligned) {
                 kind = V1C_LAUNCH_CN;
diff --git a/vr180_convert_amd/csrc/tap_table.hpp b/vr180_convert_amd/csrc/tap_table.hpp
--- a/vr180_convert_amd/csrc/tap_table.hpp
+++ b/vr180_convert_amd/csrc/tap_table.hpp
@@ -66,6 +66,66 @@
     return c;
 }
 
+constexpr int kTap8EntryBytes = 8;
+constexpr int kTap8DxMax = 1023;
+constexpr int kTap8DyMin = -512, kTap8DyMax = 511;
+constexpr int kTap8DdMin = -4, kTap8DdMax = 3;
+constexpr int kTap8EMin = -2, kTap8EMax = 1;
+
+struct TapEntry8 {
+    uint32_t w[2];
+};
+static_assert(sizeof(TapEntry8) == kTap8EntryBytes, "two dwords per lane");
+
+__host__ __device__ inline int tap_sext(uint32_t w, int pos, int bits)
+{
+    return (int)(w << (32 - bits - pos)) >> (32 - bits);
+}
+
+__host__ __device__ inline bool tap8_fits(const TapCoords& c, int K)
+{
+    const int dx1 = c.x[1] - c.x[0], dy1 = c.y[1] - c.y[0];
+    bool ok = c.x[0] >= 0 && c.x[0] <= kTapBaseMax && c.y[0] >= 0 && c.y[0] <= kTapBaseMax && dx1 >= 0 && dx1 <= kTap8DxMax &&
+              dy1 >= kTap8DyMin && dy1 <= kTap8DyMax;
+    for (int k = 2; k < kTapPX; k++) {
+        const int ddx = (c.x[k] - c.x[k - 1]) - (c.x[k - 1] - c.x[k - 2]), ddy = (c.y[k] - c.y[k - 1]) - (c.y[k - 1] - c.y[k - 2]);
+        ok = ok && ddx >= kTap8DdMin && ddx <= kTap8DdMax && ddy >= kTap8DdMin && ddy <= kTap8DdMax;
+    }
+    for (int k = 0; k < kTapPX; k++) {
+        const int e = c.y2[k] - (K - c.y[k]);
+        ok = ok && e >= kTap8EMin && e <= kTap8EMax;
+    }
+    return ok;
+}
+
+__host__ __device__ inline TapEntry8 tap8_encode(const TapCoords& c, int K)
+{
+    uint32_t dd[2][2], e[kTapPX];
+    for (int k = 2; k < kTapPX; k++) {
+        dd[0][k - 2] = (uint32_t)((c.x[k] - c.x[k - 1]) - (c.x[k - 1] - c.x[k - 2])) & 7u;
+        dd[1][k - 2] = (uint32_t)((c.y[k] - c.y[k - 1]) - (c.y[k - 1] - c.y[k - 2])) & 7u;
+    }
+    for (int k = 0; k < kTapPX; k++)
+        e[k] = (uint32_t)(c.y2[k] - (K - c.y[k])) & 3u;
+    TapEntry8 o;
+    o.w[0] = ((uint32_t)c.x[0] & 4095u) | ((uint32_t)(c.x[1] - c.x[0]) & 1023u) << 12 | dd[0][0] << 22 | dd[0][1] << 25 | e[0] << 28 | e[1] << 30;
+    o.w[1] = ((uint32_t)c.y[0] & 4095u) | ((uint32_t)(c.y[1] - c.y[0]) & 1023u) << 12 | dd[1][0] << 22 | dd[1][1] << 25 | e[2] << 28 | e[3] << 30;
+    return o;
+}
+
+__host__ __device__ inline TapCoords tap8_decode(const TapEntry8& t, int K)
+{
+    TapCoords c;
+    const int dx1 = (int)((t.w[0] >> 12) & 1023u), dx2 = dx1 + tap_sext(t.w[0], 22, 3), dx3 = dx2 + tap_sext(t.w[0], 25, 3);
+    const int dy1 = tap_sext(t.w[1], 12, 10), dy2 = dy1 + tap_sext(t.w[1], 22, 3), dy3 = dy2 + tap_sext(t.w[1], 25, 3);
+    c.x[0] = (int)(t.w[0] & 4095u), c.x[1] = c.x[0] + dx1, c.x[2] = c.x[1] + dx2, c.x[3] = c.x[2] + dx3;
+    c.y[0] = (int)(t.w[1] & 4095u), c.y[1] = c.y[0] + dy1, c.y[2] = c.y[1] + dy2, c.y[3] = c.y[2] + dy3;
+    const int e[kTapPX] = {tap_sext(t.w[0], 28, 2), (int)t.w[0] >> 30, tap_sext(t.w[1], 28, 2), (int)t.w[1] >> 30};
+    for (int k = 0; k < kTapPX; k++)
+        c.y2[k] = K - c.y[k] + e[k];
+    return c;
+}
+
 }
 
 #ifdef V1C_TAP_TABLE_OWN_QUALIFIERS
diff --git a/vr180_convert_amd/csrc/tile_device.hpp b/vr180_convert_amd/csrc/tile_device.hpp
--- a/vr180_convert_amd/csrc/tile_device.hpp
+++ b/vr180_convert_amd/csrc/tile_device.hpp
@@ -1607,6 +1607,7 @@
     MirrorRecBox b, q;
     int idx0, nidx;
     uint32_t flags;
+    int tap_k;
 };
 struct MirrorRecWords {
     uint32_t w[16];
@@ -1655,7 +1656,8 @@
     r.magic = w3, r.lpitch = (w2 & 0xffu) * 16u, r.tapk = w4;
     return r;
 }
-__host__ __device__ inline MirrorRecWords mirror_rec_encode(const TileBox& b, const TileBox& q, int seq_kb, int one_kb, int src_h, int src_w)
+__host__ __device__ inline MirrorRecWords mirror_rec_encode(const TileBox& b, const TileBox& q, int seq_kb, int one_kb, int src_h, int src_w,
+                                                            int tap_s = 0)
 {
     MirrorRecWords o;
     MirrorRecBox rb, rq;
@@ -1670,7 +1672,8 @@
     o.w[10] = fit ? (uint32_t)b.idx0 : 0u;
     o.w[11] = (fit ? (uint32_t)b.nidx : 1u) |
               (((b.interior & 2) ? kMirrorRecMpoly : 0u) | (fit_seq ? kMirrorRecFitSeq : 0u) | (fit_one ? kMirrorRecFitOne : 0u)) << 16;
-    o.w[12] = o.w[13] = o.w[14] = o.w[15] = 0u;
+    o.w[12] = fit_seq ? (uint32_t)(tap_s - 32 * (b.y0 + q.y0)) : 0u;
+    o.w[13] = o.w[14] = o.w[15] = 0u;
     return o;
 }
 __host__ __device__ inline MirrorRec mirror_rec_decode(const MirrorRecWords& v)
@@ -1679,6 +1682,7 @@
     r.b = mirror_rec_unbox(v.w[0], v.w[1], v.w[2], v.w[3], v.w[4]);
     r.q = mirror_rec_unbox(v.w[5], v.w[6], v.w[7], v.w[8], v.w[9]);
     r.idx0 = (int)v.w[10], r.nidx = (int)(v.w[11] & 0xffffu), r.flags = v.w[11] >> 16;
+    r.tap_k = (int)v.w[12];
     return r;
 }
 __device__ __forceinline__ MirrorRec load_mirror_rec(const TileBox* pairs, int tile)
diff --git a/vr180_convert_amd/remapper.py b/vr180_convert_amd/remapper.py
--- a/vr180_convert_amd/remapper.py
+++ b/vr180_convert_amd/remapper.py
@@ -149,6 +149,12 @@
         f = getattr(_native.lib(), "v1c_plan_tap_table_bytes", None)
         return int(f(self._h)) if f is not None else 0
 
+    def tap_entry_bytes(self) -> int:
+        f = getattr(_native.lib(), "v1c_plan_tap_entry_bytes", None)
+        if f is None:
+            return 12 if self.tap_table_bytes() else 0
+        return int(f(self._h))
+
     def run(self, srcs: Sequence[torch.Tensor], dsts: Sequence[torch.Tensor], rots: Sequence[Any] | None = None) -> None:
         n = len(srcs)
         if n == 0 or len(dsts) != n or (rots is not None and len(rots) != n):
@@ -237,6 +243,10 @@
 
 def last_tap_table_bytes() -> list[int]:
     return [p.tap_table_bytes() if isinstance(p, Plan) else 0 for p in getattr(_TLS, "plans", [])]
+
+
+def last_tap_entry_bytes() -> list[int]:
+    return [p.tap_entry_bytes() if isinstance(p, Plan) else 0 for p in getattr(_TLS, "plans", [])]
 
 
 def last_auto_radius_form() -> str:
```
